# TorontoDeepLearning/convnet

Hardware: AMD Instinct MI355X
Metric: images/sec (fprop+bprop+wgrad) AlexNet 224x224 bs=256 (higher is better)
Workload: dtype f32

## Files before the change

convnet_amd/_lib.py:

```python
import ctypes
import os
import re

_HERE = os.path.dirname(os.path.abspath(__file__))
LIB_PATH = os.path.join(_HERE, "lib", "libconvnet_hip.so")
_ALT_LIB = os.environ.get("CONVNET_HIP_LIB")
if _ALT_LIB:
    LIB_PATH = _ALT_LIB if os.path.isabs(_ALT_LIB) else os.path.join(_HERE, "lib", _ALT_LIB)
HEADER_PATH = os.path.join(os.path.dirname(_HERE), "include", "convnet_hip.h")

c_float_p = ctypes.POINTER(ctypes.c_float)


class cudamat(ctypes.Structure):
    _fields_ = [("data_host", c_float_p),
                ("data_device", ctypes.c_void_p),
                ("on_device", ctypes.c_int),
                ("on_host", ctypes.c_int),
                ("size", ctypes.c_int * 2),
                ("is_trans", ctypes.c_int),
                ("owns_data", ctypes.c_int),
                ("tex_obj", ctypes.c_ulonglong)]


class Shape4D(ctypes.Structure):
    _fields_ = [("shape", ctypes.c_int * 4)]


class ConvDesc(ctypes.Structure):
    _fields_ = [(n, ctypes.c_int) for n in (
        "num_input_channels", "num_output_channels", "kernel_size_y", "kernel_size_x", "kernel_size_t",
        "stride_y", "stride_x", "stride_t", "padding_y", "padding_x", "padding_t",
        "input_channel_begin", "input_channel_end", "output_channel_begin", "output_channel_end", "num_groups")]

    def copy(self):
        c = ConvDesc()
        ctypes.memmove(ctypes.byref(c), ctypes.byref(self), ctypes.sizeof(ConvDesc))
        return c


class rnd_struct(ctypes.Structure):
    _fields_ = [("dev_mults", ctypes.c_void_p), ("dev_words", ctypes.c_void_p)]


class KernelInfo(ctypes.Structure):
    _fields_ = [("name", ctypes.c_char_p), ("flops", ctypes.c_double), ("grid_blocks", ctypes.c_int), ("split_k", ctypes.c_int)]


_CTYPES = {
    "void": None, "int": ctypes.c_int, "unsigned int": ctypes.c_uint, "long": ctypes.c_long, "size_t": ctypes.c_size_t,
    "float": ctypes.c_float, "double": ctypes.c_double, "bool": ctypes.c_bool,
    "void*": ctypes.c_void_p, "void**": ctypes.POINTER(ctypes.c_void_p), "char*": ctypes.c_char_p, "const char*": ctypes.c_char_p,
    "int*": ctypes.POINTER(ctypes.c_int), "float*": c_float_p, "const float*": c_float_p, "double*": ctypes.POINTER(ctypes.c_double),
    "cudamat*": ctypes.POINTER(cudamat), "cudamat**": ctypes.POINTER(ctypes.POINTER(cudamat)), "Shape4D*": ctypes.POINTER(Shape4D),
    "ConvDesc": ConvDesc, "rnd_struct*": ctypes.POINTER(rnd_struct), "ConvnetHipKernelInfo*": ctypes.POINTER(KernelInfo)}


def _ctype(decl, named, proto):
    tok = decl.replace("*", " * ").split()
    spell = lambda t: " ".join(t).replace(" *", "*")
    if named and len(tok) > 1 and tok[-1] != "*" and spell(tok) not in _CTYPES:
        tok = tok[:-1]
    if spell(tok) not in _CTYPES:
        raise ImportError(f"include/convnet_hip.h: '{proto}' uses the type '{spell(tok)}', which convnet_amd/_lib.py (_CTYPES) does not map")
    return _CTYPES[spell(tok)]


def header_signatures(text):
    body = re.sub(r"/\*.*?\*/", "", text, flags=re.S)
    body = body[body.index('extern "C" {'):]
    sigs = {}
    for res, name, args in re.findall(r"^[ \t]*([A-Za-z_][\w \t*]*?)\s*\b(\w+)\s*\(([^();{}]*)\)\s*;", body, flags=re.M):
        proto = f"{' '.join(res.split())} {name}({' '.join(args.split())})"
        args = [a for a in args.split(",") if a.split() not in ([], ["void"])]
        sigs[name] = (_ctype(res, False, proto), [_ctype(a, True, proto) for a in args])
    return sigs


def declared_symbols(header_path=HEADER_PATH):
    return sorted(header_signatures(open(header_path).read()))


def _load():
    if not os.path.exists(LIB_PATH):
        raise ImportError(
            f"{LIB_PATH} is missing: build it with `python -c 'import __graft_entry__ as g; g.build()'` "
            "(hipcc --offload-arch=gfx950).  There is no CPU fallback for the product path.")
    import torch
    lib = ctypes.CDLL(LIB_PATH)
    for name, (res, args) in header_signatures(open(HEADER_PATH).read()).items():
        if _ALT_LIB and not hasattr(lib, name):
            continue
        fn = getattr(lib, name)
        fn.restype = res
        fn.argtypes = args
    return lib


lib = _load()

_ERRORS = {
    -1: "Incompatible matrix dimensions.", -2: "CUBLAS error.", -3: "CUDA error: ", -4: "Operation not supported on views.",
    -5: "Operation not supported on transposed matrices.", -6: "Generic error.",
    -7: "Incompatible transposedness.", -8: "Matrix is not in device memory.", -9: "Operation not supported."}


def profile_enable(on=True):
    lib.convnet_hip_profile_enable(1 if on else 0)


def profile_report():
    buf = ctypes.create_string_buffer(1 << 16)
    n = lib.convnet_hip_profile_report(buf, len(buf))
    rows = []
    for line in buf.value.decode().splitlines() if n else []:
        k, op, cnt, ms, fl, by, ex = line.split("|")
        rows.append({"kernel": k, "op": op, "launches": int(cnt), "ms": float(ms), "flops": float(fl), "bytes": float(by), "executed": float(ex)})
    return rows


def GetStringError(err_code):
    msg = _ERRORS.get(err_code, "Unknown error")
    if err_code == -3:
        msg += lib.get_last_cuda_error().decode()
    return msg


def probe_matrix_pipe(random_operands=True, seconds=0.05):
    out = (ctypes.c_double * 4)()
    rc = lib.convnet_hip_probe_matrix_pipe(1 if random_operands else 0, float(seconds), out)
    if rc != 0:
        raise RuntimeError(f"convnet_hip_probe_matrix_pipe failed: {rc}")
    return {"bf16_tflops": out[0], "tflops_eq": out[1], "ghz_counter": out[2], "ghz_issue": out[3]}
```

convnet_amd/build.py:

```python
import os
import subprocess
import sys

HERE = os.path.dirname(os.path.abspath(__file__))
SRC = os.path.join(HERE, "csrc")
OUT = os.path.join(HERE, "lib", "libconvnet_hip.so")
SOURCES = ["state.hip", "gather_gemm.hip", "patch_gemm.hip", "wgrad_wide.hip", "fewc_conv.hip", "local_conv.hip", "conv3d.hip", "batch_norm.hip", "pool_norm.hip", "elementwise.hip", "input_staging.hip", "dataset_moments.hip", "feature_rows.hip", "comm.hip", "rccl_abi_check.hip", "probe.hip"]
FLAGS = ["--offload-arch=gfx950", "-O3", "-std=c++17", "-fPIC", "-Wno-comment", "-Wno-inline-asm"]
FILE_FLAGS = {"patch_gemm.hip": ["-fno-slp-vectorize"], "wgrad_wide.hip": ["-fno-slp-vectorize"], "fewc_conv.hip": ["-fno-slp-vectorize"]}
if os.environ.get("CONVNET_BUILD_NOSLP"):
    FILE_FLAGS["gather_gemm.hip"] = ["-fno-slp-vectorize"]
if os.environ.get("CONVNET_BUILD_DIAG"):
    FLAGS.append("-DCONVNET_DIAG")


def _stale(target, deps):
    if not os.path.exists(target):
        return True
    t = os.path.getmtime(target)
    return any(os.path.getmtime(d) > t for d in deps)


def build(force=False, verbose=False):
    os.makedirs(os.path.join(HERE, "lib"), exist_ok=True)
    objdir = os.path.join(HERE, "lib", "obj")
    os.makedirs(objdir, exist_ok=True)
    headers = [os.path.join(SRC, "common.h"), os.path.join(SRC, "gather_gemm.h"), os.path.join(SRC, "wgrad_wide_schedule.h"),
               os.path.join(HERE, "..", "include", "convnet_hip.h")]
    objs, procs = [], []
    for s in SOURCES:
        src = os.path.join(SRC, s)
        obj = os.path.join(objdir, s.replace(".hip", ".o"))
        objs.append(obj)
        if force or _stale(obj, [src] + headers):
            cmd = ["hipcc", *FLAGS, *FILE_FLAGS.get(s, []), "-c", src, "-o", obj]
            if verbose:
                print(" ".join(cmd))
            procs.append((s, subprocess.Popen(cmd, stdout=subprocess.PIPE, stderr=subprocess.STDOUT, text=True)))
    failed = False
    for s, p in procs:
        out, _ = p.communicate()
        if p.returncode != 0:
            failed = True
            print(f"--- {s} failed ---\n{out}", file=sys.stderr)
        elif verbose and out.strip():
            print(out)
    if failed:
        raise RuntimeError("hipcc failed")
    if force or procs or _stale(OUT, objs):
        cmd = ["hipcc", "--offload-arch=gfx950", "-shared", "-fPIC", "-o", OUT, *objs, "-ldl"]
        r = subprocess.run(cmd, capture_output=True, text=True)
        if r.returncode != 0:
            print(r.stdout, r.stderr, file=sys.stderr)
            raise RuntimeError("link failed")
    return OUT


if __name__ == "__main__":
    print(build(force="--force" in sys.argv, verbose=True))
```

convnet_amd/convnet.py:

```python
import os
import sys
from collections import deque
from typing import Callable, NamedTuple, Optional

import torch

from . import pbtxt
from .edge import AvgPoolEdge, ConvEdge, Edge, EdgeWithWeight, FCEdge, LocalEdge, MaxPoolEdge, ResponseNormEdge
from .layer import Layer, LinearLayer, LogisticLayer, ReLULayer, SoftmaxDistLayer, SoftmaxLayer
from .matrix import Matrix
from .optimizer import RunFusedSteps
from .trainer import TrainLoopMixin


class LayerPlan(NamedTuple):
    fuse_relu: Optional[bool]
    bn_relu: Optional[bool]
    activate: bool
    output_entry: Optional[Callable]
    logistic_dropout: bool
    dropout_scale: float
    down_scale: Optional[float]
    logistic_deriv: bool


def _zero_storage(m):
    t = getattr(m, "_t", None)
    if t is not None:
        t.zero_()


class ConvNet(TrainLoopMixin):
    def __init__(self, model, fused=False, process_id=0, num_processes=1, verbose=False, exchange=None, overlap_update=None,
                 overlap_wgrad=None):
        self.verbose = verbose
        self.fused = fused
        self.overlap_update_ = bool(overlap_update)
        self.overlap_wgrad_ = bool(overlap_wgrad)
        self.wgrad_order_ = os.environ.get("CONVNET_WGRAD_ORDER", "before")
        self.side_stream_ = None
        self._pending_updates = []
        self._in_train_step = False
        self.process_id_ = process_id
        self.num_processes_ = num_processes
        self.is_root_ = process_id == 0
        self.exchange_ = exchange
        if isinstance(model, pbtxt.Model):
            self.model_ = model
        elif "\n" in model or "{" in model:
            self.model_ = pbtxt.parse(model)
        else:
            self.model_ = pbtxt.read(model)
        m = self.model_
        for e in m.edge:
            if Edge.HasParameters(e):
                w_opt = m.default_weight_optimizer.copy()
                w_opt.MergeFrom(e.weight_optimizer)
                e.mutable("weight_optimizer").CopyFrom(w_opt)
                if not e.has_no_bias:
                    b_opt = m.default_bias_optimizer.copy()
                    b_opt.MergeFrom(e.bias_optimizer)
                    e.mutable("bias_optimizer").CopyFrom(b_opt)
        for l in m.layer:
            if l.batch_normalize:
                w_opt = m.default_weight_optimizer.copy()
                w_opt.MergeFrom(l.gamma_optimizer)
                l.mutable("gamma_optimizer").CopyFrom(w_opt)
                b_opt = m.default_bias_optimizer.copy()
                w_opt.MergeFrom(l.beta_optimizer)
                l.mutable("beta_optimizer").CopyFrom(b_opt)
        Matrix.InitRandom(m.seed + process_id)
        self.model_name_ = m.name
        self.layers_, self.edges_ = [], []
        self.input_layers_, self.output_layers_, self.data_layers_ = [], [], []
        self.batch_size_ = 0
        self.current_iter_ = 0
        self.parameters_, self.grad_parameters_, self.history_ = Matrix(), Matrix(), Matrix()
        self.second_history_ = Matrix()
        self.edge_slices_ = {}
        self.train_dataset_ = None
        self.train_dataset_config_ = self.valid_dataset_config_ = None
        self.correct_accum_ = None
        self._logits_pending = set()
        self._bn_steps = []
        self.BuildNet()
        if exchange is not None and any(l.UseBatchNormalization() for l in self.layers_):
            raise SystemExit("batch_normalize is not supported with a gradient exchange (data-parallel training)")

    def log(self, *a):
        if self.verbose:
            print(*a, file=sys.stderr)

    def BuildNet(self):
        m = self.model_
        self.layers_ = [Layer.ChooseLayerClass(l) for l in m.layer]
        self.edges_ = [Edge.ChooseEdgeClass(e) for e in m.edge]
        by_name = {e.GetName(): e for e in self.edges_}
        for e in self.edges_:
            if e.IsTied():
                e.SetTiedTo(by_name[e.GetTiedEdgeName()])
        for l in self.layers_:
            for e in self.edges_:
                if l.GetName() == e.GetSourceName():
                    l.AddOutgoing(e)
                    e.SetSource(l)
                    e.SetInputChannels(l.GetNumChannels(e.GetSourceSliceName()))
                if l.GetName() == e.GetDestName():
                    l.AddIncoming(e)
                    e.SetDest(l)
                    e.SetOutputChannels(l.GetNumChannels(e.GetDestSliceName()))
        self.Sort()
        for x in (*self.edges_, *self.layers_):
            x.fused = self.fused
            for opt in (getattr(x, n, None) for n in ("weight_optimizer_", "bias_optimizer_", "gamma_optimizer_", "beta_optimizer_")):
                if opt is not None:
                    opt.fused = self.fused
        for l in self.layers_:
            if l.UseBatchNormalization():
                self._check_batch_norm(l)
            self._check_slices(l)
            if not l.incoming_edge_:
                self.input_layers_.append(l)
                self.data_layers_.append(l)
            if not l.outgoing_edge_:
                self.output_layers_.append(l)
                self.data_layers_.append(l)
        for l in self.layers_:
            if l.IsInput():
                y, x, t = l.GetSizeY(), l.GetSizeX(), l.GetSizeT()
                if y <= 0:
                    y = m.patch_size
                if x <= 0:
                    x = m.patch_size
                if t <= 0:
                    t = 1
            else:
                e0 = l.incoming_edge_[0]
                y, x, t = e0.GetNumModulesY(), e0.GetNumModulesX(), e0.GetNumModulesT()
            l.SetSize(y, x, t)
            if t > 1 and l.UseBatchNormalization():
                raise SystemExit(f"batch_normalize on layer {l.GetName()}: not supported on a layer with image_size_t > 1 ({t} frames)")
            if t > 1 and l.HasSlices():
                raise SystemExit(f"layer_slice on layer {l.GetName()}: not supported on a layer with image_size_t > 1 ({t} frames): "
                                 "time is the outermost index, so a channel range is not one column range")
            self.log(f"Layer {l.GetName()}: {y}x{x}")
            for e in l.outgoing_edge_:
                e.SetImageSize(y, x, t)
        self.PlanLayers()

    def PlanLayers(self):
        self.plan_ = {l: self._plan_layer(l) for l in self.layers_}
        self.metric_on_device_ = len(self.output_layers_) == 1 and self.plan_[self.output_layers_[0]].output_entry is not None

    def _fused_down_scale(self, l):
        return self.plan_[l].down_scale

    def _plan_layer(self, l):
        fused, hidden = self.fused, not l.IsInput() and not l.IsOutput()
        bn, logistic, scale = l.UseBatchNormalization(), isinstance(l, LogisticLayer), l.TrainDropoutScale()
        for e in l.incoming_edge_:
            if isinstance(e, MaxPoolEdge):
                e.mask_legal_ = l.dropprob_ == 0 and type(l) in (LinearLayer, ReLULayer)
        fuse_up = (fused and self._each_alone_and_all_of(l, [e.GetDestSliceName() for e in l.incoming_edge_])
                   and not isinstance(l, SoftmaxLayer) and all(e.CanFuseUp(l) for e in l.incoming_edge_))
        activate = not fused if bn else not l.IsInput() and (not fuse_up or logistic)
        entry = None
        if fused and l.IsOutput() and not l.IsInput():
            single = len(self.output_layers_) == 1 and l.dropprob_ <= 0
            if type(l) is SoftmaxLayer:
                entry = Matrix.SoftmaxCEGradCorrect
            elif single and logistic and (l.loss_function_, l.performance_metric_) == ("CROSS_ENTROPY_BINARY", "CLASSIFICATION_BINARY"):
                entry = Matrix.LogisticCEGradCorrect
            elif single and isinstance(l, SoftmaxDistLayer) and l.loss_function_ == l.performance_metric_ == "CROSS_ENTROPY_MULTINOMIAL_DISTRIBUTED":
                entry = Matrix.SoftmaxDistCEGrad
        down_scale = None
        if fused and hidden and l.is_relu and self._each_alone_and_all_of(l, [e.GetSourceSliceName() for e in l.outgoing_edge_]):
            if all(e.can_fuse_mask and not e.IsBackPropBlocked() and not l.store_dropout_noise_
                   and not (isinstance(e, MaxPoolEdge) and scale != 1.0) for e in l.outgoing_edge_):
                down_scale = scale
        return LayerPlan(fuse_relu=(l.is_relu and not bn) if fuse_up else None, bn_relu=(fused and l.is_relu) if bn else None,
                         activate=activate, output_entry=entry, logistic_dropout=fused and logistic and not l.IsInput() and l.dropprob_ > 0,
                         dropout_scale=scale, down_scale=down_scale, logistic_deriv=fused and logistic and hidden)

    @staticmethod
    def _each_alone_and_all_of(l, slice_names):
        if slice_names == [""]:
            return True
        if not slice_names:
            return False
        return (len(set(slice_names)) == len(slice_names) and set(slice_names) == set(l.slice_channels_)
                and l.GetNumChannels() == sum(l.slice_channels_.values()))

    @staticmethod
    def _check_slices(l):
        name = l.GetName()
        for what, edges, get in (("read", l.outgoing_edge_, Edge.GetSourceSliceName), ("written", l.incoming_edge_, Edge.GetDestSliceName)):
            whole = [e.GetName() for e in edges if not get(e)]
            part = [e.GetName() for e in edges if get(e)]
            if whole and part:
                raise SystemExit(f"layer_slice on layer {name}: the layer is {what} both whole (edge {whole[0]}) and by slice (edge {part[0]}); "
                                 "their add-or-overwrite flags are independent, so one would overwrite what the other has written")
        if l.UseBatchNormalization():
            if l.HasSlices():
                raise SystemExit(f"batch_normalize on layer {name}: not supported on a layer with slices")
            for e in l.incoming_edge_:
                if e.GetSourceSliceName():
                    raise SystemExit(f"batch_normalize on layer {name}: not supported on a layer fed from a slice (edge {e.GetName()})")

    @staticmethod
    def _check_batch_norm(l):
        name = l.GetName()
        if l.IsInput() or l.IsOutput():
            raise SystemExit(f"batch_normalize on layer {name}: input and output layers cannot be batch-normalised")
        if type(l) not in (LinearLayer, ReLULayer):
            raise SystemExit(f"batch_normalize on layer {name}: only LINEAR and RECTIFIED_LINEAR activations are supported")
        for e in l.incoming_edge_:
            if isinstance(e, (MaxPoolEdge, ResponseNormEdge)):
                raise SystemExit(f"batch_normalize on layer {name}: not supported behind a {e.__class__.__name__} (edge {e.GetName()})")
            if not isinstance(e, (FCEdge, ConvEdge, LocalEdge, AvgPoolEdge)):
                raise SystemExit(f"batch_normalize on layer {name}: edge {e.GetName()} ({e.__class__.__name__}) is not supported")

    def Sort(self):
        L, S = [], deque(l for l in self.layers_ if l.IsInput())
        if not S:
            raise SystemExit("Error: No layer is set to be input!")
        while S:
            n = S.popleft()
            L.append(n)
            for e in n.outgoing_edge_:
                e.SetMark()
                mm = e.GetDest()
                if mm is None:
                    raise SystemExit(f"Edge {e.GetName()} has no destination layer")
                if all(f.HasMark() for f in mm.incoming_edge_):
                    S.append(mm)
        if not all(f.HasMark() for f in self.edges_):
            raise SystemExit("Error : Network has loop(s)!")
        self.layers_ = L

    def GetLayerByName(self, name):
        for l in self.layers_:
            if l.GetName() == name:
                return l
        raise SystemExit(f"Error: No layer called {name}")

    def GetEdgeByName(self, name):
        for e in self.edges_:
            if e.GetName() == name:
                return e
        raise SystemExit(f"Error: No edge called {name}")

    def SetBatchsize(self, batch_size):
        self.batch_size_ = batch_size

    def AllocateMemory(self, fprop_only=False):
        self.AllocateLayerMemory()
        self.AllocateEdgeMemory(fprop_only)
        if self.fused:
            self.correct_accum_ = Matrix()
            self.correct_accum_.AllocateGPUMemory(1, 1, "correct count")
            self.correct_accum_.Set(0.0)

    def AllocateLayerMemory(self):
        for l in self.layers_:
            l.AllocateMemory(self.batch_size_)

    def AllocateEdgeMemory(self, fprop_only):
        total, usage = 0, {}
        for e in self.edges_:
            mem = e.GetParameterMemoryRequirement()
            usage[e] = mem
            total += ((mem + 127) // 128) * 128
        self.parameters_.AllocateGPUMemory(1, total, "parameters")
        _zero_storage(self.parameters_)
        if not fprop_only:
            self.grad_parameters_.AllocateGPUMemory(1, total, "grad parameters")
            self.grad_parameters_.Set(0.0)
            self.history_.AllocateGPUMemory(1, total, "optimizer history")
            _zero_storage(self.history_)
            second = any(o is not None and o.NeedsSecondHistory() for e in self.edges_ if isinstance(e, EdgeWithWeight)
                         for o in (e.weight_optimizer_, e.bias_optimizer_))
            if second:
                self.second_history_.AllocateGPUMemory(1, total, "optimizer second-moment history")
                _zero_storage(self.second_history_)
        offset = 0
        for e in self.edges_:
            mem = usage[e]
            if mem == 0:
                continue
            s = Matrix()
            self.parameters_.GetSlice(s, offset, offset + mem)
            e.SetMemory(s)
            if not fprop_only:
                g, h, h2 = Matrix(), Matrix(), None
                self.grad_parameters_.GetSlice(g, offset, offset + mem)
                self.history_.GetSlice(h, offset, offset + mem)
                if second:
                    h2 = Matrix()
                    self.second_history_.GetSlice(h2, offset, offset + mem)
                e.SetGradMemory(g, h, h2)
            self.edge_slices_[e] = (offset, mem)
            offset += ((mem + 127) // 128) * 128
        if self.is_root_ or self.exchange_ is None:
            for e in self.edges_:
                e.Initialize()
# ... 66 lines not shown
            ev = torch.cuda.Event()
            ev.record(torch.cuda.current_stream())
            self._pending_updates.append((owner, ev, isinstance(owner, FCEdge)))
            self._flush_updates(final=False)

    def _flush_updates(self, final):
        keep = []
        for edge, ev, held in self._pending_updates:
            if held and not final:
                keep.append((edge, ev, held))
                continue
            bucket_ev = None
            if self.exchange_ is not None and edge in self.edge_slices_:
                state = self.exchange_.BucketState(edge)
                if state == "pending":
                    if final:
                        raise RuntimeError(f"gradient bucket of {edge.GetName()} was never exchanged")
                    keep.append((edge, ev, held))
                    continue
                bucket_ev = state
            self.side_stream_.wait_event(ev)
            if bucket_ev is not None and not hasattr(bucket_ev, "wait_library_stream"):
                self.side_stream_.wait_event(bucket_ev)
            with Matrix.OnStream(self.side_stream_):
                if hasattr(bucket_ev, "wait_library_stream"):
                    bucket_ev.wait_library_stream()
                edge.UpdateWeights()
        self._pending_updates = keep

    def Bprop(self):
        for l in reversed(self.layers_):
            p = self.plan_[l]
            for e in l.outgoing_edge_:
                self._bprop_edge(e.GetDest(), l, e, fuse_mask=p.down_scale)
            if p.logistic_deriv:
                l.GetDeriv().LogisticDerivScaled(l.GetState(), p.dropout_scale)
            elif p.down_scale is None:
                l.ApplyDerivativeofDropout()
                if not l.IsInput() and not l.IsOutput():
                    l.ApplyDerivativeOfActivation()
            if l.UseBatchNormalization():
                if not self.fused and self._in_train_step and self.side_stream_ is not None and self.overlap_wgrad_:
                    ev = torch.cuda.Event()
                    ev.record(self.side_stream_)
                    torch.cuda.current_stream().wait_event(ev)
                l.ApplyDerivativeofBatchNormalization(self._bn_steps if (self.fused and self._in_train_step) else None)

    def ComputeDeriv(self):
        for l in self.output_layers_:
            if l in self._logits_pending:
                self._logits_pending.discard(l)
                self.plan_[l].output_entry(l.GetState(), l.GetData(), l.GetState(), l.GetDeriv(), self.correct_accum_, l.loss_function_weight_)
            else:
                l.ComputeDeriv()

    def GetLoss(self):
        return None if self.metric_on_device_ else [l.GetPerformanceMetric() for l in self.output_layers_]

    def TimestampModel(self):
        import time
        ts = time.strftime("%Y%m%d%H%M%S")
        while ts in self.model_.timestamp:
            ts += "_"
        self.model_.timestamp.append(ts)
        fname = os.path.join(self.model_.checkpoint_dir, f"{self.model_.name}_{ts}")
        if self.model_.checkpoint_dir:
            os.makedirs(self.model_.checkpoint_dir, exist_ok=True)
            pbtxt.write(fname + ".pbtxt", self.model_)
        self.log_file_ = fname + "_train.log"
        self.val_log_file_ = fname + "_valid.log"
        return ts

    def ReadCorrectCount(self, reset=True):
        v = float(self.correct_accum_.ToNumpy().reshape(-1)[0])
        if reset:
            self.correct_accum_.Set(0.0)
        return v

    def UpdateWeights(self):
        bn_steps, self._bn_steps = self._bn_steps, []
        if self._in_train_step and self.side_stream_ is not None:
            if self.overlap_update_:
                self._flush_updates(final=True)
            done = torch.cuda.Event()
            done.record(self.side_stream_)
            torch.cuda.current_stream().wait_event(done)
            if self.overlap_update_:
                RunFusedSteps(bn_steps)
                return
        batch = list(bn_steps) if self.fused else None
        for e in self.edges_:
            if e.IsBackPropBlocked():
                continue
            if self.exchange_ is not None and e in self.edge_slices_:
                self.exchange_.WaitFor(e)
            if batch is not None and isinstance(e, EdgeWithWeight):
                e.UpdateWeights(batch)
            else:
                e.UpdateWeights()
        if batch:
            RunFusedSteps(batch)

    def SetupDataset(self, dataset, val_data_config_file=""):
        if not isinstance(dataset, str):
            self.train_dataset_ = dataset
            self.batch_size_ = dataset.GetBatchSize()
            return
        if dataset:
            self.train_dataset_config_ = pbtxt.read(dataset, pbtxt.DatasetConfig)
        if val_data_config_file:
            self.valid_dataset_config_ = pbtxt.read(val_data_config_file, pbtxt.DatasetConfig)
        if self.train_dataset_config_ is None:
            raise SystemExit("Error: No training set provided.")
        if self.valid_dataset_config_ is None:
            self.log("Warning: No validation set provided.")
        self.train_dataset_ = self._build_data_handler(self.train_dataset_config_)
        self.SetBatchsize(self.train_dataset_.GetBatchSize())
        self.log("Training data set size", self.train_dataset_.GetDataSetSize())
        if self.valid_dataset_config_ is not None:
            self.val_dataset_ = self._build_data_handler(self.valid_dataset_config_)
            self.log("Validation data set size", self.val_dataset_.GetDataSetSize())

    def _build_data_handler(self, config):
        from .datahandler import DataHandler
        dh = DataHandler(config, seed=self.model_.seed + self.process_id_)
        by_name = {l.GetName(): l for l in self.data_layers_}
        for name, st in dh.streams_.items():
            l = by_name.get(name)
            if l is None:
                raise SystemExit(f"Data stream for layer {name}: the model has no input or output layer of that name.")
            if l.IsInput():
                want = l.GetSizeY() * l.GetSizeX() * l.GetSizeT() * l.GetNumChannels()
                if st.StagedDims() != want:
                    raise SystemExit(f"Data stream for layer {name}: the stream stages {st.StagedDims()} values per case "
                                     f"(rows of {st.GetDims()}, cropped to gpu_image_size), the layer holds {want}.")
        dh.SetInputLayers([l.GetName() for l in self.data_layers_ if l.IsInput()])
        return dh

    def GetBatch(self, dataset):
        dataset.GetBatch(self.data_layers_)

    def TrainOneBatch(self):
        for l in self.layers_:
            l.ResetAddOrOverwrite()
        for e in self.edges_:
            e.NotifyStart()
        for l in self.layers_:
            l.NotifyStart()
        if self.exchange_ is not None:
            self.exchange_.StartStep()
        if (self.overlap_update_ or self.overlap_wgrad_) and self.side_stream_ is None and torch.cuda.is_available():
            self.side_stream_ = Matrix.SharedStream("side")
        self.GetBatch(self.train_dataset_)
        self.Fprop(True)
        self.ComputeDeriv()
        error = self.GetLoss()
        self._in_train_step = True
        try:
            self.Bprop()
            self.UpdateWeights()
        finally:
            self._in_train_step = False
        self.current_iter_ += 1
        return error

    def ReduceLearningRate(self, factor):
        for e in self.edges_:
            if isinstance(e, EdgeWithWeight):
                e.ReduceLearningRate(factor)

    def GetCheckpointFilename(self):
        m = self.model_
        ts = m.timestamp[-1] if m.timestamp else ""
        return os.path.join(m.checkpoint_dir, f"{m.name}_{ts}.h5")

    def Save(self, output_file=None):
        from . import hdf5io
        if output_file is None:
            fname = self.GetCheckpointFilename()
            self.Save(fname)
            if self.model_.polyak_after > 0:
                self.LoadPolyakWeights()
                self.Save(fname + "polyak")
                self.LoadCurrentWeights()
            return
        tmp = output_file + "temp"
        with hdf5io.File(tmp, "w") as f:
            for e in self.edges_:
                e.SaveParameters(f)
            f.WriteHDF5IntAttr("__lr_reduce_counter__", getattr(self, "lr_reduce_counter_", 0))
            f.WriteHDF5IntAttr("__current_iter__", self.current_iter_)
        os.replace(tmp, output_file)

    def Load(self, input_file=None):
        from . import hdf5io
        with hdf5io.File(input_file or self.GetCheckpointFilename()) as f:
            for e in self.edges_:
                e.LoadParameters(f)
            self.lr_reduce_counter_ = f.ReadHDF5IntAttr("__lr_reduce_counter__", getattr(self, "lr_reduce_counter_", 0))
            for _ in range(self.lr_reduce_counter_):
                self.ReduceLearningRate(self.model_.reduce_lr_factor)
            self.current_iter_ = f.ReadHDF5IntAttr("__current_iter__", self.current_iter_)
```

convnet_amd/csrc/common.h:

```cpp
#pragma once
#include <hip/hip_runtime.h>

#include <cstdint>
#include <cstdio>
#include <cstdlib>

#include "../../include/convnet_hip.h"

namespace chip {

hipStream_t stream();
void* workspace(size_t bytes);
void* workspace_aux(size_t bytes);
void* workspace_planes(size_t bytes);
void* workspace_banks(size_t bytes);
void* workspace_slabs(size_t bytes);
const float* zero_page();
int matrix_path();
void set_last_error(const char* msg);
void note_kernel(const char* name, double flops, int blocks, int split_k);

struct KernelTimer {
  KernelTimer(const char* name, const char* op, double flops, double bytes, double executed = 0.0);
  ~KernelTimer();
  int slot;
};

struct PendingOp {
  int kind;
  cudamat m[4];
  Shape4D s[3];
  ConvDesc desc;
  float scaleTargets;
  int i0, i1;
  float f0, f1;
  bool b0;
  cudamat bias, mask;
  int has_bias, relu, has_mask;
  void (*launch)(PendingOp&);
};
bool defer_begin(int kind, void (*launch)(PendingOp&));
PendingOp& pending();
void flush_pending();
extern long g_absorbed;

[[noreturn]] inline void fatal(const char* what, const char* file, int line) {
  fprintf(stderr, "libconvnet_hip: fatal: %s (%s:%d)\n", what, file, line);
  exit(EXIT_FAILURE);
}

#define CHIP_CHECK(expr)                                                            \
  do {                                                                              \
    hipError_t _e = (expr);                                                         \
    if (_e != hipSuccess) ::chip::fatal(hipGetErrorString(_e), __FILE__, __LINE__); \
  } while (0)

#define CHIP_REQUIRE(cond)                                       \
  do {                                                           \
    if (!(cond)) ::chip::fatal("check failed: " #cond, __FILE__, __LINE__); \
  } while (0)

inline int launch_status() {
  hipError_t e = hipGetLastError();
  if (e != hipSuccess) {
    set_last_error(hipGetErrorString(e));
    return CUDA_ERROR;
  }
  return 0;
}

inline int env_int(const char* name, int dflt) {
  const char* e = getenv(name);
  return e && *e ? atoi(e) : dflt;
}
#define CHIP_KNOB(name, dflt) ([] { static const int v_ = ::chip::env_int(name, dflt); return v_; }())
#ifdef CONVNET_DIAG
#define CHIP_DIAG_KNOB(name, dflt) CHIP_KNOB(name, dflt)
#else
#define CHIP_DIAG_KNOB(name, dflt) (dflt)
#endif

void filter_planes_share(bool on);
bool filter_planes_shared(const long long* key, int n);
void wg_batch_begin(int frames, void* (*slab_arena)(size_t bytes), size_t max_bytes);
bool wg_batch_active();
int wg_batch_frame();
void wg_batch_end();

inline int divup(int a, int b) { return (a + b - 1) / b; }
inline size_t numel(const cudamat* m) { return (size_t)m->size[0] * (size_t)m->size[1]; }
inline bool aligned16(const void* p) { return (reinterpret_cast<uintptr_t>(p) & 15) == 0; }

}
```

convnet_amd/csrc/elementwise.hip:

```cpp
#include <cfloat>
#include <climits>
#include <cmath>

#include "common.h"

namespace chip {

using f32x4 = __attribute__((ext_vector_type(4))) float;

constexpr int kThreads = 256;
constexpr int kMaxBlocks = 2048;

inline int blocks_for(size_t work_items) {
  size_t b = (work_items + kThreads - 1) / kThreads;
  if (b > kMaxBlocks) b = kMaxBlocks;
  if (b < 1) b = 1;
  return (int)b;
}

template <typename F>
__global__ void map2_kernel(float* __restrict__ out, const float* a, const float* b, size_t n, bool vec, F f) {
  const size_t tid = (size_t)blockIdx.x * blockDim.x + threadIdx.x, stride = (size_t)gridDim.x * blockDim.x;
  if (vec) {
    const size_t n4 = n >> 2;
// ... 678 lines not shown
}

__device__ __forceinline__ void sgd_one(float& g, float& w, float& h, float l2, float clip, float eps, float mom) {
#pragma clang fp contract(off)
  if (l2 > 0.f) {
    const float t = w * l2;
    g = g + t;
  }
  if (clip > 0.f) g = g > clip ? clip : (g < -clip ? -clip : g);
  g = g * eps;
  const float hm = h * mom;
  h = hm + g;
  w = w - h;
}

__device__ __forceinline__ void adagrad_one(float& g, float& w, float& h, float& a, float delta, float step_scale, float l2, float clip, float eps,
                                            float mom) {
#pragma clang fp contract(off)
  const float c = a - delta;
  const float cc = c * c;
  const float gg = g * g;
  const float s = cc + gg;
  a = delta + sqrtf(s);
  g = g / a;
  g = g * step_scale;
  sgd_one(g, w, h, l2, clip, eps, mom);
}
__device__ __forceinline__ void rmsprop_one(float& g, float& w, float& h, float& a, float factor, float l2, float clip, float eps, float mom) {
#pragma clang fp contract(off)
  h = h * mom;
  if (l2 > 0.f) {
    const float t = w * l2;
    g = g + t;
  }
  if (clip > 0.f) g = g > clip ? clip : (g < -clip ? -clip : g);
  const float fa = factor * a;
  const float faa = fa * a;
  const float omf = 1.f - factor;
  const float og = omf * g;
  const float ogg = og * g;
  const float s = faa + ogg;
  a = sqrtf(s);
  g = g / a;
  const float eg = eps * g;
  h = h + eg;
  w = w - h;
}

struct SgdOp {
  static constexpr int N = 3;
  static constexpr bool kRefuseHuge = false;
  float l2, clip, eps, mom;
  __device__ __forceinline__ void operator()(float (&v)[N]) const { sgd_one(v[0], v[1], v[2], l2, clip, eps, mom); }
};
struct AdagradOp {
  static constexpr int N = 4;
  static constexpr bool kRefuseHuge = true;
  float delta, step_scale, l2, clip, eps, mom;
  __device__ __forceinline__ void operator()(float (&v)[N]) const { adagrad_one(v[0], v[1], v[2], v[3], delta, step_scale, l2, clip, eps, mom); }
};
struct RmsPropOp {
  static constexpr int N = 4;
  static constexpr bool kRefuseHuge = true;
  float factor, l2, clip, eps, mom;
  __device__ __forceinline__ void operator()(float (&v)[N]) const { rmsprop_one(v[0], v[1], v[2], v[3], factor, l2, clip, eps, mom); }
};
template <typename Op>
struct StepItem {
  float* p[Op::N];
  unsigned long long n;
  Op op;
  int vec;
};
template <typename Op>
__device__ __forceinline__ void step_range(const StepItem<Op>& t, size_t tid, size_t stride) {
  constexpr int N = Op::N;
  const size_t n = (size_t)t.n;
  size_t done = 0;
  if (t.vec) {
    const size_t n4 = n >> 2;
    for (size_t i = tid; i < n4; i += stride) {
      f32x4 x[N];
#pragma unroll
      for (int k = 0; k < N; ++k) x[k] = reinterpret_cast<const f32x4*>(t.p[k])[i];
#pragma unroll
      for (int e = 0; e < 4; ++e) {
        float v[N];
#pragma unroll
        for (int k = 0; k < N; ++k) v[k] = x[k][e];
        t.op(v);
#pragma unroll
        for (int k = 0; k < N; ++k) x[k][e] = v[k];
      }
#pragma unroll
      for (int k = 0; k < N; ++k) reinterpret_cast<f32x4*>(t.p[k])[i] = x[k];
    }
    done = n4 << 2;
  }
  for (size_t i = done + tid; i < n; i += stride) {
    float v[N];
#pragma unroll
    for (int k = 0; k < N; ++k) v[k] = t.p[k][i];
    t.op(v);
#pragma unroll
    for (int k = 0; k < N; ++k) t.p[k][i] = v[k];
  }
}
constexpr int kSgdMulti = 16;
template <typename Op>
struct StepBatch {
  StepItem<Op> it[kSgdMulti];
};
template <typename Op>
__device__ __forceinline__ void step_single(const StepItem<Op>& t) {
  step_range(t, (size_t)blockIdx.x * blockDim.x + threadIdx.x, (size_t)gridDim.x * blockDim.x);
}
__global__ void sgd_kernel(const StepItem<SgdOp> t) { step_single(t); }
__global__ void adagrad_kernel(const StepItem<AdagradOp> t) { step_single(t); }
__global__ void rmsprop_kernel(const StepItem<RmsPropOp> t) { step_single(t); }
__global__ void sgd_multi_kernel(const StepBatch<SgdOp> b) { step_single(b.it[blockIdx.y]); }
__global__ void adagrad_multi_kernel(const StepBatch<AdagradOp> b) { step_single(b.it[blockIdx.y]); }
__global__ void rmsprop_multi_kernel(const StepBatch<RmsPropOp> b) { step_single(b.it[blockIdx.y]); }

template <typename Op>
int step_check(cudamat* const (&mats)[Op::N]) {
  const size_t n = numel(mats[1]);
  for (cudamat* m : mats)
    if (!m->on_device) return ERROR_NOT_ON_DEVICE;
  for (cudamat* m : mats)
    if (numel(m) != n) return ERROR_INCOMPATIBLE_DIMENSIONS;
  if (Op::kRefuseHuge && n > (size_t)INT_MAX) return ERROR_UNSUPPORTED;
  return 0;
}
template <typename Op>
StepItem<Op> step_item(cudamat* const (&mats)[Op::N], const Op& op) {
  StepItem<Op> t{};
  t.vec = 1;
  for (int k = 0; k < Op::N; ++k) {
    t.p[k] = mats[k]->data_device;
    t.vec &= aligned16(t.p[k]) ? 1 : 0;
  }
  t.n = numel(mats[1]);
  t.op = op;
  return t;
}
template <typename Op>
constexpr double step_bytes() { return 4.0 * (2 * Op::N - 1); }

template <typename Op, typename K>
int step_launch(K kernel, const char* name, const char* family, cudamat* const (&mats)[Op::N], const Op& op) {
  if (int rc = step_check<Op>(mats)) return rc;
  const size_t n = numel(mats[1]);
  if (n == 0) return 0;
  KernelTimer timer(name, family, 0.0, step_bytes<Op>() * n);
  hipLaunchKernelGGL(kernel, dim3(blocks_for(n / 4 + 1)), dim3(kThreads), 0, stream(), step_item<Op>(mats, op));
  return launch_status();
}
template <typename Op, typename K, typename F>
int step_launch_multi(K kernel, const char* name, const char* family, int count, F tensor) {
  cudamat* mats[Op::N];
  Op op;
  for (int i = 0; i < count; ++i) {
    tensor(i, mats, op);
    if (int rc = step_check<Op>(mats)) return rc;
  }
  for (int base = 0; base < count; base += kSgdMulti) {
    StepBatch<Op> b{};
    int m = 0;
    size_t most = 0, total = 0;
    for (int i = base; i < count && i < base + kSgdMulti; ++i) {
      tensor(i, mats, op);
      const size_t n = numel(mats[1]);
      if (n == 0) continue;
      b.it[m++] = step_item<Op>(mats, op);
      most = n > most ? n : most;
      total += n;
    }
    if (m == 0) continue;
    KernelTimer timer(name, family, 0.0, step_bytes<Op>() * total);
    hipLaunchKernelGGL(kernel, dim3(blocks_for(most / 4 + 1), m), dim3(kThreads), 0, stream(), b);
  }
  return launch_status();
}

}

using namespace chip;

extern "C" {

namespace {
inline bool same_mat(const cudamat* a, const cudamat& b) { return a->on_device && a->data_device == b.data_device && numel(a) == numel(&b); }
bool absorb_bias(cudamat* mat, cudamat* vec, cudamat* target) {
  PendingOp& o = pending();
  if (o.kind != 1 || o.has_bias || o.relu) return false;
  const int F = o.desc.num_output_channels;
  if (!same_mat(mat, o.m[2]) || !same_mat(target, o.m[2]) || mat->is_trans || !vec->on_device || (int)numel(vec) != F || mat->size[1] != F) return false;
  o.bias = *vec;
  o.has_bias = 1;
  ++g_absorbed;
  return true;
}
bool absorb_relu(cudamat* mat, float val, cudamat* target) {
  PendingOp& o = pending();
  if ((o.kind != 1 && o.kind != 4) || o.relu || val != 0.f) return false;
  const cudamat& t = o.kind == 1 ? o.m[2] : o.m[1];
  if (!same_mat(mat, t) || !same_mat(target, t)) return false;
  o.relu = 1;
  flush_pending();
  ++g_absorbed;
  return true;
}
bool absorb_relu_deriv(cudamat* deriv, cudamat* state, cudamat* target) {
  PendingOp& o = pending();
  if ((o.kind != 2 && o.kind != 3) || o.has_mask || !state->on_device || numel(state) != numel(deriv)) return false;
  const cudamat& t = o.kind == 2 ? o.m[2] : o.m[3];
  if (!same_mat(deriv, t) || !same_mat(target, t)) return false;
  if (o.kind == 3 && !same_mat(state, o.m[0])) return false;
  o.mask = *state;
  o.has_mask = 1;
  flush_pending();
  ++g_absorbed;
  return true;
}
}

int add_row_vec(cudamat* mat, cudamat* vec, cudamat* target) {
  if (absorb_bias(mat, vec, target)) return 0;
  return add_row(mat, vec, target, 1.0f);
}
int add_row_mult(cudamat* mat, cudamat* vec, cudamat* target, float mult) { return add_row(mat, vec, target, mult); }

int sum_by_axis(cudamat* mat, cudamat* target, int axis, float mult, float p) { return axis_sum<false>(mat, target, axis, mult, p); }
int sqsum_by_axis(cudamat* mat, cudamat* target, int axis, float mult, float p) { return axis_sum<true>(mat, target, axis, mult, p); }

float sum_all(cudamat* mat, int* err_code) { return reduce_all<0>(mat, nullptr, err_code); }
float vdot(cudamat* mat1, cudamat* mat2, int* err_code) {
  if (numel(mat1) != numel(mat2)) { *err_code = ERROR_INCOMPATIBLE_DIMENSIONS; return 0.f; }
  return reduce_all<1>(mat1, mat2, err_code);
}
float euclid_norm(cudamat* mat, int* err_code) { return sqrtf(reduce_all<2>(mat, nullptr, err_code)); }

int normlimit_by_axis(cudamat* mat, cudamat* target, int axis, float norm, int constraint) {
  if (!mat->on_device || !target->on_device) return ERROR_NOT_ON_DEVICE;
  if (mat->is_trans) return ERROR_TRANSPOSED;
  if (mat->size[0] != target->size[0] || mat->size[1] != target->size[1]) return ERROR_INCOMPATIBLE_DIMENSIONS;
  const int rows = mat->size[0], cols = mat->size[1];
  if (axis == 0)
    hipLaunchKernelGGL(normlimit_cols_kernel, dim3(cols), dim3(256), 0, stream(), mat->data_device, target->data_device, rows, norm, constraint);
  else
    return rows_normlimit(nullptr, mat->data_device, target->data_device, nullptr, rows, cols, norm, constraint, false, 0.f, 0.f, 0.f, 0.f);
  return launch_status();
}

int sgd_momentum_step_normlimit(cudamat* grad, cudamat* param, cudamat* history, float l2_decay, float gradient_clip, float epsilon,
                                float momentum, float norm, int constraint) {
  const size_t n = numel(param);
  if (!grad->on_device || !param->on_device || !history->on_device) return ERROR_NOT_ON_DEVICE;
  if (numel(grad) != n || numel(history) != n) return ERROR_INCOMPATIBLE_DIMENSIONS;
  if (param->is_trans) return ERROR_TRANSPOSED;
  if (n == 0) return 0;
  return rows_normlimit(grad->data_device, param->data_device, param->data_device, history->data_device, param->size[0], param->size[1], norm,
                        constraint, true, l2_decay, gradient_clip, epsilon, momentum);
}

int lower_bound_scalar(cudamat* mat, float val, cudamat* target) {
  if (absorb_relu(mat, val, target)) return 0;
  return map2(target, mat, nullptr, [val] __device__(float x, float) { return x > val ? x : val; });
}
int upper_bound_mod_scalar(cudamat* mat, float val, cudamat* target) {
  return map2(target, mat, nullptr, [val] __device__(float x, float) { return x > val ? val : (x < -val ? -val : x); });
}
int apply_rectified_linear_deriv(cudamat* mat1, cudamat* mat2, cudamat* target) {
  if (absorb_relu_deriv(mat1, mat2, target)) return 0;
  return map2(target, mat1, mat2, [] __device__(float d, float s) { return s > 0.f ? d : 0.f * d; });
}
int assign_scalar(cudamat* mat, float alpha) {
  return map2(mat, mat, nullptr, [alpha] __device__(float, float) { return alpha; });
}
int add_scalar(cudamat* mat, float alpha, cudamat* target) {
  return map2(target, mat, nullptr, [alpha] __device__(float x, float) { return x + alpha; });
}
int mult_by_scalar(cudamat* mat, float alpha, cudamat* target, float scale_targets) {
  if (scale_targets == 0.f) return map2(target, mat, nullptr, [alpha] __device__(float x, float) { return x * alpha; });
  return map2(target, mat, target, [alpha, scale_targets] __device__(float x, float t) { return scale_targets * t + x * alpha; });
}
int divide_by_scalar(cudamat* mat, float alpha, cudamat* target) {
  return map2(target, mat, nullptr, [alpha] __device__(float x, float) { return x / alpha; });
}
int add_mult(cudamat* mat1, cudamat* mat2, float alpha) {
  return map2(mat1, mat1, mat2, [alpha] __device__(float x, float y) {
#pragma clang fp contract(off)
    const float t = alpha * y;
    return x + t;
  });
}
int add_elementwise(cudamat* mat1, cudamat* mat2, cudamat* target) {
  return map2(target, mat1, mat2, [] __device__(float x, float y) { return x + y; });
}
int subtract_elementwise(cudamat* mat1, cudamat* mat2, cudamat* target) {
  return map2(target, mat1, mat2, [] __device__(float x, float y) { return x - y; });
}
int mult_elementwise(cudamat* mat1, cudamat* mat2, cudamat* target, float scale_targets) {
  if (scale_targets != 0.f) return ERROR_UNSUPPORTED;
  return map2(target, mat1, mat2, [] __device__(float x, float y) { return x * y; });
}
int apply_sqrt(cudamat* mat, cudamat* target) {
  return map2(target, mat, nullptr, [] __device__(float x, float) { return sqrtf(x); });
}

int softmax_row_major_multi(cudamat* mat, int numslices, cudamat* target) {
  if (!mat->on_device || !target->on_device) return ERROR_NOT_ON_DEVICE;
  if (mat->is_trans) return ERROR_TRANSPOSED;
  const size_t len = numel(mat);
  if (numslices <= 0 || len % numslices != 0 || numel(target) != len) return ERROR_INCOMPATIBLE_DIMENSIONS;
  const int rows = (int)(len / numslices), cols = numslices;
  SoftmaxOut o{target->data_device, nullptr, nullptr};
  hipLaunchKernelGGL(softmax_rows_kernel<32>, dim3(divup(rows, 32)), dim3(1024), 0, stream(), mat->data_device, nullptr, o, rows, cols, 1.0f);
  return launch_status();
}
int softmax_row_major(cudamat* mat, cudamat* target) { return softmax_row_major_multi(mat, mat->size[1], target); }

int apply_softmax_grad_row_major(cudamat* mat, cudamat* labels, cudamat* target) {
  if (!mat->on_device || !labels->on_device || !target->on_device) return ERROR_NOT_ON_DEVICE;
  if (numel(labels) != (size_t)mat->size[0] || numel(target) != numel(mat)) return ERROR_INCOMPATIBLE_DIMENSIONS;
  if (target->data_device != mat->data_device) {
    int rc = copy_on_device(mat, target);
    if (rc) return rc;
  }
  hipLaunchKernelGGL(softmax_grad_kernel, dim3(divup(mat->size[0], 256)), dim3(256), 0, stream(), labels->data_device, target->data_device, mat->size[0]);
  return launch_status();
}

int get_softmax_correct_row_major(cudamat* mat, cudamat* labels, cudamat* target) {
  if (!mat->on_device || !labels->on_device || !target->on_device) return ERROR_NOT_ON_DEVICE;
  if (mat->is_trans) return ERROR_TRANSPOSED;
  if (target->size[0] != mat->size[0] || target->size[1] != 1 || numel(labels) != (size_t)mat->size[0]) return ERROR_INCOMPATIBLE_DIMENSIONS;
  hipLaunchKernelGGL(softmax_correct_kernel, dim3(divup(mat->size[0], 32)), dim3(1024), 0, stream(), mat->data_device, labels->data_device,
                     target->data_device, mat->size[0], mat->size[1]);
  return launch_status();
}

int get_softmax_cross_entropy_row_major(cudamat* mat, cudamat* labels, cudamat* target, float tiny) {
  if (!mat->on_device || !labels->on_device || !target->on_device) return ERROR_NOT_ON_DEVICE;
  if (mat->is_trans) return ERROR_TRANSPOSED;
  if (target->size[0] != mat->size[0] || target->size[1] != 1 || labels->size[0] != mat->size[0] || labels->size[1] != 1)
    return ERROR_INCOMPATIBLE_DIMENSIONS;
  hipLaunchKernelGGL(softmax_ce_kernel, dim3(divup(mat->size[0], 256)), dim3(256), 0, stream(), mat->data_device, labels->data_device,
                     target->data_device, mat->size[0], tiny);
  return launch_status();
}

int softmax_ce_grad_correct(cudamat* logits, cudamat* labels, cudamat* probs, cudamat* deriv, cudamat* correct_accum, float deriv_scale) {
  if (!logits->on_device || !labels->on_device || !probs->on_device) return ERROR_NOT_ON_DEVICE;
  if (numel(probs) != numel(logits) || (deriv && numel(deriv) != numel(logits)) || numel(labels) != (size_t)logits->size[0])
    return ERROR_INCOMPATIBLE_DIMENSIONS;
  SoftmaxOut o{probs->data_device, deriv ? deriv->data_device : nullptr, correct_accum ? correct_accum->data_device : nullptr};
  KernelTimer timer("softmax_rows_kernel", "softmax_ce", 0.0, 4.0 * numel(logits) * (deriv ? 3 : 2));
  hipLaunchKernelGGL(softmax_rows_kernel<32>, dim3(divup(logits->size[0], 32)), dim3(1024), 0, stream(), logits->data_device, labels->data_device, o,
                     logits->size[0], logits->size[1], deriv_scale);
  return launch_status();
}

int sgd_momentum_step(cudamat* grad, cudamat* param, cudamat* history, float l2_decay, float gradient_clip, float epsilon, float momentum) {
  cudamat* const mats[] = {grad, param, history};
  return step_launch<SgdOp>(sgd_kernel, "sgd_kernel", "sgd", mats, SgdOp{l2_decay, gradient_clip, epsilon, momentum});
}

int sgd_momentum_step_multi(int count, cudamat** grads, cudamat** params, cudamat** histories, const float* l2_decay, const float* gradient_clip,
                            const float* epsilon, const float* momentum) {
  if (count < 0 || (count > 0 && (!grads || !params || !histories || !l2_decay || !gradient_clip || !epsilon || !momentum))) return ERROR_GENERIC;
  return step_launch_multi<SgdOp>(sgd_multi_kernel, "sgd_multi_kernel", "sgd", count, [&](int i, cudamat* (&m)[3], SgdOp& op) {
    m[0] = grads[i]; m[1] = params[i]; m[2] = histories[i];
    op = SgdOp{l2_decay[i], gradient_clip[i], epsilon[i], momentum[i]};
  });
}

namespace {
int second_moment_check(const cudamat* a, const cudamat* b, const cudamat* c) {
  if (!a->on_device || !b->on_device || (c && !c->on_device)) return ERROR_NOT_ON_DEVICE;
  if (a->is_trans != b->is_trans) return ERROR_TRANSPOSEDNESS;
  if (numel(a) != numel(b) || (c && numel(a) != numel(c))) return ERROR_INCOMPATIBLE_DIMENSIONS;
  return 0;
}
}

int adagrad(cudamat* history, cudamat* grad, float delta) {
  if (int rc = second_moment_check(history, grad, nullptr)) return rc;
  return map2(history, history, grad, [delta] __device__(float h, float g) {
#pragma clang fp contract(off)
    const float c = h - delta;
    const float cc = c * c;
    const float gg = g * g;
    const float s = cc + gg;
    return delta + sqrtf(s);
  });
}
int rms_prop(cudamat* history, cudamat* grad, float factor) {
  if (int rc = second_moment_check(history, grad, nullptr)) return rc;
  return map2(history, history, grad, [factor] __device__(float h, float g) {
#pragma clang fp contract(off)
    const float fh = factor * h;
    const float fhh = fh * h;
    const float omf = 1.f - factor;
    const float og = omf * g;
    const float ogg = og * g;
    const float s = fhh + ogg;
    return sqrtf(s);
  });
}
int divide_elementwise(cudamat* mat1, cudamat* mat2, cudamat* target) {
  if (int rc = second_moment_check(mat1, mat2, target)) return rc;
  return map2(target, mat1, mat2, [] __device__(float x, float y) { return x / y; });
}
// ... 156 lines not shown
```

convnet_amd/csrc/fewc_conv.hip:

```cpp
#include <algorithm>

#include "gather_gemm.h"

namespace chip {
namespace gfc {

constexpr int KX = 7, KY = 7, CH = 3, S = 2, NR = CH * KY, P = 4, IMG = 32;
constexpr int PW = S * (P - 1) + KX;
constexpr int XB = IMG * 4;
constexpr int RP = 2;
constexpr int ROWB = RP * 1024;
static_assert(PW * XB <= ROWB, "patch row");
constexpr int NCH = 10, ROWS = 96;
constexpr int H0_ROWS = 11, H1_ROWS = 10;
constexpr int H0_BYTES = H0_ROWS * ROWB, H1_BYTES = H1_ROWS * ROWB;
constexpr int BIAS_OFF = 0, BIAS_BYTES = 512;
constexpr int A_OFF = BIAS_BYTES;
constexpr int A_CHUNK = 6 * ROWS * 16;
constexpr int A_BYTES = NCH * A_CHUNK;
constexpr int A_PIECES = A_BYTES / 1024;
constexpr int PATCH_OFF = A_OFF + A_BYTES;
constexpr int ZERO_OFF = PATCH_OFF + H0_BYTES + H1_BYTES;
constexpr int ZERO_BYTES = 1024 + 256;
constexpr int LDS_BYTES = ZERO_OFF + ZERO_BYTES;
static_assert(LDS_BYTES <= 160 * 1024, "LDS");
static_assert(A_BYTES % 1024 == 0, "filter bank in whole pieces");
constexpr int NGROUP = 3 * 4;
constexpr int DUMP_BYTES = 4096;

__host__ __device__ constexpr int row_off(int r) { return r < 10 ? r * ROWB : r == 20 ? 10 * ROWB : H0_BYTES + (r - 10) * ROWB; }
__host__ __device__ constexpr int slot_k(int c, int lh, int j) {
  const int r = 2 * c + (j >> 2), kx = 2 * (j & 3) + lh;
  if (kx < KX) return kx + KX * r;
  return r < KX ? r + KX * 20 : -1;
}

struct Params {
  const float* src;
  const u32x4* planes;
  float* dst;
  float* dump;
  const float* bias;
  const float* zero;
  int F, N, H, W, My, Mx, pady, padx;
  int XG, IB, tiles;
  int relu;
  int diag;
};

}

__global__ void gfc_planes_kernel(const float* __restrict__ W, u32x4* __restrict__ out, int F) {
  using namespace gfc;
  const int i = blockIdx.x * blockDim.x + threadIdx.x;
  if (i >= NCH * 2 * ROWS) return;
  const int f = i % ROWS, lh = (i / ROWS) & 1, c = i / (2 * ROWS);
  Split8 sp = {};
  if (f < F) {
    float x[8];
#pragma unroll
    for (int j = 0; j < 8; ++j) {
      const int k = slot_k(c, lh, j);
      x[j] = k >= 0 ? W[(size_t)f + (size_t)F * k] : 0.f;
    }
    split8_sat(x, sp);
  }
  u32x4* o = out + ((size_t)c * 6 + lh) * ROWS + f;
  o[0] = sp.h;
  o[2 * ROWS] = sp.m;
  o[4 * ROWS] = sp.l;
}

template <bool RELU>
__global__ __launch_bounds__(320, 1) void gfc_kernel(const gfc::Params p) {
  using namespace gfc;
  extern __shared__ __attribute__((aligned(16))) float smem[];
  char* const lds = reinterpret_cast<char*>(smem);
  const int tid = threadIdx.x;
  const int wave = __builtin_amdgcn_readfirstlane(tid >> 6), lane = tid & 63;
  const int N = p.N;

  const int G = gridDim.x, q = p.tiles / G, rem = p.tiles % G, b = blockIdx.x;
  const int T0 = b * q + min(b, rem), T1 = T0 + q + (b < rem ? 1 : 0);
  if (T0 >= T1) return;
  int xg = T0 % p.XG, oy = (T0 / p.XG) % p.My, ib = T0 / (p.XG * p.My);
  auto next_tile = [&]() __attribute__((always_inline)) {
    if (++xg == p.XG) {
      xg = 0;
      if (++oy == p.My) {
        oy = 0;
        ++ib;
      }
    }
  };

  for (int i = wave; i < A_PIECES; i += 5) {
    const char* g = reinterpret_cast<const char*>(p.planes) + (size_t)i * 1024 + lane * 16;
    __builtin_amdgcn_global_load_lds((gbl_ptr_t)g, (lds_ptr_t)(lds + A_OFF + i * 1024), 16, 0, 0);
  }
  if (tid * 16 < ZERO_BYTES) *reinterpret_cast<u32x4*>(lds + ZERO_OFF + tid * 16) = u32x4{0, 0, 0, 0};
  if (tid < BIAS_BYTES / 4) *reinterpret_cast<float*>(lds + BIAS_OFF + tid * 4) = p.bias && tid < p.F ? p.bias[tid] : 0.f;

  if (wave == 4) {
    const int lx = lane >> 3;
    const unsigned lane_off = (unsigned)lx * (unsigned)(N * 4) + (unsigned)(lane & 7) * 16u;
    const size_t plane = (size_t)p.H * p.W * N * 4, rowb = (size_t)p.W * N * 4;
    auto issue_half = [&](auto HH) __attribute__((always_inline)) {
      constexpr int h = decltype(HH)::value;
      constexpr int n = h ? H1_ROWS : H0_ROWS;
      const int y0 = S * oy - p.pady, x0 = S * P * xg - p.padx;
      const char* const origin = reinterpret_cast<const char*>(p.src) + ((ptrdiff_t)y0 * p.W + x0) * (ptrdiff_t)(N * 4) + (ptrdiff_t)ib * (IMG * 4);
      bool xok[RP];
#pragma unroll
      for (int k = 0; k < RP; ++k) xok[k] = 8 * k + lx < PW && (unsigned)(x0 + 8 * k + lx) < (unsigned)p.W;
#pragma unroll
      for (int idx = 0; idx < n; ++idx) {
        const int r = h ? 10 + idx : idx == 10 ? 20 : idx;
        const int ch = r / KY, ky = r % KY;
        const bool yok = (unsigned)(y0 + ky) < (unsigned)p.H;
        const char* const rowp = origin + (size_t)ch * plane + (size_t)ky * rowb;
#pragma unroll
        for (int k = 0; k < RP; ++k) {
          const char* g = yok && xok[k] ? rowp + (size_t)(8 * k) * (size_t)(N * 4) + lane_off : reinterpret_cast<const char*>(p.zero);
          __builtin_amdgcn_global_load_lds((gbl_ptr_t)g, (lds_ptr_t)(lds + PATCH_OFF + (h ? H0_BYTES : 0) + idx * ROWB + k * 1024), 16, 0, 0);
        }
      }
    };
    using H0 = std::integral_constant<int, 0>;
    using H1 = std::integral_constant<int, 1>;
    issue_half(H0{});
    issue_half(H1{});
    __builtin_amdgcn_s_waitcnt(0x0070);
    __syncthreads();
    for (int T = T0; T < T1; ++T) {
      const bool more = T + 1 < T1 && !(p.diag & 2);
      __builtin_amdgcn_s_waitcnt(0x0070);
      __syncthreads();
      next_tile();
      if (more) issue_half(H0{});
      __builtin_amdgcn_s_waitcnt(0x0070);
      __syncthreads();
      if (more) issue_half(H1{});
    }
    __builtin_amdgcn_s_waitcnt(0x0070);
    return;
  }

  const int li = lane & 31, lh = lane >> 5;
  const unsigned base_l = (unsigned)(PATCH_OFF + (S * wave) * XB + li * 4 + lh * XB);
  const unsigned a_l = (unsigned)(A_OFF + (lh * ROWS + li) * 16);
  const unsigned lh_mask = lh ? 0xFFFFFFFFu : 0u;

  f32x16 acc[2][3];
  u32x4 fah[2][3], fam[3], fal[3];
  Split8 fb[2];
  float bv[8];
#ifndef CONVNET_EMU
#define CHIP_HERE() asm volatile("" ::: "memory")
#else
#define CHIP_HERE() ((void)0)
#endif
  auto read_a = [&](auto CC, auto PL, u32x4 (&dst)[3]) __attribute__((always_inline)) {
    constexpr int c = decltype(CC)::value, pl = decltype(PL)::value;
    CHIP_HERE();
#pragma unroll
    for (int t = 0; t < 3; ++t) dst[t] = *reinterpret_cast<const u32x4*>(lds + a_l + c * A_CHUNK + pl * (2 * ROWS * 16) + t * 512);
  };
  auto read_b = [&](auto CC) __attribute__((always_inline)) {
    constexpr int c = decltype(CC)::value;
    unsigned lhm = lh_mask;
    CHIP_HERE();
#ifndef CONVNET_EMU
    asm volatile("" : "+v"(lhm));
#endif
#pragma unroll
    for (int j = 0; j < 8; ++j) {
      const int r = 2 * c + (j >> 2);
      const int imm_n = row_off(r) + 2 * (j & 3) * XB;
      if ((j & 3) != 3) {
        bv[j] = *reinterpret_cast<const float*>(lds + base_l + imm_n);
      } else {
        const int imm_s = r < KX ? row_off(20) + (r - 1) * XB : (ZERO_OFF - PATCH_OFF);
        bv[j] = *reinterpret_cast<const float*>(lds + (base_l + (lhm & (unsigned)(imm_s - imm_n))) + imm_n);
      }
    }
  };
  auto split_pair = [&](int s, int q) __attribute__((always_inline)) {
    const float x0 = bv[2 * q], x1 = bv[2 * q + 1];
    const unsigned H = pk_bf16(x0, x1);
    const float r0 = x0 - __uint_as_float(H << 16), r1 = x1 - __uint_as_float(H & 0xffff0000u);
    const unsigned M = pk_bf16(r0, r1);
    const float s0 = r0 - __uint_as_float(M << 16), s1 = r1 - __uint_as_float(M & 0xffff0000u);
    fb[s].h[q] = H;
    fb[s].m[q] = M;
    fb[s].l[q] = pk_bf16(s0, s1);
#ifndef CONVNET_EMU
    asm volatile("" ::"v"(fb[s].h[q]), "v"(fb[s].m[q]), "v"(fb[s].l[q]));
#endif
  };
  auto mac_step = [&](auto K, int s, f32x16 (&a)[3]) __attribute__((always_inline)) {
    constexpr int k = decltype(K)::value;
#pragma unroll
    for (int t = 0; t < 3; ++t) {
      const u32x4& av = k == 1 ? fal[t] : k == 2 || k == 3 ? fam[t] : fah[s][t];
      const u32x4& bw = k == 0 ? fb[s].l : k == 2 || k == 4 ? fb[s].m : fb[s].h;
      a[t] = mma_bf16(av, bw, a[t]);
    }
#ifndef CONVNET_EMU
    asm volatile("" : "+v"(a[0]), "+v"(a[1]), "+v"(a[2]));
#endif
  };

  struct Out {
    unsigned lane_bytes;
    int flim;
  };
  const size_t fstride = (size_t)p.My * p.Mx * N;
  const int q4 = li & 3;
  auto out_of = [&](int xg_, int oy_, int ib_, bool exists) __attribute__((always_inline)) {
    const int ox = P * xg_ + wave;
    Out o;
    o.lane_bytes = (unsigned)((((size_t)oy_ * p.Mx + ox) * N + ib_ * IMG + 4 * (li >> 2) + (size_t)(q4 + 4 * lh) * fstride) * 4);
    o.flim = exists && ox < p.Mx ? p.F : 0;
// ... 3 lines not shown
    return o;
  };
  const unsigned bias_q = (unsigned)(BIAS_OFF + (q4 + 4 * lh) * 4);
  auto bias_of = [&](auto GG) __attribute__((always_inline)) {
    constexpr int gi = decltype(GG)::value;
    return *reinterpret_cast<const float*>(lds + bias_q + (32 * (gi >> 2) + 8 * (gi & 3)) * 4);
  };
  auto swap1 = [](float v) __attribute__((always_inline)) {
#ifndef CONVNET_EMU
    return __builtin_bit_cast(float, __builtin_amdgcn_mov_dpp(__builtin_bit_cast(int, v), 0xB1, 0xF, 0xF, true));
#else
    return emu::shfl_xor(v, 1);
#endif
  };
  auto swap2 = [](float v) __attribute__((always_inline)) {
#ifndef CONVNET_EMU
    return __builtin_bit_cast(float, __builtin_amdgcn_mov_dpp(__builtin_bit_cast(int, v), 0x4E, 0xF, 0xF, true));
#else
    return emu::shfl_xor(v, 2);
#endif
  };
  const bool odd1 = (li & 1) != 0, odd2 = (li & 2) != 0;
  auto store_group = [&](auto GG, const Out& o, const f32x16 (&a)[3], float bias) __attribute__((always_inline)) {
    constexpr int gi = decltype(GG)::value, t = gi >> 2, g = gi & 3;
    constexpr int cf = 32 * t + 8 * g;
    float x0 = a[t][4 * g], x1 = a[t][4 * g + 1], x2 = a[t][4 * g + 2], x3 = a[t][4 * g + 3];
    {
      const float r01 = swap1(odd1 ? x0 : x1), r23 = swap1(odd1 ? x2 : x3);
      x0 = odd1 ? r01 : x0; x1 = odd1 ? x1 : r01;
      x2 = odd1 ? r23 : x2; x3 = odd1 ? x3 : r23;
    }
    {
      const float ra = swap2(odd2 ? x0 : x2), rb = swap2(odd2 ? x1 : x3);
      x0 = odd2 ? ra : x0; x1 = odd2 ? rb : x1;
      x2 = odd2 ? x2 : ra; x3 = odd2 ? x3 : rb;
    }
    f32x4 v = {x0 + bias, x1 + bias, x2 + bias, x3 + bias};
    if constexpr (RELU) {
#pragma unroll
      for (int e = 0; e < 4; ++e) v[e] = fmaxf(v[e], 0.f);
    }
    const bool real = cf < o.flim;
    char* const rowb = real ? reinterpret_cast<char*>(p.dst) + (size_t)cf * fstride * 4 : reinterpret_cast<char*>(p.dump);
    const unsigned off = real ? o.lane_bytes : (unsigned)lane * 16u;
#ifdef CONVNET_DIAG
    if (p.diag & 4) return;
#endif
    *reinterpret_cast<f32x4*>(rowb + off) = v;
  };

  auto chunk_body = [&](auto CC, bool has_next, f32x16 (&cur)[3], const f32x16 (&prev)[3], const Out& po) __attribute__((always_inline)) {
    constexpr int c = decltype(CC)::value, s = c & 1;
    using CN = std::integral_constant<int, (c + 1) % NCH>;
    __builtin_amdgcn_sched_barrier(0);
    if (has_next) {
      read_b(CN{});
      read_a(CN{}, std::integral_constant<int, 0>{}, fah[s ^ 1]);
    }
    CHIP_HERE();
    const float bs0 = bias_of(std::integral_constant<int, c>{});
    float bs1 = 0.f;
    if constexpr (c >= 8) bs1 = bias_of(std::integral_constant<int, c + 2>{});
    static_for<0, 6>([&](auto KK) __attribute__((always_inline)) {
      constexpr int k = decltype(KK)::value;
      if constexpr (k >= 1 && k <= 4) {
        if (has_next) split_pair(s ^ 1, k - 1);
      }
      if constexpr (k == 0 && c >= 8) store_group(std::integral_constant<int, c + 2>{}, po, prev, bs1);
      if constexpr (k == 5) store_group(std::integral_constant<int, c>{}, po, prev, bs0);
      if constexpr (k == 2) {
        if (has_next) read_a(CN{}, std::integral_constant<int, 2>{}, fal);
      }
      if constexpr (k == 4) {
        if (has_next) read_a(CN{}, std::integral_constant<int, 1>{}, fam);
      }
      mac_step(KK, s, cur);
#pragma unroll
      for (int i = 0; i < 3; ++i) {
        __builtin_amdgcn_sched_group_barrier(0x008, 1, 0);
        __builtin_amdgcn_sched_group_barrier(0x100, 4, 0);
        __builtin_amdgcn_sched_group_barrier(0x002, 12, 0);
        __builtin_amdgcn_sched_group_barrier(0x040, 1, 0);
      }
      __builtin_amdgcn_sched_barrier(0);
    });
  };
  auto run_tile = [&](bool more, f32x16 (&cur)[3], const f32x16 (&prev)[3], const Out& po) __attribute__((always_inline)) {
#pragma unroll
    for (int t = 0; t < 3; ++t)
#pragma unroll
      for (int e = 0; e < 16; ++e) cur[t][e] = 0.f;
    static_for<0, NCH>([&](auto CC) __attribute__((always_inline)) {
      constexpr int c = decltype(CC)::value;
      if constexpr (c == 4) __syncthreads();
      if constexpr (c == NCH - 1) __syncthreads();
      if constexpr (c + 1 < NCH) chunk_body(CC, true, cur, prev, po);
      else chunk_body(CC, more, cur, prev, po);
    });
  };

  __builtin_amdgcn_s_waitcnt(0x0070);
  __syncthreads();
  {
    using C0 = std::integral_constant<int, 0>;
    read_b(C0{});
    read_a(C0{}, std::integral_constant<int, 0>{}, fah[0]);
    read_a(C0{}, std::integral_constant<int, 1>{}, fam);
    read_a(C0{}, std::integral_constant<int, 2>{}, fal);
  }
#pragma unroll
  for (int q4 = 0; q4 < 4; ++q4) split_pair(0, q4);
  Out po = out_of(0, 0, 0, false);
  int T = T0;
  for (;;) {
    run_tile(T + 1 < T1, acc[0], acc[1], po);
    po = out_of(xg, oy, ib, true);
    next_tile();
    if (++T >= T1) {
      static_for<0, NGROUP>([&](auto GG) __attribute__((always_inline)) { store_group(GG, po, acc[0], bias_of(GG)); });
      break;
    }
    run_tile(T + 1 < T1, acc[1], acc[0], po);
    po = out_of(xg, oy, ib, true);
    next_tile();
    if (++T >= T1) {
      static_for<0, NGROUP>([&](auto GG) __attribute__((always_inline)) { store_group(GG, po, acc[1], bias_of(GG)); });
      break;
    }
  }
}

bool gfc_try(const float* images, const float* filters, const float* bias, float* targets, int N, int C, int H, int W, int F, int Ky, int Kx,
             int sy, int sx, int pady, int padx, int My, int Mx, float scaleTargets, int relu, double flops) {
  using namespace gfc;
  if (!CHIP_KNOB("CONVNET_GG_FEWC", 1) || matrix_path() != 1) return false;
  if (Kx != KX || Ky != KY || C != CH || sy != S || sx != S || F > ROWS || F < 8 || F % 8 != 0 || N % IMG != 0 || My < 1 || Mx < 1) return false;
  if (pady < 0 || padx < 0 || (size_t)C * H * W * N * 4 >= (size_t(1) << 32) || (size_t)F * My * Mx * N * 4 >= (size_t(1) << 32)) return false;
  if (scaleTargets != 0.f) return false;
  if ((reinterpret_cast<uintptr_t>(images) | reinterpret_cast<uintptr_t>(targets)) & 15) return false;
  static bool once = false;
  static int cus = 256;
  if (!once) {
    CHIP_CHECK(hipFuncSetAttribute(reinterpret_cast<const void*>(gfc_kernel<false>), hipFuncAttributeMaxDynamicSharedMemorySize, LDS_BYTES));
    CHIP_CHECK(hipFuncSetAttribute(reinterpret_cast<const void*>(gfc_kernel<true>), hipFuncAttributeMaxDynamicSharedMemorySize, LDS_BYTES));
#ifndef CONVNET_EMU
    int dev = 0;
    hipDeviceProp_t prop;
    if (hipGetDevice(&dev) == hipSuccess && hipGetDeviceProperties(&prop, dev) == hipSuccess && prop.multiProcessorCount > 0) cus = prop.multiProcessorCount;
#else
    cus = 4;
#endif
    once = true;
  }
  u32x4* planes = static_cast<u32x4*>(workspace_aux(A_BYTES + DUMP_BYTES));
  (void)filter_planes_shared(nullptr, 0);
  {
    KernelTimer timer("filter_planes_kernel", "conv_fprop", 0.0, 4.0 * F * C * Ky * Kx + A_BYTES);
    hipLaunchKernelGGL(gfc_planes_kernel, dim3(divup(NCH * 2 * ROWS, 256)), dim3(256), 0, stream(), filters, planes, F);
  }
  Params p{};
  p.src = images; p.planes = planes; p.dst = targets; p.bias = bias; p.zero = zero_page();
  p.dump = reinterpret_cast<float*>(reinterpret_cast<char*>(planes) + A_BYTES);
  p.F = F; p.N = N; p.H = H; p.W = W; p.My = My; p.Mx = Mx; p.pady = pady; p.padx = padx;
  p.XG = divup(Mx, P); p.IB = N / IMG; p.tiles = p.XG * My * p.IB;
  p.relu = relu; p.diag = CHIP_DIAG_KNOB("CONVNET_GFC_DIAG", 0);
  const int grid = std::min(cus, p.tiles);
  {
    KernelTimer timer("gfc_kernel<96x128,split>", "conv_fprop", flops, 0.0, 0.0);
    if (relu) hipLaunchKernelGGL(gfc_kernel<true>, dim3(grid), dim3(320), LDS_BYTES, stream(), p);
    else hipLaunchKernelGGL(gfc_kernel<false>, dim3(grid), dim3(320), LDS_BYTES, stream(), p);
  }
  note_kernel("gfc_kernel(fprop)", flops, grid, 1);
  return true;
}

}
```

convnet_amd/csrc/gather_gemm.h:

```cpp
#pragma once
#include <cmath>
#include <cstring>
#include <type_traits>

#include "common.h"

namespace chip {

using f32x16 = __attribute__((ext_vector_type(16))) float;
using u32x4 = __attribute__((ext_vector_type(4))) unsigned;
using f32x4 = __attribute__((ext_vector_type(4))) float;

constexpr int BK = 16;

#ifdef CONVNET_GG_TRACE
constexpr bool kTrace = CONVNET_GG_TRACE >= 2;
__device__ unsigned long long* g_gg_trace = nullptr;
#else
constexpr bool kTrace = false;
#endif
__device__ __forceinline__ unsigned long long trace_clock() {
#ifdef CONVNET_GG_TRACE
  return __builtin_amdgcn_s_memtime();
#else
// ... 268 lines not shown
            for (int e = 0; e < NTC; ++e) v[e] = v[e] > 0.f ? v[e] : 0.f;
          }
          if (p.mask) {
            const fvec mk = *reinterpret_cast<const fvec*>(p.mask + (dp - p.dst));
#pragma unroll
            for (int e = 0; e < NTC; ++e) v[e] = mk[e] > 0.f ? v[e] * p.post_scale : 0.f;
          }
          *reinterpret_cast<fvec*>(dp) = v;
        } else {
#pragma unroll
          for (int e = 0; e < NTC; ++e) {
            if (n + e < N) {
              float x = v[e];
              if (p.scaleTargets != 0.f) x = p.scaleTargets * dp[e] + x;
              x += bv;
              if (p.relu) x = x > 0.f ? x : 0.f;
              if (p.mask) x = p.mask[(dp - p.dst) + e] > 0.f ? x * p.post_scale : 0.f;
              dp[e] = x;
            }
          }
        }
      } else {
        if (VEC) {
          *reinterpret_cast<fvec*>(dp) = v;
        } else {
#pragma unroll
          for (int e = 0; e < NTC; ++e)
            if (n + e < N) dp[e] = v[e];
        }
      }
    }
  }
}

struct Split8 {
  u32x4 h, m, l;
};
__device__ __forceinline__ unsigned pk_bf16(float a, float b) {
  typedef float f32x2_t __attribute__((ext_vector_type(2)));
  typedef __bf16 bf16x2_t __attribute__((ext_vector_type(2)));
  f32x2_t v = {a, b};
  return __builtin_bit_cast(unsigned, __builtin_convertvector(v, bf16x2_t));
}
__device__ __forceinline__ void split8(const float (&x)[8], Split8& s) {
#pragma unroll
  for (int q = 0; q < 4; ++q) {
    const float x0 = x[2 * q], x1 = x[2 * q + 1];
    const unsigned H = pk_bf16(x0, x1);
    const float r0 = x0 - __uint_as_float(H << 16), r1 = x1 - __uint_as_float(H & 0xffff0000u);
    const unsigned M = pk_bf16(r0, r1);
    const float s0 = r0 - __uint_as_float(M << 16), s1 = r1 - __uint_as_float(M & 0xffff0000u);
    s.h[q] = H;
    s.m[q] = M;
    s.l[q] = pk_bf16(s0, s1);
  }
}
__device__ __forceinline__ void split8_sat(float (&x)[8], Split8& s) {
#pragma unroll
  for (int j = 0; j < 8; ++j)
    if (fabsf(x[j]) > __uint_as_float(0x7F7F7FFFu)) x[j] = copysignf(__uint_as_float(0x7F7F0000u), x[j]);
  split8(x, s);
}
__device__ __forceinline__ f32x16 mma_bf16(u32x4 a, u32x4 b, f32x16 c) {
  typedef __bf16 bf16x8_t __attribute__((ext_vector_type(8)));
  return __builtin_amdgcn_mfma_f32_32x32x16_bf16(__builtin_bit_cast(bf16x8_t, a), __builtin_bit_cast(bf16x8_t, b), c, 0, 0, 0);
}
__device__ __forceinline__ f32x4 mma_bf16(u32x4 a, u32x4 b, f32x4 c) {
  typedef __bf16 bf16x8_t __attribute__((ext_vector_type(8)));
  return __builtin_amdgcn_mfma_f32_16x16x32_bf16(__builtin_bit_cast(bf16x8_t, a), __builtin_bit_cast(bf16x8_t, b), c, 0, 0, 0);
}

template <typename Acc>
__device__ __forceinline__ Acc split_mac(const Split8& a, const Split8& b, Acc v) {
  v = mma_bf16(a.m, b.m, v);
  v = mma_bf16(a.h, b.l, v);
  v = mma_bf16(a.l, b.h, v);
  v = mma_bf16(a.h, b.m, v);
  v = mma_bf16(a.m, b.h, v);
  v = mma_bf16(a.h, b.h, v);
  return v;
}

struct GGTile {
  const float* A;
  int K, GX, G, TX, TYX, y0, x0, dy0, dx0, ncols, col_tiles;
  int L, tsplit;
};
__device__ __forceinline__ bool gg_select_tile(const GGParams& p, const GGClassTable& ct, GGTile& t) {
  t.A = p.A; t.K = p.K; t.GX = p.GX; t.G = p.G; t.TX = p.TX; t.TYX = p.TYX; t.y0 = p.y0; t.x0 = p.x0; t.dy0 = p.dy0; t.dx0 = p.dx0;
  t.ncols = p.ncols; t.col_tiles = p.col_tiles; t.tsplit = -1;
  if (ct.n > 0) {
    const int b = blockIdx.x;
    if (b >= ct.c[ct.n - 1].tile_end) return false;
    int c = 0;
    while (b >= ct.c[c].tile_end) ++c;
    const int cbeg = c > 0 ? ct.c[c - 1].tile_end : 0;
    {
      const int i = b - cbeg, T = ct.c[c].tile_end - cbeg;
      const int q = T >> 3, m = T & 7, r = i & 7;
      t.L = r * q + (r < m ? r : m) + (i >> 3);
    }
    const GGClass& k = ct.c[c];
    t.A = k.A; t.K = k.K; t.GX = k.GX; t.G = k.G; t.TX = k.TX; t.TYX = k.TYX;
    t.y0 = k.y0; t.x0 = k.x0; t.dy0 = k.dy0; t.dx0 = k.dx0; t.ncols = k.ncols; t.col_tiles = k.col_tiles;
  } else if (p.tail_splits > 1) {
    const int k = blockIdx.x & 7, i = blockIdx.x >> 3;
    if (i < p.tail_tf8) {
      t.L = k * p.tail_tf8 + i;
    } else {
      const int j = k * p.tail_tt8 + (i - p.tail_tf8);
      if (j >= (p.row_tiles * t.col_tiles - p.tail_first) * p.tail_splits) return false;
      t.L = p.tail_first + j / p.tail_splits;
      t.tsplit = j % p.tail_splits;
    }
  } else {
    const int tiles = p.row_tiles * t.col_tiles;
    const int per = (tiles + 7) >> 3;
    t.L = xcd_remap(blockIdx.x, tiles);
    if (t.L >= tiles || (int)blockIdx.x >= per * 8) return false;
  }
  return true;
}

constexpr int kTailFixParts = 4;
template <int WR, int WC, int MT, int CW, bool VEC>
__global__ __launch_bounds__(WR* WC * 64) void gg_tail_fix_kernel(const GGParams p) {
  constexpr int NT = WR * WC * 64, NTC = CW / 32, ROWS = WR * MT * 32;
  using fvec = __attribute__((ext_vector_type(NTC))) float;
  const int tile = blockIdx.x / kTailFixParts, part = blockIdx.x % kTailFixParts;
  const int L = p.tail_first + tile;
  const int tid = threadIdx.x;
  const int reg_lo = part * (16 / kTailFixParts), reg_hi = reg_lo + 16 / kTailFixParts;
  f32x16 acc[MT][NTC];
  const float* pp = p.tail_partial + (size_t)tile * p.tail_splits * (size_t)(ROWS * WC * CW);
#pragma unroll
  for (int t = 0; t < MT; ++t)
#pragma unroll
    for (int reg = 0; reg < 16; ++reg) {
      if (reg < reg_lo || reg >= reg_hi) continue;
      fvec v = *reinterpret_cast<const fvec*>(pp + ((size_t)(t * 16 + reg) * NT + tid) * NTC);
      for (int sp = 1; sp < p.tail_splits; ++sp)
        v += *reinterpret_cast<const fvec*>(pp + (size_t)sp * (ROWS * WC * CW) + ((size_t)(t * 16 + reg) * NT + tid) * NTC);
#pragma unroll
      for (int u = 0; u < NTC; ++u) acc[t][u][reg] = v[u];
    }
  gg_epilogue<WR, WC, MT, CW, VEC>(p, acc, L % p.row_tiles, L / p.row_tiles, 0, p.ncols, p.GX, p.G, p.dy0, p.dx0, reg_lo, reg_hi);
}

struct PatchBank {
  const float* W;
  int F, C, Ky, Kx, cy, cx, sy, sx, TYc, TXc;
  bool dgrad;
};
void filter_planes_rt_launch(const PatchBank& bank, void* out, int TYX, int TH, const char* op);
void filter_planes_gk_launch(const float* W, void* out, int F, int K, int KP, int TH, const char* op);
bool patch_shape_ok(GGParams& p, size_t dst_elems);
void patch_run(GGParams& p, size_t dst_elems, const char* op, double flops, const PatchBank& bank);
bool patch_classes_ok(const GGParams& base, const GGClassTable& ct);
void patch_run_classes(GGParams& p, GGClassTable& ct, const char* op, double flops, double exec);

bool gfc_try(const float* images, const float* filters, const float* bias, float* targets, int N, int C, int H, int W, int F, int Ky, int Kx,
             int sy, int sx, int pady, int padx, int My, int Mx, float scaleTargets, int relu, double flops);

struct WGParams {
  const float* src;
  const float* dout;
  float* dst;
  float* partial;
  const float* zero;
  float* bias_dst;
  int K, F, N;
  int GX, M;
  int TX, TYX;
  int SH, SW;
  int ssy, ssx, y0, x0;
  int nchunk;
  int chunks_total;
  int chunks_per_split;
  int splits;
  int k_tiles, f_tiles;
  float scaleTargets, scaleOutput;
  int prio;
  int wide;
};

constexpr int WG_NB = 32;
constexpr int WG_PITCH = WG_NB + 4;

void wg_reduce_launch(const WGParams& p, size_t total, int splits, int groups, const char* op);
float* wg_batch_partial(const WGParams& p, size_t total, int splits);
bool wgw_try(WGParams& p, bool vec, bool split_products, const char* op, double flops, double exec);

void gg_reduce_launch(const GGParams& p, size_t dst_elems, int splits, const char* op);

inline double gg_split_time(int tiles, int sp, double slots, double tile_flops, double block_rate, size_t dst_elems) {
  const double rounds = std::ceil(tiles * (double)sp / slots);
  double t = rounds * (tile_flops / sp) / block_rate;
  if (sp > 1) t += sizeof(float) * (double)dst_elems * (2.0 * sp + 1) / 4.0e12 + 4e-6;
  return t;
}
inline int gg_split_k(int tiles, double slots, double tile_flops, double block_rate, size_t dst_elems, int kchunks, int units,
                      double* best_time = nullptr) {
  int splits = 1;
  double best_t = 1e30;
  if (dst_elems > 0 && kchunks >= 16)
    for (int sp = 1; sp <= 16 && kchunks / sp >= 8 && units / sp >= 1; ++sp) {
      const double t = gg_split_time(tiles, sp, slots, tile_flops, block_rate, dst_elems);
      if (t < best_t * 0.97) {
        best_t = t;
        splits = sp;
      }
    }
  if (best_time) *best_time = best_t;
  return splits;
}
inline bool gg_partial_last_round(int tiles, int slots, int kchunks) { return tiles > slots && tiles % slots != 0 && kchunks >= 32; }
inline int gg_tail_split(int tiles, int slots, double tile_flops, double block_rate, int tile_elems, int kchunks) {
  const int rem = tiles - (tiles / slots) * slots;
  const double tile_bytes = sizeof(float) * (double)tile_elems;
  const double t_round = tile_flops / block_rate;
  double best = 0.95;
  int best_s = 1;
  for (int s = 2; s <= 8 && kchunks / s >= 8; ++s) {
    const double cost = std::ceil(rem * (double)s / slots) / s + (rem * (s + 1.0) * tile_bytes / 4.0e12 + 6e-6) / t_round;
    if (cost < best) {
      best = cost;
      best_s = s;
    }
  }
  return best_s;
}
inline void gg_set_tail(GGParams& p, int tiles, int slots, int units, int s, int tile_elems) {
  const int full = (tiles / slots) * slots, rem = tiles - full;
  p.tail_first = full;
  p.tail_cps = divup(units, s);
  p.tail_splits = divup(units, p.tail_cps);
  p.tail_tf8 = full / 8;
  p.tail_tt8 = divup(rem * p.tail_splits, 8);
  p.tail_partial = static_cast<float*>(workspace(sizeof(float) * (size_t)rem * p.tail_splits * tile_elems));
}

}
```

convnet_amd/csrc/gather_gemm.hip:

```cpp
#include <algorithm>
#include <array>
#include <cmath>
#include <map>
#include <vector>
#include <cstdlib>
#include <string>
#include <type_traits>

#include "common.h"

#include "gather_gemm.h"

namespace chip {

template <int WR, int WC, int MT, int CW, bool A_KCONTIG, bool VEC, bool O3 = false, bool SPLIT = false>
__global__ __launch_bounds__(WR* WC * 64, (O3 ? 3 : 2)) void gg_kernel(const GGParams pin, const GGClassTable ct) {
  constexpr int NT = WR * WC * 64;
  constexpr int NTC = CW / 32, CW4 = CW / 4;
  using fvec = __attribute__((ext_vector_type(NTC))) float;
  constexpr int ROWS = WR * MT * 32;
  constexpr int APITCH = A_KCONTIG ? (BK + 4) : ROWS;
  constexpr int A_STAGE = A_KCONTIG ? ROWS * APITCH : BK * ROWS;
  constexpr int B_STAGE = WC * BK * CW;
  constexpr int NA = ((A_KCONTIG ? ROWS * (BK / 4) : BK * (ROWS / 4)) + NT - 1) / NT;
// ... 1482 lines not shown
}

void gg_run_classes(GGParams& p, GGClassTable& ct, bool vec, const GGTimer& tm) {
  gg_with_tile(gg_tile(p.R, vec, false), [&](auto t) {
    using T = decltype(t);
    gg_launch_classes<T::WR, T::WC, T::MT, T::CW>(p, ct, vec, tm);
  });
}

template <int WM, int WN, int MT, int NTL, int TS = 32>
void wg_launch_cfg(WGParams& p, bool vec, const GGTimer& tm) {
  constexpr int KT = WM * MT * TS, FT = WN * NTL * TS;
  const size_t lds = sizeof(float) * 2 * (KT + FT) * (vec ? WG_NB : WG_PITCH);
  p.k_tiles = divup(p.K, KT);
  if (p.bias_dst && divup(p.K + 1, KT) != p.k_tiles) p.bias_dst = nullptr;
  p.f_tiles = divup(p.F, FT);
  p.zero = zero_page();
  p.prio = wg_prio_mode();
  const int tiles = p.k_tiles * p.f_tiles;
  const size_t total = (size_t)(p.K + (p.bias_dst ? 1 : 0)) * p.F;
  const bool no_wide = CHIP_DIAG_KNOB("CONVNET_WG_NO_WIDE", 0) != 0;
  p.wide = (!no_wide && vec && TS == 32 && WM == 2 && WN == 2 && MT == 2 && NTL == 2 && p.F % 4 == 0 && aligned16(p.dst) &&
            (!p.bias_dst || aligned16(p.bias_dst))) ? 1 : 0;
  int splits = 1;
  if (tiles < kTargetBlocks) {
    splits = kTargetBlocks / tiles;
    const int max_by_len = p.chunks_total / 16 > 0 ? p.chunks_total / 16 : 1;
    if (splits > max_by_len) splits = max_by_len;
    const size_t max_by_bytes = (size_t(256) << 20) / (total * sizeof(float)) + 1;
    if ((size_t)splits > max_by_bytes) splits = (int)max_by_bytes;
    if (splits > 1024) splits = 1024;
    if (splits < 1) splits = 1;
  }
  p.chunks_per_split = divup(p.chunks_total, splits);
  splits = divup(p.chunks_total, p.chunks_per_split);
  p.splits = splits;
  const int groups = splits > 64 ? 32 : 1;
  float* const frame_slabs = wg_batch_partial(p, total, splits);
  p.partial = frame_slabs ? frame_slabs
                          : splits > 1 ? static_cast<float*>(workspace(sizeof(float) * total * (splits + (groups > 1 ? groups : 0)))) : nullptr;
  dim3 grid(((tiles * splits + 7) / 8) * 8), block(WM * WN * 64);
  static const std::string kname_f = "wg_kernel<" + std::to_string(WM) + "," + std::to_string(WN) + "," + std::to_string(MT) + "," + std::to_string(NTL) + (TS == 16 ? ",x16>" : ">");
  static const std::string kname_s = kname_f.substr(0, kname_f.size() - 1) + ",split>";
  const bool split_products = vec && wg_split_mode();
  const std::string& kname = split_products ? kname_s : kname_f;
  {
    KernelTimer timer(kname.c_str(), tm.op, tm.flops, 0.0, tm.exec);
    if (split_products) {
      allow_big_lds(wg_kernel<WM, WN, MT, NTL, true, TS, true>, lds);
      hipLaunchKernelGGL((wg_kernel<WM, WN, MT, NTL, true, TS, true>), grid, block, lds, stream(), p);
    } else if (vec) {
      allow_big_lds(wg_kernel<WM, WN, MT, NTL, true, TS>, lds);
      hipLaunchKernelGGL((wg_kernel<WM, WN, MT, NTL, true, TS>), grid, block, lds, stream(), p);
    } else {
      allow_big_lds(wg_kernel<WM, WN, MT, NTL, false, TS>, lds);
      hipLaunchKernelGGL((wg_kernel<WM, WN, MT, NTL, false, TS>), grid, block, lds, stream(), p);
    }
  }
  if (splits > 1 && !frame_slabs) wg_reduce_launch(p, total, splits, groups, tm.op);
}

void wg_launch(WGParams& p, bool vec, const GGTimer& tm) {
  if (wgw_try(p, vec, vec && wg_split_mode(), tm.op, tm.flops, tm.exec)) return;
  int ft = 128, pad = divup(p.F, 128) * 128;
  const int cands[3] = {96, 64, 32};
  for (int c : cands) {
    const int q = divup(p.F, c) * c;
    if (q < pad) {
      ft = c;
      pad = q;
    }
  }
  const bool k160 = divup(p.K, 160) * 160 < divup(p.K, 128) * 128;
  if (ft == 128) wg_launch_cfg<2, 2, 2, 2>(p, vec, tm);
  else if (ft == 96 && k160) wg_launch_cfg<2, 2, 5, 3, 16>(p, vec, tm);
  else if (ft == 96) wg_launch_cfg<4, 1, 1, 3>(p, vec, tm);
  else if (ft == 64) wg_launch_cfg<4, 1, 1, 2>(p, vec, tm);
  else wg_launch_cfg<4, 1, 1, 1>(p, vec, tm);
}

struct ConvGeo {
  int N, C, H, W, F, Ky, Kx, sy, sx, py, px, My, Mx;
};

ConvGeo conv_geo(const Shape4D* img, const Shape4D* flt, const Shape4D* out, const ConvDesc& d, const cudamat* mi,
                 const cudamat* mf, const cudamat* mo) {
  ConvGeo g;
  g.N = img->shape[0]; g.W = img->shape[1]; g.H = img->shape[2]; g.C = img->shape[3];
  g.Mx = out->shape[1]; g.My = out->shape[2]; g.F = out->shape[3];
  g.Ky = d.kernel_size_y; g.Kx = d.kernel_size_x; g.sy = d.stride_y; g.sx = d.stride_x;
  g.py = d.padding_y; g.px = d.padding_x;
  CHIP_REQUIRE(out->shape[0] == g.N);
  CHIP_REQUIRE(d.num_input_channels == g.C && d.num_output_channels == g.F);
  CHIP_REQUIRE(d.num_groups == 1);
  CHIP_REQUIRE(d.input_channel_begin == 0 && (d.input_channel_end == 0 || d.input_channel_end == g.C));
  CHIP_REQUIRE(d.output_channel_begin == 0 && (d.output_channel_end == 0 || d.output_channel_end == g.F));
  CHIP_REQUIRE(flt->shape[0] == g.F && flt->shape[1] == g.Kx && flt->shape[2] == g.Ky && flt->shape[3] == g.C);
  CHIP_REQUIRE(mi->size[0] == g.N && mi->size[1] == g.H * g.W * g.C);
  CHIP_REQUIRE(mo->size[0] == g.N && mo->size[1] == g.My * g.Mx * g.F);
  CHIP_REQUIRE(mf->size[0] == g.F && mf->size[1] == g.Ky * g.Kx * g.C);
  CHIP_REQUIRE(g.My == (g.H - 2 * g.py - g.Ky) / g.sy + 1 && g.Mx == (g.W - 2 * g.px - g.Kx) / g.sx + 1);
  CHIP_REQUIRE(d.kernel_size_t <= 1);
  CHIP_REQUIRE((size_t)g.N * g.H * g.W * g.C < (1ull << 31) && (size_t)g.N * g.My * g.Mx * g.F < (1ull << 31));
  return g;
}

inline bool gg_presplit_mode() {
  return gg_split_mode() && !CHIP_DIAG_KNOB("CONVNET_GG_NO_PRESPLIT", 0);
}

const unsigned* gk_table(int C, int H, int W, int N, int Ky, int Kx) {
  static std::map<std::array<int, 7>, unsigned*> cache;
  int dev = 0;
  CHIP_CHECK(hipGetDevice(&dev));
  const std::array<int, 7> key = {dev, C, H, W, N, Ky, Kx};
  auto it = cache.find(key);
  if (it != cache.end()) return it->second;
  const int K = C * Ky * Kx, KP = divup(K, BK) * BK;
  std::vector<unsigned> tab(2 * (size_t)KP);
  for (int k = 0; k < KP; ++k) {
    const int kk = std::min(k, K - 1), ch = kk / (Ky * Kx), tap = kk % (Ky * Kx), a = tap / Kx, b = tap % Kx;
    tab[k] = (unsigned)(((size_t)(ch * H + a) * W + b) * N * 4);
    tab[KP + k] = ((unsigned)a << 16) | (unsigned)b;
  }
  unsigned* d = nullptr;
  CHIP_CHECK(hipMalloc((void**)&d, tab.size() * sizeof(unsigned)));
  CHIP_CHECK(hipMemcpy(d, tab.data(), tab.size() * sizeof(unsigned), hipMemcpyHostToDevice));
  cache[key] = d;
  return d;
}

void conv_up_impl(cudamat* images, cudamat* filters, cudamat* bias, cudamat* targets, Shape4D* is, Shape4D* fs, Shape4D* ts,
                  const ConvDesc& d, float scaleTargets, int relu) {
  const ConvGeo g = conv_geo(is, fs, ts, d, images, filters, targets);
  GGParams p{};
  p.A = filters->data_device; p.src = images->data_device; p.dst = targets->data_device;
  p.bias = bias ? bias->data_device : nullptr;
  p.R = g.F; p.K = g.C * g.Ky * g.Kx; p.N = g.N; p.lda = g.F;
  p.GX = g.Mx; p.G = g.My * g.Mx; p.TX = g.Kx; p.TYX = g.Ky * g.Kx;
  p.SH = g.H; p.SW = g.W; p.ssy = g.sy; p.ssx = g.sx; p.y0 = g.py; p.x0 = g.px; p.dir = 1;
  p.DW = g.Mx; p.DP = g.My * g.Mx; p.dsy = 1; p.dsx = 1; p.dy0 = 0; p.dx0 = 0;
  p.scaleTargets = scaleTargets; p.relu = relu;
  const bool vec = g.N % 4 == 0 && g.F % 4 == 0 && aligned16(p.A) && aligned16(p.src) && aligned16(p.dst);
  const size_t dst_elems = (size_t)g.N * p.DP * g.F;
  const GGTimer tm{"conv_fprop", 2.0 * g.N * p.G * (double)g.F * p.K, 0.0};
  if (vec && gg_presplit_mode() && gg_producer_mode() &&
      gfc_try(images->data_device, filters->data_device, p.bias, targets->data_device, g.N, g.C, g.H, g.W, g.F, g.Ky, g.Kx, g.sy, g.sx, -g.py, -g.px,
              g.My, g.Mx, scaleTargets, relu, tm.flops))
    return;
  if (vec && gg_presplit_mode() && gg_producer_mode() && g.C % BK != 0 && g.F > 32 && CHIP_KNOB("CONVNET_GG_GK", 1) &&
      (size_t)g.C * g.H * g.W * g.N < (size_t(1) << 30)) {
    const int K = g.C * g.Ky * g.Kx, KP = divup(K, BK) * BK, TH = gg_tile_rows(g.F);
    void* planes = workspace_aux((size_t)96 * (KP / 16) * divup(g.F, TH) * TH);
    filter_planes_gk_launch(filters->data_device, planes, g.F, K, KP, TH, "conv_fprop");
    p.A = static_cast<const float*>(planes);
    p.apre = 1;
    p.gk = 1;
    p.ktab = gk_table(g.C, g.H, g.W, g.N, g.Ky, g.Kx);
    p.K = KP;
    p.KC = KP;
    gg_run<false>(p, vec, dst_elems, tm);
    note_kernel("gg_kernel(fprop)", tm.flops, p.row_tiles * p.col_tiles, p.splits);
    return;
  }
  if (vec && ggp_shape_ok(g.F, g.C) && gg_presplit_mode()) {
    p.KC = g.C;
    if (patch_shape_ok(p, dst_elems)) {
      const PatchBank bank{filters->data_device, g.F, g.C, g.Ky, g.Kx, 0, 0, 1, 1, g.Ky, g.Kx, false};
      patch_run(p, dst_elems, tm.op, tm.flops, bank);
      note_kernel(convnet_hip_get_patch_mode() >= 3 ? "gpw_kernel(fprop)" : "gpp_kernel(fprop)", tm.flops, p.row_tiles * p.col_tiles, p.splits);
      return;
    }
    p.KC = 0;
  }
  if (vec && ggp_shape_ok(g.F, g.C)) {
    const size_t welems = (size_t)g.F * p.K;
    if (gg_presplit_mode()) {
      const int TH = gg_tile_rows(g.F);
      void* planes = workspace_aux((size_t)96 * (g.C / 16) * p.TYX * divup(g.F, TH) * TH);
      const PatchBank bank{filters->data_device, g.F, g.C, g.Ky, g.Kx, 0, 0, 1, 1, g.Ky, g.Kx, false};
      filter_planes_rt_launch(bank, planes, p.TYX, TH, "conv_fprop");
      p.A = static_cast<const float*>(planes);
      p.apre = 1;
    } else if (p.TYX > 1) {
      float* wt = static_cast<float*>(workspace_aux(sizeof(float) * welems));
      int nb = (int)((welems + 255) / 256);
      if (nb > 2048) nb = 2048;
      const long long key[6] = {2, (long long)(uintptr_t)filters->data_device, (long long)(uintptr_t)wt, g.F, g.C, p.TYX};
      if (!filter_planes_shared(key, 6)) {
        KernelTimer timer("filter_tapmajor_kernel", "conv_fprop", 0.0, 8.0 * welems);
        hipLaunchKernelGGL(filter_tapmajor_kernel, dim3(nb), dim3(256), 0, stream(), filters->data_device, wt, g.F, g.C, p.TYX);
      }
      p.A = wt;
    }
    p.KC = g.C;
  }
  gg_run<false>(p, vec, dst_elems, tm);
  note_kernel("gg_kernel(fprop)", tm.flops, p.row_tiles * p.col_tiles, p.splits);
}

}
}

using namespace chip;

#ifdef CONVNET_GG_TRACE
extern "C" void convnet_hip_debug_set_gg_trace(unsigned long long* dev_buf) {
  CHIP_CHECK(hipMemcpyToSymbol(HIP_SYMBOL(chip::g_gg_trace), &dev_buf, sizeof dev_buf));
}
#endif

extern "C" {

static void conv_down_impl(cudamat* derivs, cudamat* filters, cudamat* targets, Shape4D* ds, Shape4D* fs, Shape4D* ts, const ConvDesc& d,
                           float scaleTargets, cudamat* mask, float post_scale);
static void launch_conv_up(PendingOp& o) {
  conv_up_impl(&o.m[0], &o.m[1], o.has_bias ? &o.bias : nullptr, &o.m[2], &o.s[0], &o.s[1], &o.s[2], o.desc, o.scaleTargets, o.relu);
}
static void launch_conv_down(PendingOp& o) {
  conv_down_impl(&o.m[0], &o.m[1], &o.m[2], &o.s[0], &o.s[1], &o.s[2], o.desc, o.scaleTargets, o.has_mask ? &o.mask : nullptr, 1.0f);
}
static bool park_conv(int kind, void (*launch)(PendingOp&), cudamat* a, cudamat* b, cudamat* c, Shape4D* sa, Shape4D* sb, Shape4D* sc, const ConvDesc& d,
                      float scaleTargets) {
  if (!defer_begin(kind, launch)) return false;
  if (kind == 1) (void)conv_geo(sa, sb, sc, d, a, b, c);
  else (void)conv_geo(sc, sb, sa, d, c, b, a);
  PendingOp& o = pending();
  o.m[0] = *a; o.m[1] = *b; o.m[2] = *c;
  o.s[0] = *sa; o.s[1] = *sb; o.s[2] = *sc;
  o.desc = d;
  o.scaleTargets = scaleTargets;
  return true;
}

void convUp(cudamat* images, cudamat* filters, cudamat* targets, Shape4D* is, Shape4D* fs, Shape4D* ts, ConvDesc d,
            float scaleTargets) {
  if (park_conv(1, launch_conv_up, images, filters, targets, is, fs, ts, d, scaleTargets)) return;
  conv_up_impl(images, filters, nullptr, targets, is, fs, ts, d, scaleTargets, 0);
}

void convUpGemm(cudamat* images, cudamat* filters, cudamat* targets, Shape4D* is, Shape4D* fs, Shape4D* ts, ConvDesc d,
                float scaleTargets) {
  convUp(images, filters, targets, is, fs, ts, d, scaleTargets);
}

void convUpBiasAct(cudamat* images, cudamat* filters, cudamat* bias, cudamat* targets, Shape4D* is, Shape4D* fs, Shape4D* ts,
                   ConvDesc d, float scaleTargets, int relu) {
  if (bias) CHIP_REQUIRE(bias->size[0] * bias->size[1] == d.num_output_channels);
  conv_up_impl(images, filters, bias, targets, is, fs, ts, d, scaleTargets, relu);
}

static void conv_down_impl(cudamat* derivs, cudamat* filters, cudamat* targets, Shape4D* ds, Shape4D* fs, Shape4D* ts, const ConvDesc& d,
                           float scaleTargets, cudamat* mask, float post_scale) {
  const ConvGeo g = conv_geo(ts, fs, ds, d, targets, filters, derivs);
  if (mask) CHIP_REQUIRE(numel(mask) == numel(targets));
  const size_t wt_floats = ((size_t)g.C * g.F * g.Ky * g.Kx + 64 * (size_t)g.sy * g.sx + 63) / 64 * 64;
  const int TH = gg_tile_rows(g.C);
  const size_t pl_floats = (size_t)24 * (g.F / 16 + 1) * g.Ky * g.Kx * divup(g.C, TH) * TH + 64 * (size_t)g.sy * g.sx;
  float* wt = static_cast<float*>(workspace_aux(sizeof(float) * (wt_floats + pl_floats)));
  size_t poff = 0;
  size_t woff = 0;
  double flops = 0;
  int blocks = 0;
  bool patched = false;
  GGParams base{};
  base.src = derivs->data_device; base.dst = targets->data_device; base.bias = nullptr;
  base.R = g.C; base.N = g.N; base.lda = g.C;
  base.SH = g.My; base.SW = g.Mx; base.ssy = 1; base.ssx = 1; base.dir = -1;
  base.DW = g.W; base.DP = g.H * g.W; base.dsy = g.sy; base.dsx = g.sx;
  base.scaleTargets = scaleTargets; base.relu = 0;
  base.mask = mask ? mask->data_device : nullptr; base.post_scale = post_scale;
  const bool vec = g.N % 4 == 0 && g.C % 4 == 0 && aligned16(base.src) && aligned16(base.dst) && aligned16(base.mask);
  GGClassTable ct{};
  const bool tapm = vec && ggp_shape_ok(g.C, g.F);
  if (tapm) base.KC = g.F;
  const bool pre = tapm && gg_presplit_mode();
  float* const planes = wt + wt_floats;
  if (pre) base.apre = 1;
  const bool multi = g.sy * g.sx > 1 && g.sy * g.sx <= kMaxClasses;
  const double alg_flops = 2.0 * g.N * (double)g.My * g.Mx * (double)g.F * g.C * g.Ky * g.Kx;
  struct StrideClass {
    int cy, cx, TYc, TXc, jy0, jx0, iy0, ix0, GY, GX;
  };
  std::vector<StrideClass> classes;
  double exec_total = 0;
  auto first_j = [](int cls, int pad, int s) {
    const int need = -pad - cls;
    return need > 0 ? (need + s - 1) / s : 0;
  };
  for (int cy = 0; cy < g.sy; ++cy)
    for (int cx = 0; cx < g.sx; ++cx) {
      StrideClass c{};
      c.cy = cy; c.cx = cx;
      c.TYc = cy < g.Ky ? divup(g.Ky - cy, g.sy) : 0;
      c.TXc = cx < g.Kx ? divup(g.Kx - cx, g.sx) : 0;
      c.jy0 = first_j(cy, g.py, g.sy); c.jx0 = first_j(cx, g.px, g.sx);
      c.iy0 = cy + g.py + g.sy * c.jy0; c.ix0 = cx + g.px + g.sx * c.jx0;
      if (c.iy0 >= g.H || c.ix0 >= g.W) continue;
      c.GY = (g.H - 1 - c.iy0) / g.sy + 1; c.GX = (g.W - 1 - c.ix0) / g.sx + 1;
      exec_total += 2.0 * g.N * (double)(c.GY * c.GX) * g.C * (double)(g.F * c.TYc * c.TXc);
      classes.push_back(c);
    }
  for (const StrideClass& c : classes) {
    const int cy = c.cy, cx = c.cx, TYc = c.TYc, TXc = c.TXc;
    float* wc = wt + woff;
    const size_t welems = (size_t)g.C * g.F * TYc * TXc;
    woff += (welems + 63) / 64 * 64;
    GGClass k{};
    k.A = wc; k.K = g.F * TYc * TXc;
    k.GX = c.GX; k.G = c.GY * c.GX; k.TX = TXc > 0 ? TXc : 1; k.TYX = TYc * TXc > 0 ? TYc * TXc : 1;
    k.y0 = c.jy0; k.x0 = c.jx0; k.dy0 = c.iy0; k.dx0 = c.ix0;
    const bool whole = g.sy == 1 && g.sx == 1 && c.GY == g.H && c.GX == g.W;
    const size_t dst_elems = whole ? (size_t)g.N * g.H * g.W * g.C : 0;
    const double cflops = 2.0 * g.N * k.G * (double)g.C * k.K;
    const GGTimer tm{"conv_dgrad", exec_total > 0 ? alg_flops * (cflops / exec_total) : 0.0, cflops};
    const PatchBank bank{filters->data_device, g.F, g.C, g.Ky, g.Kx, cy, cx, g.sy, g.sx, TYc, TXc, true};
    if (!multi && pre && welems > 0) {
      GGParams p = base;
      p.K = k.K; p.GX = c.GX; p.G = k.G; p.TX = TXc; p.TYX = TYc * TXc;
      p.y0 = k.y0; p.x0 = k.x0; p.dy0 = k.dy0; p.dx0 = k.dx0;
      if (patch_shape_ok(p, dst_elems)) {
        flops += cflops;
        patch_run(p, dst_elems, tm.op, tm.flops, bank);
        patched = true;
        blocks += p.row_tiles * p.col_tiles;
        continue;
      }
    }
    if (pre && welems > 0) {
      float* pc = planes + poff;
      poff += ((size_t)24 * (g.F / 16) * TYc * TXc * divup(g.C, TH) * TH + 63) / 64 * 64;
      filter_planes_rt_launch(bank, pc, TYc * TXc, TH, "conv_dgrad");
      k.A = pc;
    } else if (welems > 0) {
      int nb = (int)((welems + 255) / 256);
      if (nb > 2048) nb = 2048;
      (void)filter_planes_shared(nullptr, 0);
      KernelTimer timer("dgrad_filter_kernel", "conv_dgrad", 0.0, 8.0 * welems);
      hipLaunchKernelGGL(dgrad_filter_kernel, dim3(nb), dim3(256), 0, stream(), filters->data_device, wc, g.F, g.C, g.Ky,
                         g.Kx, cy, cx, g.sy, g.sx, TYc, TXc, tapm ? 1 : 0);
    }
    flops += cflops;
    if (multi) {
      ct.c[ct.n++] = k;
      continue;
    }
    GGParams p = base;
    p.A = k.A; p.K = k.K; p.GX = k.GX; p.G = k.G; p.TX = k.TX; p.TYX = k.TYX;
    p.y0 = k.y0; p.x0 = k.x0; p.dy0 = k.dy0; p.dx0 = k.dx0;
    gg_run<false>(p, vec, dst_elems, tm);
    blocks += p.row_tiles * p.col_tiles;
  }
  if (multi && ct.n > 0) {
    if (pre && patch_classes_ok(base, ct)) {
      patch_run_classes(base, ct, "conv_dgrad", alg_flops, flops);
      patched = true;
    } else {
      gg_run_classes(base, ct, vec, GGTimer{"conv_dgrad", alg_flops, flops});
    }
    blocks = ct.c[ct.n - 1].tile_end;
  }
  note_kernel(!patched ? "gg_kernel(dgrad)" : convnet_hip_get_patch_mode() >= 3 ? "gpw_kernel(dgrad)" : "gpp_kernel(dgrad)", alg_flops, blocks, 1);
}

void convDown(cudamat* derivs, cudamat* filters, cudamat* targets, Shape4D* ds, Shape4D* fs, Shape4D* ts, ConvDesc d,
              float scaleTargets) {
  if (park_conv(2, launch_conv_down, derivs, filters, targets, ds, fs, ts, d, scaleTargets)) return;
  conv_down_impl(derivs, filters, targets, ds, fs, ts, d, scaleTargets, nullptr, 1.0f);
}

void convDownGemm(cudamat* derivs, cudamat* filters, cudamat* targets, Shape4D* ds, Shape4D* fs, Shape4D* ts, ConvDesc d,
                  float scaleTargets) {
  convDown(derivs, filters, targets, ds, fs, ts, d, scaleTargets);
}

void convDownMask(cudamat* derivs, cudamat* filters, cudamat* state, cudamat* targets, Shape4D* ds, Shape4D* fs, Shape4D* ts, ConvDesc d,
                  float scaleTargets, float post_scale) {
  conv_down_impl(derivs, filters, targets, ds, fs, ts, d, scaleTargets, state, post_scale);
}

static void conv_outp_impl(cudamat* images, cudamat* derivs, cudamat* targets, cudamat* bias_grad, Shape4D* is, Shape4D* ds, Shape4D* ts,
                           const ConvDesc& d, float scaleTargets, float scaleOutput) {
  const ConvGeo g = conv_geo(is, ts, ds, d, images, targets, derivs);
  WGParams p{};
  if (bias_grad) {
    CHIP_REQUIRE(bias_grad->on_device && (size_t)numel(bias_grad) == (size_t)g.F);
    p.bias_dst = bias_grad->data_device;
  }
  p.src = images->data_device; p.dout = derivs->data_device; p.dst = targets->data_device;
  p.K = g.C * g.Ky * g.Kx; p.F = g.F; p.N = g.N;
  p.GX = g.Mx; p.M = g.My * g.Mx; p.TX = g.Kx; p.TYX = g.Ky * g.Kx; p.SH = g.H; p.SW = g.W;
  p.ssy = g.sy; p.ssx = g.sx; p.y0 = g.py; p.x0 = g.px;
  p.nchunk = divup(g.N, WG_NB); p.chunks_total = p.M * p.nchunk;
  p.scaleTargets = scaleTargets; p.scaleOutput = scaleOutput;
  const bool vec = g.N % 4 == 0 && aligned16(p.src) && aligned16(p.dout);
  const GGTimer tm{"conv_wgrad", 2.0 * g.N * p.M * (double)g.F * p.K, 0.0};
  wg_launch(p, vec, tm);
  note_kernel("wg_kernel(wgrad)", tm.flops, p.k_tiles * p.f_tiles, p.splits);
  if (bias_grad && !p.bias_dst) {
    cudamat view = *derivs;
    view.size[0] = g.N * p.M;
    view.size[1] = g.F;
    view.is_trans = 0;
    view.owns_data = 0;
    CHIP_REQUIRE(sum_by_axis(&view, bias_grad, 0, scaleOutput, wg_batch_active() && wg_batch_frame() > 1 ? 1.f : scaleTargets) == 0);
  }
}

void convOutpGemm(cudamat* images, cudamat* derivs, cudamat* targets, Shape4D* is, Shape4D* ds, Shape4D* ts, ConvDesc d,
                  float scaleTargets, float scaleOutput) {
  conv_outp_impl(images, derivs, targets, nullptr, is, ds, ts, d, scaleTargets, scaleOutput);
}

void convOutpBias(cudamat* images, cudamat* derivs, cudamat* targets, cudamat* bias_grad, Shape4D* is, Shape4D* ds, Shape4D* ts,
                  ConvDesc d, float scaleTargets, float scaleOutput) {
  conv_outp_impl(images, derivs, targets, bias_grad, is, ds, ts, d, scaleTargets, scaleOutput);
}

void convOutp(cudamat* images, cudamat* derivs, cudamat* targets, Shape4D* is, Shape4D* ds, Shape4D* ts, ConvDesc d,
              int , int , float scaleTargets, float scaleOutput) {
  convOutpGemm(images, derivs, targets, is, ds, ts, d, scaleTargets, scaleOutput);
}

static int dot_impl(cudamat* mat1, cudamat* mat2, cudamat* bias, cudamat* target, float beta, float alpha, int relu, cudamat* mask,
                    float post_scale) {
  if (!mat1->on_device || !mat2->on_device || !target->on_device) return ERROR_NOT_ON_DEVICE;
  const int t1 = mat1->is_trans, t2 = mat2->is_trans;
  const int m = t1 ? mat1->size[1] : mat1->size[0], k1 = t1 ? mat1->size[0] : mat1->size[1];
  const int k2 = t2 ? mat2->size[1] : mat2->size[0], n = t2 ? mat2->size[0] : mat2->size[1];
  if (m != target->size[0] || n != target->size[1] || k1 != k2) return ERROR_INCOMPATIBLE_DIMENSIONS;
  if (target->is_trans) return ERROR_TRANSPOSED;
  const int K = k1;
  if ((t1 && t2) || (!t1 && alpha != 1.0f)) {
    if (bias || relu || mask) return ERROR_UNSUPPORTED;
    if (m == 0 || n == 0) return 0;
    KernelTimer timer("dot_generic_kernel", "dot_generic", 2.0 * m * (double)n * K, 0.0);
    hipLaunchKernelGGL(dot_generic_kernel, dim3(divup(m, 32), divup(n, 32)), dim3(256), 0, stream(), mat1->data_device, mat2->data_device,
                       target->data_device, m, n, K, mat1->size[0], mat2->size[0], t1, t2, beta, alpha);
    return launch_status();
  }
  if (!t1) {
    GGParams p{};
    p.src = mat1->data_device; p.dst = target->data_device; p.bias = bias ? bias->data_device : nullptr;
    p.A = mat2->data_device;
    p.R = n; p.K = K; p.N = m; p.lda = mat2->size[0];
    p.GX = 1; p.G = 1; p.TX = 1; p.TYX = 1; p.SH = 1; p.SW = 1; p.ssy = 1; p.ssx = 1; p.y0 = 0; p.x0 = 0; p.dir = 1;
    p.DW = 1; p.DP = 1; p.dsy = 1; p.dsx = 1; p.dy0 = 0; p.dx0 = 0;
    p.scaleTargets = beta; p.relu = relu;
    if (mask && numel(mask) != numel(target)) return ERROR_INCOMPATIBLE_DIMENSIONS;
    p.mask = mask ? mask->data_device : nullptr; p.post_scale = post_scale;
    const bool base_vec = m % 4 == 0 && aligned16(p.src) && aligned16(p.dst) && aligned16(p.A) && aligned16(p.mask);
    const GGTimer tm{t2 ? "fc_fprop" : "fc_dgrad", 2.0 * m * (double)n * K, 0.0};
    p.skinny = m <= 128 && n > 64 && !CHIP_DIAG_KNOB("CONVNET_GG_NO_SKINNY", 0);
    if (t2) {
      const bool v = base_vec && n % 4 == 0;
      if (v && !p.skinny && ggp_shape_ok(n, K)) p.KC = K;
      gg_run<false>(p, v, (size_t)m * n, tm);
    } else {
      gg_run<true>(p, base_vec && K % 4 == 0 && mat2->size[0] % 4 == 0, (size_t)m * n, tm);
    }
    note_kernel(t2 ? "gg_kernel(fc NT)" : "gg_kernel(fc NN)", tm.flops, p.row_tiles * p.col_tiles, p.splits);
    return launch_status();
  }
  if (t1 && !t2) {
    if (bias || relu || mask) return ERROR_UNSUPPORTED;
    WGParams p{};
    p.src = mat2->data_device; p.dout = mat1->data_device; p.dst = target->data_device;
    p.K = n; p.F = m; p.N = K;
    p.GX = 1; p.M = 1; p.TX = 1; p.TYX = 1; p.SH = 1; p.SW = 1; p.ssy = 1; p.ssx = 1; p.y0 = 0; p.x0 = 0;
    p.nchunk = divup(K, WG_NB); p.chunks_total = p.nchunk;
    p.scaleTargets = beta; p.scaleOutput = alpha;
    const bool vec = K % 4 == 0 && aligned16(p.src) && aligned16(p.dout);
    const GGTimer tm{"fc_wgrad", 2.0 * m * (double)n * K, 0.0};
    wg_launch(p, vec, tm);
    note_kernel("wg_kernel(fc TN)", tm.flops, p.k_tiles * p.f_tiles, p.splits);
    return launch_status();
  }
  return ERROR_UNSUPPORTED;
}

int dotBiasAct(cudamat* mat1, cudamat* mat2, cudamat* bias, cudamat* target, float beta, float alpha, int relu) {
  return dot_impl(mat1, mat2, bias, target, beta, alpha, relu, nullptr, 1.0f);
}

int dotMask(cudamat* mat1, cudamat* mat2, cudamat* state, cudamat* target, float beta, float alpha, float post_scale) {
  return dot_impl(mat1, mat2, nullptr, target, beta, alpha, 0, state, post_scale);
// ... 8 lines not shown
```

convnet_amd/csrc/patch_gemm.hip:

```cpp
#include <algorithm>
#include <cmath>
#include <cstdlib>
#include <string>

#include "gather_gemm.h"

#ifndef CONVNET_GPV_LDS_MAP
#define CONVNET_GPV_LDS_MAP 0
#endif
#ifndef CONVNET_GPV_FILT_LATE
#define CONVNET_GPV_FILT_LATE 1
#endif

namespace chip {

__global__ void __launch_bounds__(256) act_planes_kernel(const float* __restrict__ src, u32x4* __restrict__ out, int CB, int HW, int N4) {
  const size_t total = (size_t)CB * 2 * HW * N4;
  const size_t cstride = (size_t)HW * N4 * 4;
  const int IB = N4 / 16;
  for (size_t i = (size_t)blockIdx.x * blockDim.x + threadIdx.x; i < total; i += (size_t)gridDim.x * blockDim.x) {
    const int n4 = (int)(i % N4);
    size_t r = i / N4;
    const int pix = (int)(r % HW);
    r /= HW;
    const int lh = (int)(r & 1), cb = (int)(r >> 1);
    const float* sp = src + ((size_t)(16 * cb + lh) * HW + pix) * (size_t)(N4 * 4) + 4 * n4;
    f32x4 v[8];
#pragma unroll
    for (int j = 0; j < 8; ++j) v[j] = ld4(sp + 2 * j * cstride);
    u32x4* o = out + ((((size_t)cb * HW + pix) * IB + (n4 >> 4)) * 6 + lh) * 64 + 4 * (n4 & 15);
#pragma unroll
    for (int e = 0; e < 4; ++e) {
      float x[8];
#pragma unroll
      for (int j = 0; j < 8; ++j) x[j] = v[j][e];
      Split8 s;
      split8_sat(x, s);
      o[e] = s.h;
      o[128 + e] = s.m;
      o[256 + e] = s.l;
    }
  }
}

__global__ void filter_planes_rt_kernel(const float* __restrict__ W, u32x4* __restrict__ out, int F, int C, int TYX, int TH) {
  const int RT = (F + TH - 1) / TH;
  const size_t total = (size_t)(C / 16) * TYX * 2 * RT * TH;
  for (size_t i = (size_t)blockIdx.x * blockDim.x + threadIdx.x; i < total; i += (size_t)gridDim.x * blockDim.x) {
    const int f = (int)(i % (RT * TH));
    const size_t r = i / (RT * TH);
    const int lh = (int)(r & 1);
    const size_t chunk = r >> 1;
    const int tap = (int)(chunk % TYX), cb = (int)(chunk / TYX);
    Split8 sp = {};
    if (f < F) {
      float x[8];
#pragma unroll
      for (int j = 0; j < 8; ++j) x[j] = W[(size_t)f + (size_t)F * (tap + (size_t)TYX * (16 * cb + 2 * j + lh))];
      split8_sat(x, sp);
    }
    u32x4* o = out + ((chunk * RT + f / TH) * 6 + lh) * TH + f % TH;
    o[0] = sp.h;
    o[2 * TH] = sp.m;
    o[4 * TH] = sp.l;
  }
}
__global__ void dgrad_filter_planes_rt_kernel(const float* __restrict__ W, u32x4* __restrict__ out, int F, int C, int Ky, int Kx, int cy, int cx,
                                              int sy, int sx, int TYc, int TXc, int TH) {
  const int TYXc = TYc * TXc, RT = (C + TH - 1) / TH;
  const size_t total = (size_t)(F / 16) * TYXc * 2 * RT * TH;
  for (size_t i = (size_t)blockIdx.x * blockDim.x + threadIdx.x; i < total; i += (size_t)gridDim.x * blockDim.x) {
    const int c = (int)(i % (RT * TH));
    const size_t r = i / (RT * TH);
    const int lh = (int)(r & 1);
    const size_t chunk = r >> 1;
    const int tap = (int)(chunk % TYXc), fb = (int)(chunk / TYXc);
    const int a = tap / TXc, b = tap - a * TXc;
    Split8 sp = {};
    if (c < C) {
      const float* wp = W + (size_t)F * ((cx + sx * b) + Kx * ((cy + sy * a) + (size_t)Ky * c)) + 16 * fb + lh;
      float x[8];
#pragma unroll
      for (int j = 0; j < 8; ++j) x[j] = wp[2 * j];
      split8_sat(x, sp);
    }
    u32x4* o = out + ((chunk * RT + c / TH) * 6 + lh) * TH + c % TH;
    o[0] = sp.h;
    o[2 * TH] = sp.m;
    o[4 * TH] = sp.l;
  }
}

__global__ void filter_planes_gk_kernel(const float* __restrict__ W, u32x4* __restrict__ out, int F, int K, int KP, int TH) {
  const int RT = (F + TH - 1) / TH;
  const size_t total = (size_t)(KP / 16) * 2 * RT * TH;
  for (size_t i = (size_t)blockIdx.x * blockDim.x + threadIdx.x; i < total; i += (size_t)gridDim.x * blockDim.x) {
    const int f = (int)(i % (RT * TH));
    const size_t r = i / (RT * TH);
    const int lh = (int)(r & 1);
    const size_t chunk = r >> 1;
    float x[8];
#pragma unroll
    for (int j = 0; j < 8; ++j) {
      const int k = 16 * (int)chunk + 2 * j + lh;
      x[j] = (f < F && k < K) ? W[(size_t)f + (size_t)F * k] : 0.f;
    }
    Split8 sp;
    split8_sat(x, sp);
    u32x4* o = out + ((chunk * RT + f / TH) * 6 + lh) * TH + f % TH;
    o[0] = sp.h;
    o[2 * TH] = sp.m;
    o[4 * TH] = sp.l;
  }
}
namespace {
bool g_share_on = false;
int g_share_n = 0;
long long g_share_key[20];
}
void filter_planes_share(bool on) {
  g_share_on = on;
  g_share_n = 0;
}
bool filter_planes_shared(const long long* key, int n) {
  if (!g_share_on) return false;
  bool same = n == g_share_n;
  for (int i = 0; same && i < n; ++i) same = key[i] == g_share_key[i];
  g_share_n = n;
  for (int i = 0; i < n; ++i) g_share_key[i] = key[i];
  return same;
}

void filter_planes_gk_launch(const float* W, void* out, int F, int K, int KP, int TH, const char* op) {
  const long long key[7] = {0, (long long)(uintptr_t)W, (long long)(uintptr_t)out, F, K, KP, TH};
  if (filter_planes_shared(key, 7)) return;
  const size_t work = (size_t)(KP / 16) * 2 * divup(F, TH) * TH;
  int nb = (int)((work + 255) / 256);
  if (nb > 2048) nb = 2048;
  KernelTimer timer("filter_planes_kernel", op, 0.0, 10.0 * (double)F * K);
  hipLaunchKernelGGL(filter_planes_gk_kernel, dim3(nb), dim3(256), 0, stream(), W, static_cast<u32x4*>(out), F, K, KP, TH);
}

void filter_planes_rt_launch(const PatchBank& b, void* out, int TYX, int TH, const char* op) {
  const long long key[17] = {1, (long long)(uintptr_t)b.W, (long long)(uintptr_t)out, b.F, b.C, b.Ky, b.Kx, b.cy, b.cx, b.sy, b.sx, b.TYc, b.TXc,
                             b.dgrad, TYX, TH, 0};
  if (filter_planes_shared(key, 17)) return;
  const int R = b.dgrad ? b.C : b.F, KCn = b.dgrad ? b.F : b.C;
  const size_t work = (size_t)(KCn / 16) * TYX * 2 * divup(R, TH) * TH;
  int nb = (int)((work + 255) / 256);
  if (nb > 2048) nb = 2048;
  KernelTimer timer(b.dgrad ? "dgrad_filter_planes_kernel" : "filter_planes_kernel", op, 0.0, 10.0 * (double)R * KCn * TYX);
  if (b.dgrad)
    hipLaunchKernelGGL(dgrad_filter_planes_rt_kernel, dim3(nb), dim3(256), 0, stream(), b.W, static_cast<u32x4*>(out), b.F, b.C, b.Ky, b.Kx, b.cy,
                       b.cx, b.sy, b.sx, b.TYc, b.TXc, TH);
  else
    hipLaunchKernelGGL(filter_planes_rt_kernel, dim3(nb), dim3(256), 0, stream(), b.W, static_cast<u32x4*>(out), b.F, b.C, TYX, TH);
}

__device__ __forceinline__ int slot_pos(int img) { return (img & 48) | ((img + (img >> 4)) & 15); }
__device__ __forceinline__ int slot_img(int pos) { return (pos & 48) | ((pos - (pos >> 4)) & 15); }

template <int WR, int WC, int MT, int CW, bool BRAW>
__global__ __launch_bounds__(WR* WC * 64 + 64, 2) void gpp_kernel(const GGParams pin, const GGClassTable ct) {
  constexpr int NC = WR * WC * 64;
  constexpr int NTC = CW / 32;
  using fvec = __attribute__((ext_vector_type(NTC))) float;
  constexpr int ROWS = WR * MT * 32;
  constexpr int A_STAGE = 6 * ROWS * 4;
  constexpr int STA = 3;
  constexpr int NS = 8;
  constexpr int PS = BRAW ? 4 : 6;
  constexpr int SLAB = PS * NS * 256;
  constexpr int NA = A_STAGE / 4 / 64;
  constexpr int NBP = PS * NS;
  constexpr int UW = CW / 64;
  static_assert(WC * UW == kPatchP && NTC == 4, "tile = kPatchP units of 64 images; slot_pos is the NTC = 4 swizzle");
  static_assert(NA + NBP < 64 && NA % 2 == 0, "vmcnt immediate; batch sizes are even");
  extern __shared__ __attribute__((aligned(16))) float smem[];
  float* As = smem;
  float* Bs = smem + STA * A_STAGE;

  const GGParams& p = pin;
  GGTile T;
  if (!gg_select_tile(p, ct, T)) return;
  const int L = T.L, tsplit = T.tsplit;
  const int row_tile = L % p.row_tiles, col_tile = L / p.row_tiles;
  const int split = blockIdx.y;
  const int tid = threadIdx.x;
  const int wave = __builtin_amdgcn_readfirstlane(tid >> 6), lane = tid & 63;
  const int r0 = row_tile * ROWS;
  const int N = p.N;

  const int G = T.G, GX = T.GX, units = p.IB * G;
  int u_ib[kPatchP], u_oy[kPatchP], u_ox[kPatchP], S[kPatchP];
  bool u_ok[kPatchP];
  int ys_f = 1 << 30, ys_l = -(1 << 30);
#pragma unroll
  for (int j = 0; j < kPatchP; ++j) {
    const int U = col_tile * kPatchP + j;
    u_ok[j] = U < units;
    const int ib = u_ok[j] ? U / G : 0, m = u_ok[j] ? U - ib * G : 0;
    u_ib[j] = ib;
    u_oy[j] = m / GX;
    u_ox[j] = m - u_oy[j] * GX;
    if (u_ok[j]) {
      const int ys0 = u_oy[j] * p.ssy + T.y0;
      ys_f = min(ys_f, ys0);
      ys_l = max(ys_l, ys0);
    }
    S[j] = j == 0 ? 0 : S[j - 1] + (!u_ok[j] ? 0 : (u_ib[j] == u_ib[j - 1] && u_oy[j] == u_oy[j - 1]) ? 1 : 3);
  }

  const int TX = T.TX, TYX = T.TYX, TYn = TYX / TX;
  const int ng = p.ng, gc0 = p.gcnt[0], gc1 = p.gcnt[1], gbase0 = p.gb0[0], gbase1 = p.gb0[1];
  int a_lo = 0, a_hi = TYn - 1;
  const bool skip = tsplit < 0 && p.splits == 1;
  if (skip) {
    if (p.dir > 0) { a_lo = max(0, -ys_l); a_hi = min(TYn - 1, p.SH - 1 - ys_f); }
    else { a_lo = max(0, ys_f - (p.SH - 1)); a_hi = min(TYn - 1, ys_l); }
  }
  const int nrow = max(0, a_hi - a_lo + 1);
  const int nsc_all = (p.KC / BK) * nrow * ng;
  int sc_beg = 0, sc_end = nsc_all;
  if (!skip) {
    const int cps = tsplit >= 0 ? p.tail_cps : p.chunks_per_split;
    sc_beg = min(nsc_all, (tsplit >= 0 ? tsplit : split) * cps);
    sc_end = min(nsc_all, sc_beg + cps);
  }
  const int nsc = sc_end - sc_beg;
  int nchunks;
  if (ng == 1) nchunks = nsc * gc0;
  else {
    const int n1 = (sc_end >> 1) - (sc_beg >> 1);
    nchunks = (nsc - n1) * gc0 + n1 * gc1;
  }


  if (wave == WR * WC) {
    __builtin_amdgcn_s_setprio(3);
    if (nchunks == 0) {
      __builtin_amdgcn_s_barrier();
      return;
    }
    const char* const planes = reinterpret_cast<const char*>(p.planes);
    const unsigned lane_off = (unsigned)slot_img(lane) * 16u;
    const size_t ch_bytes = (size_t)p.SH * p.SW * N * 4;
    const size_t lane_off_raw = (size_t)(lane >> 4) * ch_bytes + (size_t)(lane & 15) * 16;
    const char* const rawsrc = reinterpret_cast<const char*>(p.src);
    const int dir = p.dir, SH = p.SH, SW = p.SW, ssy = p.ssy, ssx = p.ssx;
#ifdef CONVNET_DIAG
    const int diag = p.prio;
#else
    constexpr int diag = 0;
#endif
    const unsigned a_lane = (unsigned)lane * 16u;
    const char* const abase0 = reinterpret_cast<const char*>(T.A) + (size_t)row_tile * (6 * ROWS * 16);
    const size_t a_chunk_bytes = (size_t)p.row_tiles * (6 * ROWS * 16);

    int A_cb, A_a, A_g, A_i, A_left = nchunks;
    {
      A_g = sc_beg % ng;
      const int r = sc_beg / ng;
      A_a = a_lo + (nrow > 0 ? r % nrow : 0);
      A_cb = nrow > 0 ? r / nrow : 0;
      A_i = 0;
    }
    auto issue_a = [&](int stage) __attribute__((always_inline)) {
      const int b = (A_g ? gbase1 : gbase0) + A_i * dir * ssx;
      const char* abase = abase0 + a_chunk_bytes * (size_t)(A_cb * TYX + A_a * TX + b);
      const unsigned lda0 = lds_addr(As + stage * A_STAGE);
#pragma unroll
      for (int it = 0; it < NA; it += 4) {
        lds_dma4(a_lane, abase, abase, abase, abase, lda0 + 1024u * it);
        abase += 4096;
      }
      --A_left;
      if (++A_i == (A_g ? gc1 : gc0)) {
        A_i = 0;
        if (++A_g == ng) {
          A_g = 0;
          if (++A_a > a_hi) {
            A_a = a_lo;
            ++A_cb;
          }
        }
      }
    };

    int B_cb, B_a, B_g;
    {
      B_g = sc_beg % ng;
      const int r = sc_beg / ng;
      B_a = a_lo + (nrow > 0 ? r % nrow : 0);
      B_cb = nrow > 0 ? r / nrow : 0;
    }
    constexpr unsigned kNoSlot = 0xFFFFFFFFu;
    constexpr unsigned kZeroSlot = 0xFFFFFFFEu;
    const int IBn = p.IB;
    auto slot_desc = [&]() __attribute__((always_inline)) {
      const int s = lane & (NS - 1);
      const int cnt = B_g ? gc1 : gc0, b0 = B_g ? gbase1 : gbase0;
      unsigned off = kNoSlot;
#pragma unroll
      for (int j = 0; j < kPatchP; ++j) {
        const int i = s - S[j];
        if (u_ok[j] && i >= 0 && i < cnt) {
          const int ys = u_oy[j] * ssy + T.y0 + dir * B_a;
          const int xs = u_ox[j] * ssx + T.x0 + dir * b0 + i * ssx;
          const bool in = (unsigned)ys < (unsigned)SH && (unsigned)xs < (unsigned)SW;
// ... 1172 lines not shown
        load_a(stage, fan);
        mac_step(K1{}, fa, fc, NTC - 1);
        split_pair(0, 0, fn);
        mac_step(K2{}, fa, fc, NTC - 1);
        split_pair(0, 1, fn);
        mac_step(K3{}, fa, fc, NTC - 1);
        split_pair(0, 2, fn);
        mac_step(K4{}, fa, fc, NTC - 1);
        split_pair(0, 3, fn);
        mac_step(K5{}, fa, fc, NTC - 1);
        CHIP_PIN_SPLIT8(fn);
        __builtin_amdgcn_sched_barrier(0);
      }
    };
    auto run = [&](Split8 (&fa)[MT], Split8 (&fan)[MT]) __attribute__((always_inline)) { chunk(fa, fan); };
    load_a(0, fa0);
    read_b();
#pragma unroll
    for (int q = 0; q < 4; ++q) split_pair(0, q, fb[0]);
    int c = 0;
    if (nchunks & 1) {
      run(fa0, fa1);
      c = 1;
    } else {
#pragma unroll
      for (int t = 0; t < MT; ++t) fa1[t] = fa0[t];
    }
    for (; c < nchunks; c += 2) {
      run(fa1, fa0);
      run(fa0, fa1);
    }
    __builtin_amdgcn_s_waitcnt(0x0070);
  }

  acc_settle();
  if (tsplit >= 0) {
    float* pp = p.tail_partial + ((size_t)(L - p.tail_first) * p.tail_splits + tsplit) * (size_t)(ROWS * WC * CW);
#pragma unroll
    for (int t = 0; t < MT; ++t)
#pragma unroll
      for (int reg = 0; reg < 16; ++reg) {
        fvec v;
#pragma unroll
        for (int u = 0; u < NTC; ++u) v[u] = acc_elem<true>(acc[t][u][reg]);
        *reinterpret_cast<fvec*>(pp + ((size_t)(t * 16 + reg) * NC + tid) * NTC) = v;
      }
    return;
  }
  gg_epilogue<1, WC, MT, CW, true, true>(p, acc, row_tile, col_tile, split, T.ncols, T.GX, T.G, T.dy0, T.dx0);
}

namespace {

int g_patch_mode = -1;
inline int patch_mode() {
  if (g_patch_mode < 0) g_patch_mode = CHIP_KNOB("CONVNET_GG_PATCH", 3);
  return g_patch_mode;
}

template <typename Kern>
int patch_slots(Kern kern, int threads, size_t lds) {
  CHIP_CHECK(hipFuncSetAttribute(reinterpret_cast<const void*>(kern), hipFuncAttributeMaxDynamicSharedMemorySize, (int)lds));
  int n = 0;
  CHIP_CHECK(hipOccupancyMaxActiveBlocksPerMultiprocessor(&n, reinterpret_cast<const void*>(kern), threads, lds));
#ifdef CONVNET_EMU
  if (const char* e = getenv("CONVNET_EMU_SLOTS")) return atoi(e);
#endif
  return (n < 1 ? 1 : n) * 256;
}

struct WidePlan {
  int splits;
  bool take;
};
inline int wide_rows(int R) { return R > 64 && R <= 96 ? 96 : 128; }
inline bool wide_is_var(const GGParams& p) { return !(p.ng == 1 && p.gcnt[0] == 3 && wide_rows(p.R) == 128); }
inline WidePlan wide_plan(const GGParams& p, size_t dst_elems, int slots) {
  const int CB = p.KC / BK, TYn = p.TYX / p.TX, rows = wide_rows(p.R);
  const int tiles = divup(p.R, rows) * divup((p.N / 64) * p.G, kWideP);
  const int nsc = CB * TYn * p.ng, kchunks = CB * p.TYX;
  const double block_rate = 230e12 / slots;
  const double fl = 2.0 * rows * (double)(kWideP * 64) * (double)p.K;
  auto finish = [&](int sp) {
    const int cps = divup(nsc, sp);
    return divup(nsc, cps);
  };
  if (tiles <= slots) {
    int best_sp = 1;
    double best_t = 1e30;
    for (int sp = 1; sp <= 16 && tiles * sp <= slots && (sp == 1 || (dst_elems > 0 && kchunks / sp >= 8 && nsc / sp >= 1)); ++sp) {
      const double t = gg_split_time(tiles, sp, slots, fl, block_rate, dst_elems);
      if (t < best_t * 0.97) {
        best_t = t;
        best_sp = sp;
      }
    }
    const int sp = finish(best_sp);
    const double fill = (double)tiles * sp / slots;
    if (fill >= (wide_is_var(p) ? 0.85 : sp > 1 ? 0.60 : 0.75)) return {sp, true};
  }
  const int splits = finish(gg_split_k(tiles, slots, fl, block_rate, dst_elems, kchunks, nsc));
  const long long blocks = (long long)tiles * splits;
  const long long rounds = (blocks + slots - 1) / slots;
  const bool fill = (double)blocks >= 0.85 * (double)(rounds * slots) || (splits == 1 && rounds >= 4);
  return {splits, fill && (splits == 1 || rounds == 1)};
}
constexpr size_t wide_lds(int rows) { return sizeof(float) * (3 * (6 * rows * 4) + 2 * (kWideNS * 1024) + 1024); }
constexpr size_t kWideLds = wide_lds(128);
inline int wide_slots(int rows = 128, bool var = false) {
  static const int n = patch_slots(gpw_kernel, 256, kWideLds);
  if (!var) return n;
  static const int n4 = patch_slots(gpv_kernel<4>, 256, wide_lds(128)), n3 = patch_slots(gpv_kernel<3>, 256, wide_lds(96));
  return rows == 96 ? n3 : n4;
}

}

bool patch_shape_ok(GGParams& p, size_t dst_elems) {
  if (!patch_mode() || matrix_path() == 0 || p.KC <= 0 || p.KC % BK != 0) return false;
  if (p.N % 64 != 0 || p.GX < 4 || p.R <= 64) return false;
  if ((size_t)p.SH * p.SW * p.N >= (size_t(1) << 28)) return false;
  if (p.ssx < 1 || p.ssx > 2 || (p.dir < 0 && p.ssx != 1)) return false;
  p.ng = p.ssx;
  for (int r = 0; r < p.ng; ++r) {
    const int cnt = p.TX > r ? (p.TX - r + p.ssx - 1) / p.ssx : 0;
    if (cnt < 2 || cnt > 3) return false;
    p.gcnt[r] = cnt;
    p.gb0[r] = p.dir > 0 ? r : r + (cnt - 1) * p.ssx;
  }
  if (p.ng == 1) { p.gcnt[1] = p.gcnt[0]; p.gb0[1] = p.gb0[0]; }
  if (patch_mode() >= 3) {
    if (p.GX < kWideP) return false;
    return patch_mode() == 4 || wide_plan(p, dst_elems, wide_slots(wide_rows(p.R), wide_is_var(p))).take;
  }
  return true;
}

void patch_run(GGParams& p, size_t dst_elems, const char* op, double flops, const PatchBank& bank) {
  constexpr int WR = 2, WC = 2, MT = 2, CW = 128;
  static_assert(128 == WR * MT * 32, "row tile");
  const int mode = patch_mode();
  const bool wide = mode >= 3, braw = mode != 2;
  const bool var = wide && wide_is_var(p);
  const int ROWS = wide ? wide_rows(p.R) : 128;
  const int PU = wide ? kWideP : kPatchP;
  const int TCOLS = PU * 64;
  const int threads = wide ? 256 : WR * WC * 64 + 64;
  const int C = p.KC, HW = p.SH * p.SW, N = p.N, CB = C / BK;
  const size_t elems = (size_t)C * HW * N;
  const int RT = divup(p.R, ROWS);
  {
    const size_t welems = (size_t)CB * p.TYX * RT * ROWS * 16;
    u32x4* ap = static_cast<u32x4*>(workspace_aux(welems * 6 + (CHIP_DIAG_KNOB("CONVNET_GPP_DIAG", 0) ? 65536 : 0)));
    filter_planes_rt_launch(bank, ap, p.TYX, ROWS, op);
    p.A = reinterpret_cast<const float*>(ap);
    p.apre = 1;
  }
  u32x4* planes = nullptr;
  if (!braw) {
    planes = static_cast<u32x4*>(workspace_planes(elems * 6));
    KernelTimer timer("act_planes_kernel", op, 0.0, 10.0 * elems);
    const size_t work = (size_t)CB * 2 * HW * (N / 4);
    size_t nb = (work + 255) / 256;
    if (nb > 16384) nb = 16384;
    hipLaunchKernelGGL(act_planes_kernel, dim3((unsigned)nb), dim3(256), 0, stream(), p.src, planes, CB, HW, N / 4);
  }
  p.patch = 1;
  p.IB = N / 64;
  p.planes = planes;
  p.NP = N;
  p.ncols = 0;
  p.row_tiles = RT;
  p.col_tiles = divup(p.IB * p.G, PU);
  p.zero = zero_page();
  p.prio = CHIP_DIAG_KNOB("CONVNET_GPP_DIAG", 0);
  constexpr size_t lds_p = sizeof(float) * (3 * (6 * 128 * 4) + 2 * (6 * 8 * 256)), lds_r = sizeof(float) * (3 * (6 * 128 * 4) + 2 * (4 * 8 * 256));
  const size_t lds_w = wide_lds(ROWS);
  static const int slots_p = patch_slots(gpp_kernel<WR, WC, MT, CW, false>, WR * WC * 64 + 64, lds_p);
  static const int slots_r = patch_slots(gpp_kernel<WR, WC, MT, CW, true>, WR * WC * 64 + 64, lds_r);
  const int slots = wide ? wide_slots(ROWS, var) : braw ? slots_r : slots_p;
  const int tiles = p.row_tiles * p.col_tiles;
  const int TYn = p.TYX / p.TX;
  const int nsc = CB * TYn * p.ng;
  const int kchunks = CB * p.TYX;
  const double block_rate = 230e12 / slots;
  const double fl = 2.0 * ROWS * (double)TCOLS * (double)p.K;
  int splits = wide ? wide_plan(p, dst_elems, slots).splits : gg_split_k(tiles, slots, fl, block_rate, dst_elems, kchunks, nsc);
  p.chunks_per_split = divup(nsc, splits);
  splits = divup(nsc, p.chunks_per_split);
  p.splits = splits;
  p.slab = dst_elems;
  p.partial = splits > 1 ? static_cast<float*>(workspace(sizeof(float) * dst_elems * splits)) : nullptr;
  p.tail_splits = 1;
  p.tail_partial = nullptr;
  if (splits == 1 && dst_elems > 0 && gg_partial_last_round(tiles, slots, kchunks)) {
    int best_s = gg_tail_split(tiles, slots, fl, block_rate, ROWS * TCOLS, kchunks);
#ifdef CONVNET_EMU
    if (const char* e = getenv("CONVNET_EMU_TAIL")) best_s = atoi(e);
#endif
    if (best_s > 1) gg_set_tail(p, tiles, slots, nsc, best_s, ROWS * TCOLS);
  }
  dim3 grid(p.tail_splits > 1 ? 8 * (p.tail_tf8 + p.tail_tt8) : ((tiles + 7) / 8) * 8, splits);
  static const GGClassTable kNone = {};
  {
    KernelTimer timer(var ? (ROWS == 96 ? "gpv_kernel<96x512,split,raw>" : "gpv_kernel<128x512,split,raw>")
                      : wide ? "gpw_kernel<128x512,split,raw>" : braw ? "gpp_kernel<2,2,2,128,split,raw>" : "gpp_kernel<2,2,2,128,split,planes>", op, flops, 0.0, 0.0);
    if (var && ROWS == 96) hipLaunchKernelGGL(gpv_kernel<3>, grid, dim3(threads), lds_w, stream(), p, kNone);
    else if (var) hipLaunchKernelGGL(gpv_kernel<4>, grid, dim3(threads), lds_w, stream(), p, kNone);
    else if (wide) hipLaunchKernelGGL(gpw_kernel, grid, dim3(threads), lds_w, stream(), p, kNone);
    else if (braw) hipLaunchKernelGGL((gpp_kernel<WR, WC, MT, CW, true>), grid, dim3(threads), lds_r, stream(), p, kNone);
    else hipLaunchKernelGGL((gpp_kernel<WR, WC, MT, CW, false>), grid, dim3(threads), lds_p, stream(), p, kNone);
  }
  if (p.tail_splits > 1) {
    const int rem = tiles - p.tail_first;
    KernelTimer timer("gg_tail_fix_kernel", op, 0.0, sizeof(float) * (double)rem * (p.tail_splits + 1) * ROWS * TCOLS);
    if (wide && ROWS == 96) hipLaunchKernelGGL(gpw_tail_fix_kernel<3>, dim3(rem * kTailFixParts), dim3(256), 0, stream(), p);
    else if (wide) hipLaunchKernelGGL(gpw_tail_fix_kernel<4>, dim3(rem * kTailFixParts), dim3(256), 0, stream(), p);
    else hipLaunchKernelGGL((gg_tail_fix_kernel<WR, WC, MT, CW, true>), dim3(rem * kTailFixParts), dim3(WR * WC * 64), 0, stream(), p);
  }
  if (splits > 1) gg_reduce_launch(p, dst_elems, splits, op);
}

bool patch_classes_ok(const GGParams& base, const GGClassTable& ct) {
  if (patch_mode() < 4 || matrix_path() == 0 || !base.apre || base.KC <= 0 || base.KC % BK != 0) return false;
  if (base.N % 64 != 0 || base.R <= 64 || base.dir >= 0 || base.ssx != 1 || base.ssy != 1) return false;
  if ((size_t)base.SH * base.SW * base.N >= (size_t(1) << 28)) return false;
  if (ct.n < 1) return false;
  for (int i = 0; i < ct.n; ++i)
    if (ct.c[i].TX < 2 || ct.c[i].TX > 3 || ct.c[i].GX < kWideP || ct.c[i].TYX % ct.c[i].TX != 0) return false;
  return true;
}
void patch_run_classes(GGParams& p, GGClassTable& ct, const char* op, double flops, double exec) {
  const int ROWS = wide_rows(p.R);
  p.patch = 1;
  p.IB = p.N / 64;
  p.planes = nullptr;
  p.NP = p.N;
  p.ncols = 0;
  p.row_tiles = divup(p.R, ROWS);
  p.zero = zero_page();
  p.prio = CHIP_DIAG_KNOB("CONVNET_GPP_DIAG", 0);
  p.splits = 1;
  p.chunks_per_split = 1 << 24;
  p.partial = nullptr;
  p.slab = 0;
  p.tail_splits = 1;
  p.tail_partial = nullptr;
  p.ng = 1;
  std::sort(ct.c, ct.c + ct.n, [](const GGClass& a, const GGClass& b) { return a.K > b.K; });
  int end = 0;
  for (int i = 0; i < ct.n; ++i) {
    ct.c[i].ncols = 0;
    ct.c[i].col_tiles = divup(p.IB * ct.c[i].G, kWideP);
    end += p.row_tiles * ct.c[i].col_tiles;
    ct.c[i].tile_end = end;
  }
  p.col_tiles = ct.c[0].col_tiles;
  wide_slots(ROWS, true);
  KernelTimer timer(ROWS == 96 ? "gpv_kernel<96x512,split,raw>" : "gpv_kernel<128x512,split,raw>", op, flops, 0.0, exec);
  if (ROWS == 96) hipLaunchKernelGGL(gpv_kernel<3>, dim3(end), dim3(256), wide_lds(96), stream(), p, ct);
  else hipLaunchKernelGGL(gpv_kernel<4>, dim3(end), dim3(256), wide_lds(128), stream(), p, ct);
}

}

extern "C" {
void convnet_hip_set_patch_mode(int mode) { chip::g_patch_mode = mode < 0 ? 0 : mode > 4 ? 4 : mode; }
int convnet_hip_get_patch_mode(void) { return chip::patch_mode(); }
}
```

convnet_amd/csrc/state.hip:

```cpp
#include <cstdio>
#include <cstring>
#include <map>
#include <string>
#include <vector>

#include "common.h"

namespace chip {
namespace {
hipStream_t g_stream = nullptr;
std::string g_last_error;
ConvnetHipKernelInfo g_info = {"none", 0.0, 0, 1};
}

namespace {
int g_defer = -1;
PendingOp g_pending = {};
bool g_flushing = false;
inline bool defer_on() {
  if (g_defer < 0) g_defer = env_int("CONVNET_DEFER_EPILOGUES", 0) != 0 ? 1 : 0;
  return g_defer != 0;
}
}
long g_absorbed = 0;
PendingOp& pending() { return g_pending; }
void flush_pending() {
  if (g_pending.kind == 0 || g_flushing) return;
  PendingOp o = g_pending;
  g_pending.kind = 0;
  g_flushing = true;
  o.launch(o);
  g_flushing = false;
}
bool defer_begin(int kind, void (*launch)(PendingOp&)) {
  if (!defer_on() || g_flushing) return false;
  flush_pending();
  g_pending = PendingOp{};
  g_pending.kind = kind;
  g_pending.launch = launch;
  return true;
}

hipStream_t stream() {
  flush_pending();
  return g_stream;
}

int g_matrix_path = -1;
int matrix_path() {
  if (g_matrix_path < 0) {
    const char* e = getenv("CONVNET_GG_SPLIT");
    g_matrix_path = (e && *e) ? (atoi(e) != 0 ? 1 : 0) : 0;
  }
  return g_matrix_path;
}

namespace {
struct Arena {
  void* p = nullptr;
  size_t cap = 0;
};
std::map<hipStream_t, Arena> g_arena[5];

void* arena_get(int which, size_t bytes, size_t slack) {
  flush_pending();
  Arena& a = g_arena[which][g_stream];
  if (bytes <= a.cap) return a.p;
  CHIP_CHECK(hipStreamSynchronize(stream()));
  if (a.p) CHIP_CHECK(hipFree(a.p));
  a.cap = ((bytes + slack) >> 20) << 20;
  CHIP_CHECK(hipMalloc(&a.p, a.cap));
  return a.p;
}
}

void* workspace(size_t bytes) { return arena_get(0, bytes, size_t(1) << 22); }

void* workspace_aux(size_t bytes) { return arena_get(1, bytes, size_t(1) << 20); }
void* workspace_planes(size_t bytes) { return arena_get(2, bytes, size_t(1) << 22); }
void* workspace_banks(size_t bytes) { return arena_get(3, bytes, size_t(1) << 20); }
void* workspace_slabs(size_t bytes) { return arena_get(4, bytes, size_t(1) << 20); }

const float* zero_page() {
  static float* z = nullptr;
  if (!z) {
    CHIP_CHECK(hipMalloc((void**)&z, 256));
    CHIP_CHECK(hipMemset(z, 0, 256));
    const float ones[4] = {1.f, 1.f, 1.f, 1.f};
    CHIP_CHECK(hipMemcpy(z + 32, ones, sizeof ones, hipMemcpyHostToDevice));
  }
  return z;
}

void set_last_error(const char* msg) { g_last_error = msg ? msg : ""; }

void note_kernel(const char* name, double flops, int blocks, int split_k) {
  g_info.name = name;
  g_info.flops = flops;
  g_info.grid_blocks = blocks;
  g_info.split_k = split_k;
}

namespace {
struct ProfRec {
  std::string name, op;
  double flops, bytes, executed;
  hipEvent_t start, stop;
};
bool g_prof_on = false;
std::vector<ProfRec> g_prof;
std::vector<hipEvent_t> g_event_pool;
hipEvent_t get_event() {
  if (!g_event_pool.empty()) {
    hipEvent_t e = g_event_pool.back();
    g_event_pool.pop_back();
    return e;
  }
  hipEvent_t e;
  CHIP_CHECK(hipEventCreate(&e));
  return e;
}
}

KernelTimer::KernelTimer(const char* name, const char* op, double flops, double bytes, double executed) : slot(-1) {
  if (!g_prof_on) return;
  ProfRec r{name, op, flops, bytes, executed > 0.0 ? executed : flops, get_event(), get_event()};
  CHIP_CHECK(hipEventRecord(r.start, stream()));
  g_prof.push_back(r);
  slot = (int)g_prof.size() - 1;
}
KernelTimer::~KernelTimer() {
  if (slot >= 0) CHIP_CHECK(hipEventRecord(g_prof[slot].stop, stream()));
}

__global__ void transpose_kernel(const float* __restrict__ src, float* __restrict__ dst, int rows, int cols) {
  __shared__ float tile[32][33];
  const int bx = blockIdx.x * 32, by = blockIdx.y * 32;
  const int tx = threadIdx.x & 31, ty = threadIdx.x >> 5;
  for (int j = ty; j < 32; j += 8) {
    const int r = bx + tx, c = by + j;
    if (r < rows && c < cols) tile[j][tx] = src[(size_t)r + (size_t)rows * c];
  }
  __syncthreads();
  for (int j = ty; j < 32; j += 8) {
    const int c = by + tx, r = bx + j;
    if (r < rows && c < cols) dst[(size_t)c + (size_t)cols * r] = tile[tx][j];
  }
}

}

using namespace chip;

extern "C" {

int convnet_hip_init(int device_id) {
  if (hipSetDevice(device_id) != hipSuccess) return CUDA_ERROR;
  return 0;
}

void convnet_hip_shutdown(void) {
  flush_pending();
  hipDeviceSynchronize();
  for (auto& per_stream : g_arena) {
    for (auto& kv : per_stream)
      if (kv.second.p) hipFree(kv.second.p);
    per_stream.clear();
  }
}

void convnet_hip_set_stream(void* s) {
  flush_pending();
  g_stream = (hipStream_t)s;
}
void convnet_hip_set_deferred_epilogues(int on) {
  flush_pending();
  g_defer = on != 0 ? 1 : 0;
}
int convnet_hip_get_deferred_epilogues(void) { return defer_on() ? 1 : 0; }
long convnet_hip_deferred_absorbed(void) { return chip::g_absorbed; }
void* convnet_hip_get_stream(void) {
  flush_pending();
  return (void*)g_stream;
}

int convnet_hip_reserve_workspace(size_t bytes) {
  workspace(bytes);
  return 0;
}

const char* convnet_hip_version(void) { return "convnet_hip 0.2 (gfx950; fp32 products via bf16-split or fp32 MFMA)"; }
void convnet_hip_set_matrix_path(int path) { chip::g_matrix_path = path != 0 ? 1 : 0; }
int convnet_hip_get_matrix_path(void) { return chip::matrix_path(); }
const char* get_last_cuda_error(void) {
  flush_pending();
  return g_last_error.c_str();
}

int cuda_set_device(int deviceId) {
  flush_pending();
  return hipSetDevice(deviceId) == hipSuccess ? 0 : CUDA_ERROR;
}

void cuda_sync_threads(void) { CHIP_CHECK(hipStreamSynchronize(stream())); }

static int event_status(hipError_t err) {
  if (err != hipSuccess) {
    set_last_error(hipGetErrorString(err));
    printf("%s\n", hipGetErrorString(err));
  }
  return err != hipSuccess;
}
int cuda_create_event(void** t) { return event_status(hipEventCreateWithFlags(reinterpret_cast<hipEvent_t*>(t), hipEventDisableTiming)); }
int cuda_record_event(void** t) { return event_status(hipEventRecord(*reinterpret_cast<hipEvent_t*>(t), stream())); }
int cuda_synchronize_event(void** t) { return event_status(hipStreamWaitEvent(stream(), *reinterpret_cast<hipEvent_t*>(t), 0)); }
int destroy_tex(cudamat* mat) {
  if (mat) mat->tex_obj = 0;
  return 0;
}
int cublas_init(void) { return 0; }
int cublas_shutdown(void) {
  convnet_hip_shutdown();
  return 0;
}

void convnet_hip_last_kernel_info(ConvnetHipKernelInfo* out) {
  flush_pending();
  *out = g_info;
}

void convnet_hip_profile_enable(int on) { g_prof_on = on != 0; }

size_t convnet_hip_profile_report(char* buf, size_t cap) {
  if (g_prof.empty()) return 0;
  hipStreamSynchronize(stream());
  struct Agg { long n = 0; double ms = 0, flops = 0, bytes = 0, executed = 0; };
  std::map<std::string, Agg> agg;
  for (auto& r : g_prof) {
    float ms = 0.f;
    hipEventElapsedTime(&ms, r.start, r.stop);
    Agg& a = agg[r.name + "|" + r.op];
    a.n++; a.ms += ms; a.flops += r.flops; a.bytes += r.bytes; a.executed += r.executed;
    g_event_pool.push_back(r.start);
    g_event_pool.push_back(r.stop);
  }
  g_prof.clear();
  std::string out;
  char line[512];
  for (auto& kv : agg) {
    snprintf(line, sizeof line, "%s|%ld|%.6f|%.6e|%.6e|%.6e\n", kv.first.c_str(), kv.second.n, kv.second.ms, kv.second.flops, kv.second.bytes,
             kv.second.executed);
    out += line;
  }
  if (out.size() + 1 > cap) return 0;
  memcpy(buf, out.c_str(), out.size() + 1);
  return out.size();
}

int allocate_device_memory(cudamat* mat) {
  const size_t bytes = numel(mat) * sizeof(float);
  if (hipMalloc((void**)&mat->data_device, bytes ? bytes : 4) != hipSuccess) {
    set_last_error("hipMalloc failed");
    return CUDA_ERROR;
  }
  mat->on_device = 1;
  return 0;
}

int free_device_memory(cudamat* mat) {
  flush_pending();
  if (mat->owns_data && mat->on_device) {
    if (hipFree(mat->data_device) != hipSuccess) return CUDA_ERROR;
    mat->on_device = 0;
    mat->data_device = nullptr;
  }
  return 0;
}

int copy_to_host(cudamat* mat) {
  if (!mat->on_device) return ERROR_NOT_ON_DEVICE;
  const size_t bytes = numel(mat) * sizeof(float);
  if (hipMemcpyAsync(mat->data_host, mat->data_device, bytes, hipMemcpyDeviceToHost, stream()) != hipSuccess) return CUDA_ERROR;
  if (hipStreamSynchronize(stream()) != hipSuccess) return CUDA_ERROR;
  mat->on_host = 1;
  return 0;
}

int copy_to_device(cudamat* mat) {
  if (!mat->on_device) {
    int rc = allocate_device_memory(mat);
    if (rc) return rc;
  }
  const size_t bytes = numel(mat) * sizeof(float);
  if (hipMemcpyAsync(mat->data_device, mat->data_host, bytes, hipMemcpyHostToDevice, stream()) != hipSuccess) return CUDA_ERROR;
  if (hipStreamSynchronize(stream()) != hipSuccess) return CUDA_ERROR;
  return 0;
}

int copy_to_host_slice(cudamat* mat, size_t start, size_t end) {
  if (!mat->on_device) return ERROR_NOT_ON_DEVICE;
  if (end > (size_t)mat->size[1] || start > end) return ERROR_INCOMPATIBLE_DIMENSIONS;
  const size_t off = start * mat->size[0], bytes = (end - start) * mat->size[0] * sizeof(float);
  if (hipMemcpyAsync(mat->data_host + off, mat->data_device + off, bytes, hipMemcpyDeviceToHost, stream()) != hipSuccess) return CUDA_ERROR;
  return hipStreamSynchronize(stream()) == hipSuccess ? 0 : CUDA_ERROR;
}

int copy_to_device_slice(cudamat* mat, size_t start, size_t end) {
  if (end <= start || end > (size_t)mat->size[1]) return ERROR_GENERIC;
  if (!mat->on_device) {
    const int rc = allocate_device_memory(mat);
    if (rc) return rc;
  }
  const size_t off = start * mat->size[0], bytes = (end - start) * mat->size[0] * sizeof(float);
  if (hipMemcpyAsync(mat->data_device + off, mat->data_host + off, bytes, hipMemcpyHostToDevice, stream()) != hipSuccess) return CUDA_ERROR;
  return hipStreamSynchronize(stream()) == hipSuccess ? 0 : CUDA_ERROR;
}

int copy_on_device(cudamat* mat1, cudamat* mat2) {
  if (mat1->size[0] != mat2->size[0] || mat1->size[1] != mat2->size[1]) return ERROR_INCOMPATIBLE_DIMENSIONS;
  if (hipMemcpyAsync(mat2->data_device, mat1->data_device, numel(mat1) * sizeof(float), hipMemcpyDeviceToDevice, stream()) != hipSuccess) return CUDA_ERROR;
  return 0;
}

int copy_transpose(cudamat* source, cudamat* target) {
  if (source->size[0] != target->size[1] || source->size[1] != target->size[0]) return ERROR_INCOMPATIBLE_DIMENSIONS;
  const int rows = source->size[0], cols = source->size[1];
  dim3 grid(divup(rows, 32), divup(cols, 32));
  hipLaunchKernelGGL(transpose_kernel, grid, dim3(256), 0, stream(), source->data_device, target->data_device, rows, cols);
  return launch_status();
}

int reshape(cudamat* mat, int m, int n) {
  if (m < 0 && n < 0) return ERROR_GENERIC;
  const long long total = (long long)mat->size[0] * mat->size[1];
  if (m < 0) m = (int)(total / n);
  if (n < 0) n = (int)(total / m);
  if (total != (long long)m * n) return ERROR_INCOMPATIBLE_DIMENSIONS;
  mat->size[0] = m;
  mat->size[1] = n;
  return 0;
}

int get_slice(cudamat* source, cudamat* target, unsigned int first_col, unsigned int last_col) {
  if (source->is_trans) return ERROR_TRANSPOSED;
  if (!source->on_device) return ERROR_NOT_ON_DEVICE;
  if (last_col > (unsigned)source->size[1] || first_col >= last_col) return ERROR_INCOMPATIBLE_DIMENSIONS;
  const size_t rows = source->size[0];
  target->data_host = source->data_host ? source->data_host + first_col * rows : nullptr;
  target->data_device = source->data_device + first_col * rows;
  target->on_device = 1;
  target->on_host = 0;
  target->size[0] = source->size[0];
  target->size[1] = last_col - first_col;
// ... 50 lines not shown
```

include/convnet_hip.h:

```cpp
#ifndef CONVNET_HIP_H_
#define CONVNET_HIP_H_

#include <stdbool.h>
#include <stddef.h>

#ifdef __cplusplus
extern "C" {
#endif

#define ERROR_INCOMPATIBLE_DIMENSIONS -1
#define CUBLAS_ERROR -2
#define CUDA_ERROR -3
#define VIEW_ERROR -4
#define ERROR_TRANSPOSED -5
#define ERROR_GENERIC -6
#define ERROR_TRANSPOSEDNESS -7
#define ERROR_NOT_ON_DEVICE -8
#define ERROR_UNSUPPORTED -9

typedef struct cudamat {
  float* data_host;
  float* data_device;
  int on_device;
  int on_host;
  int size[2];
  int is_trans;
  int owns_data;
  unsigned long long tex_obj;
} cudamat;
typedef cudamat hipmat;

typedef struct Shape4D {
  int shape[4];
} Shape4D;

typedef struct ConvDesc {
  int num_input_channels;
  int num_output_channels;
  int kernel_size_y;
  int kernel_size_x;
  int kernel_size_t;
  int stride_y;
  int stride_x;
  int stride_t;
  int padding_y;
  int padding_x;
  int padding_t;
  int input_channel_begin;
  int input_channel_end;
  int output_channel_begin;
  int output_channel_end;
  int num_groups;
} ConvDesc;

int convnet_hip_init(int device_id);
void convnet_hip_shutdown(void);
void convnet_hip_set_stream(void* hip_stream);
void* convnet_hip_get_stream(void);
int convnet_hip_reserve_workspace(size_t bytes);
const char* convnet_hip_version(void);
void convnet_hip_set_matrix_path(int path);
int convnet_hip_get_matrix_path(void);
void convnet_hip_set_patch_mode(int mode);
int convnet_hip_get_patch_mode(void);
void convnet_hip_set_wgrad_tile(int mode);
int convnet_hip_get_wgrad_tile(void);
void convnet_hip_set_deferred_epilogues(int on);
int convnet_hip_get_deferred_epilogues(void);
long convnet_hip_deferred_absorbed(void);
const char* get_last_cuda_error(void);
int cuda_set_device(int deviceId);
void cuda_sync_threads(void);
int cuda_create_event(void** t);
int cuda_record_event(void** t);
int cuda_synchronize_event(void** t);
int cublas_init(void);
int cublas_shutdown(void);
int destroy_tex(cudamat* mat);

int allocate_device_memory(cudamat* mat);
int free_device_memory(cudamat* mat);
int copy_to_host(cudamat* mat);
int copy_to_device(cudamat* mat);
int copy_to_host_slice(cudamat* mat, size_t start, size_t end);
int copy_to_device_slice(cudamat* mat, size_t start, size_t end);
int copy_on_device(cudamat* mat1, cudamat* mat2);
int copy_transpose(cudamat* source, cudamat* target);
int reshape(cudamat* mat, int m, int n);
int get_slice(cudamat* source, cudamat* target, unsigned int first_col, unsigned int last_col);
void init_from_array(cudamat* mat, float* data, int m, int n);
int init_empty(cudamat* mat, int m, int n);
int write_at(cudamat* mat, int row, int col, float val);
float read_from(cudamat* mat, int row, int col, int* err_code);

int extract_patches(cudamat* images, cudamat* patches, cudamat* width_offset, cudamat* height_offset, cudamat* flip,
                    int img_width, int img_height, int patch_width, int patch_height);
int stage_patches_u8(void* chunk, int dims, int num_cases, cudamat* case_index, cudamat* mean, cudamat* std, cudamat* patches,
                     cudamat* width_offset, cudamat* height_offset, cudamat* flip, int img_width, int img_height, int patch_width,
                     int patch_height);
int chunk_moments_u8(void* chunk, int dims, int num_cases, int first_case, int cases, int num_colors, void* acc);
int stage_clips_u8(void* frames, int frame_dims, int num_frames, cudamat* first_frame, int clip_frames, cudamat* mean, cudamat* std,
                   cudamat* patches, cudamat* width_offset, cudamat* height_offset, cudamat* flip, int img_width, int img_height,
                   int patch_width, int patch_height);
void convnet_hip_set_stage_clips_grid(int mode);
int stage_images_u8(void* bytes, size_t num_bytes, void* image_table, int num_images, void* taps, int num_taps, void* case_table,
                    cudamat* mean, cudamat* std, cudamat* patches, cudamat* width_offset, cudamat* height_offset, cudamat* flip,
                    int img_width, int img_height, int patch_width, int patch_height);
int crop_images_u8(void* bytes, size_t num_bytes, void* image_table, int num_images, void* taps, int num_taps, void* case_table,
                   int num_cases, void* rows, int img_width, int img_height);
int feature_rows(cudamat* state, cudamat* sum, int pass, int passes, int cases, cudamat* carry, int consumed, int group, cudamat* rows);
int shuffleColumns(cudamat* source, cudamat* rand_perm_indices);
int add_col_vec(cudamat* mat, cudamat* vec, cudamat* target);
int add_col_mult(cudamat* mat, cudamat* vec, cudamat* target, float mult);
int div_by_col_vec(cudamat* mat, cudamat* vec, cudamat* target);
int mult_by_row_vec(cudamat* mat, cudamat* vec, cudamat* target);
int div_by_row_vec(cudamat* mat, cudamat* vec, cudamat* target);
int add_to_each_pixel(cudamat* mat1, cudamat* mat2, cudamat* target, float mult);
int normalize_by_axis(cudamat* mat, cudamat* target, int axis);

void convUpGemm(cudamat* images, cudamat* filters, cudamat* targets,
                Shape4D* images_shape, Shape4D* filters_shape,
                Shape4D* targets_shape, ConvDesc conv_desc,
                float scaleTargets);
void convDownGemm(cudamat* derivs, cudamat* filters, cudamat* targets,
                  Shape4D* derivs_shape, Shape4D* filters_shape,
                  Shape4D* targets_shape, ConvDesc conv_desc,
                  float scaleTargets);
void convOutpGemm(cudamat* images, cudamat* derivs, cudamat* targets,
                  Shape4D* images_shape, Shape4D* derivs_shape,
                  Shape4D* targets_shape, ConvDesc conv_desc,
                  float scaleTargets, float scaleOutput);
void convUp(cudamat* images, cudamat* filters, cudamat* targets,
            Shape4D* images_shape, Shape4D* filters_shape, Shape4D* targets_shape,
            ConvDesc conv_desc, float scaleTargets);
void convDown(cudamat* derivs, cudamat* filters, cudamat* targets,
              Shape4D* derivs_shape, Shape4D* filters_shape, Shape4D* targets_shape,
              ConvDesc conv_desc, float scaleTargets);
void convOutp(cudamat* images, cudamat* derivs, cudamat* targets,
              Shape4D* images_shape, Shape4D* derivs_shape, Shape4D* targets_shape,
              ConvDesc conv_desc, int partialSumY, int partialSumX, float scaleTargets,
              float scaleOutput);

void localUp(cudamat* images, cudamat* filters, cudamat* targets,
             Shape4D* images_shape, Shape4D* filters_shape, Shape4D* targets_shape,
             ConvDesc conv_desc, float scaleTargets);
void localDown(cudamat* derivs, cudamat* filters, cudamat* targets,
               Shape4D* derivs_shape, Shape4D* filters_shape, Shape4D* targets_shape,
               ConvDesc conv_desc, float scaleTargets);
void localOutp(cudamat* images, cudamat* derivs, cudamat* targets,
               Shape4D* images_shape, Shape4D* derivs_shape, Shape4D* targets_shape,
               ConvDesc conv_desc, float scaleTargets, float scaleOutput);
void localUpGemm(cudamat* images, cudamat* filters, cudamat* targets,
                Shape4D* images_shape, Shape4D* filters_shape,
                Shape4D* targets_shape, ConvDesc conv_desc,
                float scaleTargets);
void localDownGemm(cudamat* derivs, cudamat* filters, cudamat* targets,
                  Shape4D* derivs_shape, Shape4D* filters_shape,
                  Shape4D* targets_shape, ConvDesc conv_desc,
                  float scaleTargets);
void localOutpGemm(cudamat* images, cudamat* derivs, cudamat* targets,
                  Shape4D* images_shape, Shape4D* derivs_shape,
                  Shape4D* targets_shape, ConvDesc conv_desc,
                  float scaleTargets, float scaleOutput);
void localUpBiasAct(cudamat* images, cudamat* filters, cudamat* bias, cudamat* targets,
                    Shape4D* images_shape, Shape4D* filters_shape, Shape4D* targets_shape,
                    ConvDesc conv_desc, float scaleTargets, int relu);

void convUp3DGemm(cudamat* images, cudamat* filters, cudamat* targets,
                  Shape4D* images_shape, Shape4D* filters_shape,
                  Shape4D* targets_shape, ConvDesc conv_desc,
                  float scaleTargets);
void convDown3DGemm(cudamat* derivs, cudamat* filters, cudamat* targets,
                    Shape4D* derivs_shape, Shape4D* filters_shape,
                    Shape4D* targets_shape, ConvDesc conv_desc,
                    float scaleTargets);
void convOutp3DGemm(cudamat* images, cudamat* derivs, cudamat* targets,
                    Shape4D* images_shape, Shape4D* derivs_shape,
                    Shape4D* targets_shape, ConvDesc conv_desc,
                    float scaleTargets, float scaleOutput);
void ResponseNormCrossMap3DGemm(cudamat* images, cudamat* targets, int numFilters, int sizeF, float addScale,
                                float powScale, bool blocked, int image_size_t);
void ResponseNormCrossMap3DUndoGemm(cudamat* outGrads, cudamat* inputs, cudamat* targets,
                                    int numFilters, int sizeF, float addScale, float powScale, bool blocked,
                                    int image_size_t);
void convUp3DBiasAct(cudamat* images, cudamat* filters, cudamat* bias, cudamat* targets,
                     Shape4D* images_shape, Shape4D* filters_shape, Shape4D* targets_shape,
                     ConvDesc conv_desc, float scaleTargets, int relu);
void convDown3DMask(cudamat* derivs, cudamat* filters, cudamat* state, cudamat* targets,
                    Shape4D* derivs_shape, Shape4D* filters_shape, Shape4D* targets_shape,
                    ConvDesc conv_desc, float scaleTargets, float post_scale);
void convOutp3DBias(cudamat* images, cudamat* derivs, cudamat* targets, cudamat* bias_grad,
                    Shape4D* images_shape, Shape4D* derivs_shape, Shape4D* targets_shape,
                    ConvDesc conv_desc, float scaleTargets, float scaleOutput);
void ResponseNormCrossMap3DRelu(cudamat* images, cudamat* targets, int numFilters, int sizeF, float addScale,
                                float powScale, bool blocked, int image_size_t);

void MaxPoolGemm(cudamat* images, cudamat* targets, Shape4D* images_shape,
                 Shape4D* targets_shape, ConvDesc conv_desc, float scaleTargets,
                 float scaleOutput);
void MaxPoolUndoGemm(cudamat* images, cudamat* maxGrads, cudamat* maxActs,
                     cudamat* targets, Shape4D* images_shape,
                     Shape4D* maxGrads_shape, ConvDesc conv_desc,
                     float scaleTargets);
void AvgPoolGemm(cudamat* images, cudamat* targets, Shape4D* images_shape,
                 Shape4D* targets_shape, ConvDesc conv_desc, float scaleTargets,
                 float scaleOutput);
void AvgPoolUndoGemm(cudamat* avgGrads, cudamat* targets,
                     Shape4D* avgGrads_shape, Shape4D* targets_shape,
                     ConvDesc conv_desc, float scaleTargets);
void MaxPool(cudamat* images, cudamat* targets, Shape4D* images_shape,
             Shape4D* targets_shape, ConvDesc conv_desc);
void AvgPool(cudamat* images, cudamat* targets, Shape4D* images_shape,
             Shape4D* targets_shape, ConvDesc conv_desc);
void MaxPoolUndo(cudamat* images, cudamat* maxGrads, cudamat* maxActs,
                 cudamat* targets, Shape4D* images_shape, Shape4D* maxGrads_shape,
                 ConvDesc conv_desc, float scaleTargets);
void AvgPoolUndo(cudamat* avgGrads, cudamat* targets, Shape4D* avgGrads_shape,
                 Shape4D* targets_shape, ConvDesc conv_desc, float scaleTargets);

void ResponseNormCrossMapGemm(cudamat* images, cudamat* targets, int numFilters, int sizeF,
                              float addScale, float powScale, bool blocked);
void ResponseNormCrossMapUndoGemm(cudamat* outGrads, cudamat* inputs, cudamat* targets,
// ... 140 lines not shown
```

Before: 28060.

## Batch per-step filter plane builds into one table launched at step start

Adds a per-training-step plane table. At step begin, all filter split-plane conversions recorded in the previous step (fprop, dgrad, gfc forms) are built together into a dedicated arena, and later conv calls look up the prebuilt planes instead of launching their own conversion kernels. The table is dropped whenever weights are updated, so stale planes are never used. The intent is to cut many small conversion kernel launches and the reconversion of the same weights for fprop and dgrad, at the cost of extra workspace and bookkeeping.

```diff
diff --git a/convnet_amd/_lib.py b/convnet_amd/_lib.py
--- a/convnet_amd/_lib.py
+++ b/convnet_amd/_lib.py
@@ -45,6 +45,13 @@
 
 class KernelInfo(ctypes.Structure):
     _fields_ = [("name", ctypes.c_char_p), ("flops", ctypes.c_double), ("grid_blocks", ctypes.c_int), ("split_k", ctypes.c_int)]
+
+
+PLANES_MAX = 16
+
+
+class PlaneRequest(ctypes.Structure):
+    _fields_ = [("bank", ctypes.c_void_p), ("form", ctypes.c_int), ("geo", ctypes.c_int * 13)]
 
 
 _CTYPES = {
diff --git a/convnet_amd/build.py b/convnet_amd/build.py
--- a/convnet_amd/build.py
+++ b/convnet_amd/build.py
@@ -25,7 +25,7 @@
     os.makedirs(os.path.join(HERE, "lib"), exist_ok=True)
     objdir = os.path.join(HERE, "lib", "obj")
     os.makedirs(objdir, exist_ok=True)
-    headers = [os.path.join(SRC, "common.h"), os.path.join(SRC, "gather_gemm.h"), os.path.join(SRC, "wgrad_wide_schedule.h"),
+    headers = [os.path.join(SRC, "common.h"), os.path.join(SRC, "gather_gemm.h"), os.path.join(SRC, "wgrad_wide_schedule.h"), os.path.join(SRC, "plane_forms.h"),
                os.path.join(HERE, "..", "include", "convnet_hip.h")]
     objs, procs = [], []
     for s in SOURCES:
diff --git a/convnet_amd/convnet.py b/convnet_amd/convnet.py
--- a/convnet_amd/convnet.py
+++ b/convnet_amd/convnet.py
@@ -8,9 +8,13 @@
 from . import pbtxt
 from .edge import AvgPoolEdge, ConvEdge, Edge, EdgeWithWeight, FCEdge, LocalEdge, MaxPoolEdge, ResponseNormEdge
 from .layer import Layer, LinearLayer, LogisticLayer, ReLULayer, SoftmaxDistLayer, SoftmaxLayer
+from ._lib import PLANES_MAX, PlaneRequest, lib
 from .matrix import Matrix
 from .optimizer import RunFusedSteps
 from .trainer import TrainLoopMixin
+
+
+_planes_begin, _planes_end = getattr(lib, "convnet_hip_planes_begin", None), getattr(lib, "convnet_hip_planes_end", None)
 
 
 class LayerPlan(NamedTuple):
@@ -83,6 +87,9 @@
         self.correct_accum_ = None
         self._logits_pending = set()
         self._bn_steps = []
+        self.plane_table_ = True
+        self._plane_requests = (PlaneRequest * PLANES_MAX)()
+        self._plane_count = 0
         self.BuildNet()
         if exchange is not None and any(l.UseBatchNormalization() for l in self.layers_):
             raise SystemExit("batch_normalize is not supported with a gradient exchange (data-parallel training)")
@@ -151,6 +158,10 @@
     def PlanLayers(self):
         self.plan_ = {l: self._plan_layer(l) for l in self.layers_}
         self.metric_on_device_ = len(self.output_layers_) == 1 and self.plan_[self.output_layers_[0]].output_entry is not None
+        convs = [e for e in self.edges_ if isinstance(e, ConvEdge)]
+        self.plane_table_ok_ = bool(self.fused and convs and _planes_begin is not None and all(
+            not e.IsTied() and e.image_size_t_ == 1 and not e.weight_optimizer_.NeedsSecondHistory() for e in convs))
+        self._plane_count = 0
 
     def _fused_down_scale(self, l):
         return self.plan_[l].down_scale
@@ -523,15 +534,21 @@
         if (self.overlap_update_ or self.overlap_wgrad_) and self.side_stream_ is None and torch.cuda.is_available():
             self.side_stream_ = Matrix.SharedStream("side")
         self.GetBatch(self.train_dataset_)
-        self.Fprop(True)
-        self.ComputeDeriv()
-        error = self.GetLoss()
-        self._in_train_step = True
+        planes = (self.plane_table_ and self.plane_table_ok_ and self.exchange_ is None
+                  and not self.overlap_update_ and not self.overlap_wgrad_)
         try:
+            if planes:
+                _planes_begin(self._plane_requests, self._plane_count)
+            self.Fprop(True)
+            self.ComputeDeriv()
+            error = self.GetLoss()
+            self._in_train_step = True
             self.Bprop()
             self.UpdateWeights()
         finally:
             self._in_train_step = False
+            if planes:
+                self._plane_count = _planes_end(self._plane_requests, PLANES_MAX)
         self.current_iter_ += 1
         return error
 
diff --git a/convnet_amd/csrc/common.h b/convnet_amd/csrc/common.h
--- a/convnet_amd/csrc/common.h
+++ b/convnet_amd/csrc/common.h
@@ -15,6 +15,7 @@
 void* workspace_planes(size_t bytes);
 void* workspace_banks(size_t bytes);
 void* workspace_slabs(size_t bytes);
+void* workspace_step_planes(size_t bytes);
 const float* zero_page();
 int matrix_path();
 void set_last_error(const char* msg);
@@ -87,6 +88,8 @@
 int wg_batch_frame();
 void wg_batch_end();
 
+void planes_table_drop();
+
 inline int divup(int a, int b) { return (a + b - 1) / b; }
 inline size_t numel(const cudamat* m) { return (size_t)m->size[0] * (size_t)m->size[1]; }
 inline bool aligned16(const void* p) { return (reinterpret_cast<uintptr_t>(p) & 15) == 0; }
diff --git a/convnet_amd/csrc/elementwise.hip b/convnet_amd/csrc/elementwise.hip
--- a/convnet_amd/csrc/elementwise.hip
+++ b/convnet_amd/csrc/elementwise.hip
@@ -854,6 +854,7 @@
   if (int rc = step_check<Op>(mats)) return rc;
   const size_t n = numel(mats[1]);
   if (n == 0) return 0;
+  planes_table_drop();
   KernelTimer timer(name, family, 0.0, step_bytes<Op>() * n);
   hipLaunchKernelGGL(kernel, dim3(blocks_for(n / 4 + 1)), dim3(kThreads), 0, stream(), step_item<Op>(mats, op));
   return launch_status();
@@ -866,6 +867,7 @@
     tensor(i, mats, op);
     if (int rc = step_check<Op>(mats)) return rc;
   }
+  planes_table_drop();
   for (int base = 0; base < count; base += kSgdMulti) {
     StepBatch<Op> b{};
     int m = 0;
@@ -948,6 +950,7 @@
   if (mat->is_trans) return ERROR_TRANSPOSED;
   if (mat->size[0] != target->size[0] || mat->size[1] != target->size[1]) return ERROR_INCOMPATIBLE_DIMENSIONS;
   const int rows = mat->size[0], cols = mat->size[1];
+  planes_table_drop();
   if (axis == 0)
     hipLaunchKernelGGL(normlimit_cols_kernel, dim3(cols), dim3(256), 0, stream(), mat->data_device, target->data_device, rows, norm, constraint);
   else
@@ -962,6 +965,7 @@
   if (numel(grad) != n || numel(history) != n) return ERROR_INCOMPATIBLE_DIMENSIONS;
   if (param->is_trans) return ERROR_TRANSPOSED;
   if (n == 0) return 0;
+  planes_table_drop();
   return rows_normlimit(grad->data_device, param->data_device, param->data_device, history->data_device, param->size[0], param->size[1], norm,
                         constraint, true, l2_decay, gradient_clip, epsilon, momentum);
 }
diff --git a/convnet_amd/csrc/fewc_conv.hip b/convnet_amd/csrc/fewc_conv.hip
--- a/convnet_amd/csrc/fewc_conv.hip
+++ b/convnet_amd/csrc/fewc_conv.hip
@@ -1,17 +1,16 @@
 #include <algorithm>
 
-#include "gather_gemm.h"
+#include "plane_forms.h"
 
 namespace chip {
 namespace gfc {
 
-constexpr int KX = 7, KY = 7, CH = 3, S = 2, NR = CH * KY, P = 4, IMG = 32;
+constexpr int KY = 7, CH = 3, S = 2, NR = CH * KY, P = 4, IMG = 32;
 constexpr int PW = S * (P - 1) + KX;
 constexpr int XB = IMG * 4;
 constexpr int RP = 2;
 constexpr int ROWB = RP * 1024;
 static_assert(PW * XB <= ROWB, "patch row");
-constexpr int NCH = 10, ROWS = 96;
 constexpr int H0_ROWS = 11, H1_ROWS = 10;
 constexpr int H0_BYTES = H0_ROWS * ROWB, H1_BYTES = H1_ROWS * ROWB;
 constexpr int BIAS_OFF = 0, BIAS_BYTES = 512;
@@ -29,11 +28,6 @@
 constexpr int DUMP_BYTES = 4096;
 
 __host__ __device__ constexpr int row_off(int r) { return r < 10 ? r * ROWB : r == 20 ? 10 * ROWB : H0_BYTES + (r - 10) * ROWB; }
-__host__ __device__ constexpr int slot_k(int c, int lh, int j) {
-  const int r = 2 * c + (j >> 2), kx = 2 * (j & 3) + lh;
-  if (kx < KX) return kx + KX * r;
-  return r < KX ? r + KX * 20 : -1;
-}
 
 struct Params {
   const float* src;
@@ -51,24 +45,13 @@
 }
 
 __global__ void gfc_planes_kernel(const float* __restrict__ W, u32x4* __restrict__ out, int F) {
+  gfc_planes_body(W, out, F, (size_t)blockIdx.x * blockDim.x + threadIdx.x, (size_t)gridDim.x * blockDim.x);
+}
+
+void gfc_planes_launch(const float* W, void* out, int F) {
   using namespace gfc;
-  const int i = blockIdx.x * blockDim.x + threadIdx.x;
-  if (i >= NCH * 2 * ROWS) return;
-  const int f = i % ROWS, lh = (i / ROWS) & 1, c = i / (2 * ROWS);
-  Split8 sp = {};
-  if (f < F) {
-    float x[8];
-#pragma unroll
-    for (int j = 0; j < 8; ++j) {
-      const int k = slot_k(c, lh, j);
-      x[j] = k >= 0 ? W[(size_t)f + (size_t)F * k] : 0.f;
-    }
-    split8_sat(x, sp);
-  }
-  u32x4* o = out + ((size_t)c * 6 + lh) * ROWS + f;
-  o[0] = sp.h;
-  o[2 * ROWS] = sp.m;
-  o[4 * ROWS] = sp.l;
+  KernelTimer timer("filter_planes_kernel", "conv_fprop", 0.0, 4.0 * F * CH * KY * KX + A_BYTES);
+  hipLaunchKernelGGL(gfc_planes_kernel, dim3(divup(NCH * 2 * ROWS, 256)), dim3(256), 0, stream(), W, static_cast<u32x4*>(out), F);
 }
 
 template <bool RELU>
@@ -378,15 +361,18 @@
 #endif
     once = true;
   }
-  u32x4* planes = static_cast<u32x4*>(workspace_aux(A_BYTES + DUMP_BYTES));
+  u32x4* const aux = static_cast<u32x4*>(workspace_aux(A_BYTES + DUMP_BYTES));
   (void)filter_planes_shared(nullptr, 0);
-  {
-    KernelTimer timer("filter_planes_kernel", "conv_fprop", 0.0, 4.0 * F * C * Ky * Kx + A_BYTES);
-    hipLaunchKernelGGL(gfc_planes_kernel, dim3(divup(NCH * 2 * ROWS, 256)), dim3(256), 0, stream(), filters, planes, F);
+  ConvnetPlaneRequest rq = plane_request(CONVNET_PLANES_GFC, filters);
+  rq.geo[0] = F;
+  const u32x4* planes = static_cast<const u32x4*>(planes_table_find(rq));
+  if (!planes) {
+    planes = aux;
+    gfc_planes_launch(filters, aux, F);
   }
   Params p{};
   p.src = images; p.planes = planes; p.dst = targets; p.bias = bias; p.zero = zero_page();
-  p.dump = reinterpret_cast<float*>(reinterpret_cast<char*>(planes) + A_BYTES);
+  p.dump = reinterpret_cast<float*>(reinterpret_cast<char*>(aux) + A_BYTES);
   p.F = F; p.N = N; p.H = H; p.W = W; p.My = My; p.Mx = Mx; p.pady = pady; p.padx = padx;
   p.XG = divup(Mx, P); p.IB = N / IMG; p.tiles = p.XG * My * p.IB;
   p.relu = relu; p.diag = CHIP_DIAG_KNOB("CONVNET_GFC_DIAG", 0);
diff --git a/convnet_amd/csrc/gather_gemm.h b/convnet_amd/csrc/gather_gemm.h
--- a/convnet_amd/csrc/gather_gemm.h
+++ b/convnet_amd/csrc/gather_gemm.h
@@ -444,8 +444,8 @@
   int F, C, Ky, Kx, cy, cx, sy, sx, TYc, TXc;
   bool dgrad;
 };
-void filter_planes_rt_launch(const PatchBank& bank, void* out, int TYX, int TH, const char* op);
-void filter_planes_gk_launch(const float* W, void* out, int F, int K, int KP, int TH, const char* op);
+const void* filter_planes_rt_launch(const PatchBank& bank, void* out, int TYX, int TH, const char* op);
+const void* filter_planes_gk_launch(const float* W, void* out, int F, int K, int KP, int TH, const char* op);
 bool patch_shape_ok(GGParams& p, size_t dst_elems);
 void patch_run(GGParams& p, size_t dst_elems, const char* op, double flops, const PatchBank& bank);
 bool patch_classes_ok(const GGParams& base, const GGClassTable& ct);
diff --git a/convnet_amd/csrc/gather_gemm.hip b/convnet_amd/csrc/gather_gemm.hip
--- a/convnet_amd/csrc/gather_gemm.hip
+++ b/convnet_amd/csrc/gather_gemm.hip
@@ -1658,8 +1658,7 @@
       (size_t)g.C * g.H * g.W * g.N < (size_t(1) << 30)) {
     const int K = g.C * g.Ky * g.Kx, KP = divup(K, BK) * BK, TH = gg_tile_rows(g.F);
     void* planes = workspace_aux((size_t)96 * (KP / 16) * divup(g.F, TH) * TH);
-    filter_planes_gk_launch(filters->data_device, planes, g.F, K, KP, TH, "conv_fprop");
-    p.A = static_cast<const float*>(planes);
+    p.A = static_cast<const float*>(filter_planes_gk_launch(filters->data_device, planes, g.F, K, KP, TH, "conv_fprop"));
     p.apre = 1;
     p.gk = 1;
     p.ktab = gk_table(g.C, g.H, g.W, g.N, g.Ky, g.Kx);
@@ -1685,8 +1684,7 @@
       const int TH = gg_tile_rows(g.F);
       void* planes = workspace_aux((size_t)96 * (g.C / 16) * p.TYX * divup(g.F, TH) * TH);
       const PatchBank bank{filters->data_device, g.F, g.C, g.Ky, g.Kx, 0, 0, 1, 1, g.Ky, g.Kx, false};
-      filter_planes_rt_launch(bank, planes, p.TYX, TH, "conv_fprop");
-      p.A = static_cast<const float*>(planes);
+      p.A = static_cast<const float*>(filter_planes_rt_launch(bank, planes, p.TYX, TH, "conv_fprop"));
       p.apre = 1;
     } else if (p.TYX > 1) {
       float* wt = static_cast<float*>(workspace_aux(sizeof(float) * welems));
@@ -1836,8 +1834,7 @@
     if (pre && welems > 0) {
       float* pc = planes + poff;
       poff += ((size_t)24 * (g.F / 16) * TYc * TXc * divup(g.C, TH) * TH + 63) / 64 * 64;
-      filter_planes_rt_launch(bank, pc, TYc * TXc, TH, "conv_dgrad");
-      k.A = pc;
+      k.A = static_cast<const float*>(filter_planes_rt_launch(bank, pc, TYc * TXc, TH, "conv_dgrad"));
     } else if (welems > 0) {
       int nb = (int)((welems + 255) / 256);
       if (nb > 2048) nb = 2048;
diff --git a/convnet_amd/csrc/patch_gemm.hip b/convnet_amd/csrc/patch_gemm.hip
--- a/convnet_amd/csrc/patch_gemm.hip
+++ b/convnet_amd/csrc/patch_gemm.hip
@@ -2,8 +2,9 @@
 #include <cmath>
 #include <cstdlib>
 #include <string>
-
-#include "gather_gemm.h"
+#include <vector>
+
+#include "plane_forms.h"
 
 #ifndef CONVNET_GPV_LDS_MAP
 #define CONVNET_GPV_LDS_MAP 0
@@ -44,74 +45,16 @@
 }
 
 __global__ void filter_planes_rt_kernel(const float* __restrict__ W, u32x4* __restrict__ out, int F, int C, int TYX, int TH) {
-  const int RT = (F + TH - 1) / TH;
-  const size_t total = (size_t)(C / 16) * TYX * 2 * RT * TH;
-  for (size_t i = (size_t)blockIdx.x * blockDim.x + threadIdx.x; i < total; i += (size_t)gridDim.x * blockDim.x) {
-    const int f = (int)(i % (RT * TH));
-    const size_t r = i / (RT * TH);
-    const int lh = (int)(r & 1);
-    const size_t chunk = r >> 1;
-    const int tap = (int)(chunk % TYX), cb = (int)(chunk / TYX);
-    Split8 sp = {};
-    if (f < F) {
-      float x[8];
-#pragma unroll
-      for (int j = 0; j < 8; ++j) x[j] = W[(size_t)f + (size_t)F * (tap + (size_t)TYX * (16 * cb + 2 * j + lh))];
-      split8_sat(x, sp);
-    }
-    u32x4* o = out + ((chunk * RT + f / TH) * 6 + lh) * TH + f % TH;
-    o[0] = sp.h;
-    o[2 * TH] = sp.m;
-    o[4 * TH] = sp.l;
-  }
+  filter_planes_rt_body(W, out, F, C, TYX, TH, (size_t)blockIdx.x * blockDim.x + threadIdx.x, (size_t)gridDim.x * blockDim.x);
 }
 __global__ void dgrad_filter_planes_rt_kernel(const float* __restrict__ W, u32x4* __restrict__ out, int F, int C, int Ky, int Kx, int cy, int cx,
                                               int sy, int sx, int TYc, int TXc, int TH) {
-  const int TYXc = TYc * TXc, RT = (C + TH - 1) / TH;
-  const size_t total = (size_t)(F / 16) * TYXc * 2 * RT * TH;
-  for (size_t i = (size_t)blockIdx.x * blockDim.x + threadIdx.x; i < total; i += (size_t)gridDim.x * blockDim.x) {
-    const int c = (int)(i % (RT * TH));
-    const size_t r = i / (RT * TH);
-    const int lh = (int)(r & 1);
-    const size_t chunk = r >> 1;
-    const int tap = (int)(chunk % TYXc), fb = (int)(chunk / TYXc);
-    const int a = tap / TXc, b = tap - a * TXc;
-    Split8 sp = {};
-    if (c < C) {
-      const float* wp = W + (size_t)F * ((cx + sx * b) + Kx * ((cy + sy * a) + (size_t)Ky * c)) + 16 * fb + lh;
-      float x[8];
-#pragma unroll
-      for (int j = 0; j < 8; ++j) x[j] = wp[2 * j];
-      split8_sat(x, sp);
-    }
-    u32x4* o = out + ((chunk * RT + c / TH) * 6 + lh) * TH + c % TH;
-    o[0] = sp.h;
-    o[2 * TH] = sp.m;
-    o[4 * TH] = sp.l;
-  }
+  dgrad_filter_planes_rt_body(W, out, F, C, Ky, Kx, cy, cx, sy, sx, TYc, TXc, TH, (size_t)blockIdx.x * blockDim.x + threadIdx.x,
+                              (size_t)gridDim.x * blockDim.x);
 }
 
 __global__ void filter_planes_gk_kernel(const float* __restrict__ W, u32x4* __restrict__ out, int F, int K, int KP, int TH) {
-  const int RT = (F + TH - 1) / TH;
-  const size_t total = (size_t)(KP / 16) * 2 * RT * TH;
-  for (size_t i = (size_t)blockIdx.x * blockDim.x + threadIdx.x; i < total; i += (size_t)gridDim.x * blockDim.x) {
-    const int f = (int)(i % (RT * TH));
-    const size_t r = i / (RT * TH);
-    const int lh = (int)(r & 1);
-    const size_t chunk = r >> 1;
-    float x[8];
-#pragma unroll
-    for (int j = 0; j < 8; ++j) {
-      const int k = 16 * (int)chunk + 2 * j + lh;
-      x[j] = (f < F && k < K) ? W[(size_t)f + (size_t)F * k] : 0.f;
-    }
-    Split8 sp;
-    split8_sat(x, sp);
-    u32x4* o = out + ((chunk * RT + f / TH) * 6 + lh) * TH + f % TH;
-    o[0] = sp.h;
-    o[2 * TH] = sp.m;
-    o[4 * TH] = sp.l;
-  }
+  filter_planes_gk_body(W, out, F, K, KP, TH, (size_t)blockIdx.x * blockDim.x + threadIdx.x, (size_t)gridDim.x * blockDim.x);
 }
 namespace {
 bool g_share_on = false;
@@ -131,30 +74,206 @@
   return same;
 }
 
-void filter_planes_gk_launch(const float* W, void* out, int F, int K, int KP, int TH, const char* op) {
+namespace {
+struct PlaneJob {
+  const float* W;
+  u32x4* out;
+  int form, b0;
+  int g[12];
+};
+struct PlaneBatch {
+  PlaneJob j[CONVNET_PLANES_MAX];
+  int n;
+};
+struct PlaneSlot {
+  ConvnetPlaneRequest rq;
+  const void* buf;
+};
+bool g_tab_open = false;
+hipStream_t g_tab_stream = nullptr;
+int g_tab_n = 0;
+PlaneSlot g_tab[CONVNET_PLANES_MAX];
+std::vector<ConvnetPlaneRequest> g_seen;
+constexpr size_t kSeenMax = 256;
+
+bool same_request(const ConvnetPlaneRequest& a, const ConvnetPlaneRequest& b) {
+  if (a.bank != b.bank || a.form != b.form) return false;
+  for (int i = 0; i < 13; ++i)
+    if (a.geo[i] != b.geo[i]) return false;
+  return true;
+}
+size_t plane_work(const ConvnetPlaneRequest& r) {
+  const int* g = r.geo;
+  if (!r.bank) return 0;
+  switch (r.form) {
+    case CONVNET_PLANES_GK: {
+      const int F = g[0], K = g[1], KP = g[2], TH = g[3];
+      if (F < 1 || K < 1 || KP < K || KP % 16 != 0 || TH < 1) return 0;
+      return (size_t)(KP / 16) * 2 * divup(F, TH) * TH;
+    }
+    case CONVNET_PLANES_RT:
+    case CONVNET_PLANES_RT_DGRAD: {
+      const int F = g[0], C = g[1], Ky = g[2], Kx = g[3], cy = g[4], cx = g[5], sy = g[6], sx = g[7], TYc = g[8], TXc = g[9], TYX = g[10], TH = g[11];
+      const bool dgrad = r.form == CONVNET_PLANES_RT_DGRAD;
+      if (F < 1 || C < 1 || Ky < 1 || Kx < 1 || cy < 0 || cx < 0 || sy < 1 || sx < 1 || TYc < 1 || TXc < 1 || TH < 1) return 0;
+      if (TYX != TYc * TXc || cy + sy * (TYc - 1) >= Ky || cx + sx * (TXc - 1) >= Kx) return 0;
+      if (!dgrad && (cy != 0 || cx != 0 || sy != 1 || sx != 1 || TYc != Ky || TXc != Kx)) return 0;
+      const int R = dgrad ? C : F, KCn = dgrad ? F : C;
+      if (KCn % 16 != 0) return 0;
+      return (size_t)(KCn / 16) * TYX * 2 * divup(R, TH) * TH;
+    }
+    case CONVNET_PLANES_GFC:
+      if (g[0] < 1 || g[0] > gfc::ROWS) return 0;
+      return (size_t)gfc::NCH * 2 * gfc::ROWS;
+    default:
+      return 0;
+  }
+}
+}
+
+__global__ void __launch_bounds__(256) planes_multi_kernel(const PlaneBatch b) {
+  int j = 0;
+  while (j + 1 < b.n && (int)blockIdx.x >= b.j[j + 1].b0) ++j;
+  const PlaneJob& q = b.j[j];
+  const int nb = (j + 1 < b.n ? b.j[j + 1].b0 : (int)gridDim.x) - q.b0;
+  const size_t tid = (size_t)((int)blockIdx.x - q.b0) * 256 + threadIdx.x, stride = (size_t)nb * 256;
+  const int* g = q.g;
+  switch (q.form) {
+    case CONVNET_PLANES_GK: filter_planes_gk_body(q.W, q.out, g[0], g[1], g[2], g[3], tid, stride); break;
+    case CONVNET_PLANES_RT: filter_planes_rt_body(q.W, q.out, g[0], g[1], g[10], g[11], tid, stride); break;
+    case CONVNET_PLANES_RT_DGRAD:
+      dgrad_filter_planes_rt_body(q.W, q.out, g[0], g[1], g[2], g[3], g[4], g[5], g[6], g[7], g[8], g[9], g[11], tid, stride);
+      break;
+    default: gfc_planes_body(q.W, q.out, g[0], tid, stride); break;
+  }
+}
+
+#ifdef CONVNET_EMU
+void* workspace_step_planes(size_t bytes) {
+  static void* p = nullptr;
+  static size_t cap = 0;
+  if (bytes > cap) {
+    free(p);
+    cap = (bytes + 4095) / 4096 * 4096;
+    p = aligned_alloc(4096, cap);
+  }
+  return p;
+}
+#endif
+
+ConvnetPlaneRequest plane_request(int form, const float* bank) {
+  ConvnetPlaneRequest rq{};
+  rq.bank = bank;
+  rq.form = form;
+  return rq;
+}
+const void* planes_table_find(const ConvnetPlaneRequest& rq) {
+  if (!g_tab_open || g_share_on || CHIP_DIAG_KNOB("CONVNET_GPP_DIAG", 0) || stream() != g_tab_stream) return nullptr;
+  bool known = false;
+  for (const ConvnetPlaneRequest& s : g_seen) known = known || same_request(s, rq);
+  if (!known && g_seen.size() < kSeenMax) g_seen.push_back(rq);
+  for (int i = 0; i < g_tab_n; ++i)
+    if (same_request(g_tab[i].rq, rq)) return g_tab[i].buf;
+  return nullptr;
+}
+void planes_table_drop() { g_tab_n = 0; }
+
+int planes_table_begin(const ConvnetPlaneRequest* reqs, int n) {
+  g_tab_open = false;
+  g_tab_n = 0;
+  g_seen.clear();
+  g_tab_open = true;
+  g_tab_stream = stream();
+  if (!reqs || n <= 0) return 0;
+  PlaneBatch b{};
+  size_t off[CONVNET_PLANES_MAX], bytes = 0;
+  double moved = 0;
+  int blocks = 0;
+  for (int i = 0; i < n && b.n < CONVNET_PLANES_MAX; ++i) {
+    const size_t work = plane_work(reqs[i]);
+    if (work == 0) continue;
+    bool twice = false;
+    for (int k = 0; k < b.n; ++k) twice = twice || same_request(g_tab[k].rq, reqs[i]);
+    if (twice) continue;
+    int nb = (int)((work + 255) / 256);
+    if (nb > 2048) nb = 2048;
+    PlaneJob& q = b.j[b.n];
+    q.W = reqs[i].bank;
+    q.form = reqs[i].form;
+    q.b0 = blocks;
+    for (int k = 0; k < 12; ++k) q.g[k] = reqs[i].geo[k];
+    g_tab[b.n].rq = reqs[i];
+    off[b.n] = bytes;
+    bytes += (work * 48 + 255) / 256 * 256;
+    moved += 48.0 * work + 4.0 * 8 * work;
+    blocks += nb;
+    ++b.n;
+  }
+  if (b.n == 0) return 0;
+  char* base = static_cast<char*>(workspace_step_planes(bytes));
+  for (int i = 0; i < b.n; ++i) {
+    b.j[i].out = reinterpret_cast<u32x4*>(base + off[i]);
+    g_tab[i].buf = base + off[i];
+  }
+  {
+    KernelTimer timer("planes_multi_kernel", "conv_planes", 0.0, moved);
+    hipLaunchKernelGGL(planes_multi_kernel, dim3(blocks), dim3(256), 0, stream(), b);
+  }
+  g_tab_n = b.n;
+  g_tab_open = true;
+  return b.n;
+}
+int planes_table_end(ConvnetPlaneRequest* seen, int cap) {
+  int m = 0;
+  if (g_tab_open && seen)
+    for (const ConvnetPlaneRequest& s : g_seen)
+      if (m < cap) seen[m++] = s;
+  g_tab_open = false;
+  g_tab_n = 0;
+  g_seen.clear();
+  return m;
+}
+
+void plane_launch_one(const ConvnetPlaneRequest& rq, void* out, const char* op) {
+  const int* g = rq.geo;
+  int nb = (int)((plane_work(rq) + 255) / 256);
+  if (nb > 2048) nb = 2048;
+  u32x4* o = static_cast<u32x4*>(out);
+  if (rq.form == CONVNET_PLANES_GFC) {
+    gfc_planes_launch(rq.bank, out, g[0]);
+  } else if (rq.form == CONVNET_PLANES_GK) {
+    KernelTimer timer("filter_planes_kernel", op, 0.0, 10.0 * (double)g[0] * g[1]);
+    hipLaunchKernelGGL(filter_planes_gk_kernel, dim3(nb), dim3(256), 0, stream(), rq.bank, o, g[0], g[1], g[2], g[3]);
+  } else if (rq.form == CONVNET_PLANES_RT) {
+    KernelTimer timer("filter_planes_kernel", op, 0.0, 10.0 * (double)g[0] * g[1] * g[10]);
+    hipLaunchKernelGGL(filter_planes_rt_kernel, dim3(nb), dim3(256), 0, stream(), rq.bank, o, g[0], g[1], g[10], g[11]);
+  } else {
+    KernelTimer timer("dgrad_filter_planes_kernel", op, 0.0, 10.0 * (double)g[1] * g[0] * g[10]);
+    hipLaunchKernelGGL(dgrad_filter_planes_rt_kernel, dim3(nb), dim3(256), 0, stream(), rq.bank, o, g[0], g[1], g[2], g[3], g[4], g[5], g[6], g[7],
+                       g[8], g[9], g[11]);
+  }
+}
+
+const void* filter_planes_gk_launch(const float* W, void* out, int F, int K, int KP, int TH, const char* op) {
   const long long key[7] = {0, (long long)(uintptr_t)W, (long long)(uintptr_t)out, F, K, KP, TH};
-  if (filter_planes_shared(key, 7)) return;
-  const size_t work = (size_t)(KP / 16) * 2 * divup(F, TH) * TH;
-  int nb = (int)((work + 255) / 256);
-  if (nb > 2048) nb = 2048;
-  KernelTimer timer("filter_planes_kernel", op, 0.0, 10.0 * (double)F * K);
-  hipLaunchKernelGGL(filter_planes_gk_kernel, dim3(nb), dim3(256), 0, stream(), W, static_cast<u32x4*>(out), F, K, KP, TH);
-}
-
-void filter_planes_rt_launch(const PatchBank& b, void* out, int TYX, int TH, const char* op) {
+  if (filter_planes_shared(key, 7)) return out;
+  ConvnetPlaneRequest rq = plane_request(CONVNET_PLANES_GK, W);
+  rq.geo[0] = F; rq.geo[1] = K; rq.geo[2] = KP; rq.geo[3] = TH;
+  if (const void* ready = planes_table_find(rq)) return ready;
+  plane_launch_one(rq, out, op);
+  return out;
+}
+
+const void* filter_planes_rt_launch(const PatchBank& b, void* out, int TYX, int TH, const char* op) {
   const long long key[17] = {1, (long long)(uintptr_t)b.W, (long long)(uintptr_t)out, b.F, b.C, b.Ky, b.Kx, b.cy, b.cx, b.sy, b.sx, b.TYc, b.TXc,
                              b.dgrad, TYX, TH, 0};
-  if (filter_planes_shared(key, 17)) return;
-  const int R = b.dgrad ? b.C : b.F, KCn = b.dgrad ? b.F : b.C;
-  const size_t work = (size_t)(KCn / 16) * TYX * 2 * divup(R, TH) * TH;
-  int nb = (int)((work + 255) / 256);
-  if (nb > 2048) nb = 2048;
-  KernelTimer timer(b.dgrad ? "dgrad_filter_planes_kernel" : "filter_planes_kernel", op, 0.0, 10.0 * (double)R * KCn * TYX);
-  if (b.dgrad)
-    hipLaunchKernelGGL(dgrad_filter_planes_rt_kernel, dim3(nb), dim3(256), 0, stream(), b.W, static_cast<u32x4*>(out), b.F, b.C, b.Ky, b.Kx, b.cy,
-                       b.cx, b.sy, b.sx, b.TYc, b.TXc, TH);
-  else
-    hipLaunchKernelGGL(filter_planes_rt_kernel, dim3(nb), dim3(256), 0, stream(), b.W, static_cast<u32x4*>(out), b.F, b.C, TYX, TH);
+  if (filter_planes_shared(key, 17)) return out;
+  ConvnetPlaneRequest rq = plane_request(b.dgrad ? CONVNET_PLANES_RT_DGRAD : CONVNET_PLANES_RT, b.W);
+  const int geo[12] = {b.F, b.C, b.Ky, b.Kx, b.cy, b.cx, b.sy, b.sx, b.TYc, b.TXc, TYX, TH};
+  for (int i = 0; i < 12; ++i) rq.geo[i] = geo[i];
+  if (const void* ready = planes_table_find(rq)) return ready;
+  plane_launch_one(rq, out, op);
+  return out;
 }
 
 __device__ __forceinline__ int slot_pos(int img) { return (img & 48) | ((img + (img >> 4)) & 15); }
@@ -1633,8 +1752,7 @@
   {
     const size_t welems = (size_t)CB * p.TYX * RT * ROWS * 16;
     u32x4* ap = static_cast<u32x4*>(workspace_aux(welems * 6 + (CHIP_DIAG_KNOB("CONVNET_GPP_DIAG", 0) ? 65536 : 0)));
-    filter_planes_rt_launch(bank, ap, p.TYX, ROWS, op);
-    p.A = reinterpret_cast<const float*>(ap);
+    p.A = static_cast<const float*>(filter_planes_rt_launch(bank, ap, p.TYX, ROWS, op));
     p.apre = 1;
   }
   u32x4* planes = nullptr;
@@ -1746,6 +1864,15 @@
 }
 
 extern "C" {
+int convnet_hip_planes_begin(void* reqs, int n) { return chip::planes_table_begin(static_cast<const ConvnetPlaneRequest*>(reqs), n); }
+int convnet_hip_planes_end(void* seen, int cap) { return chip::planes_table_end(static_cast<ConvnetPlaneRequest*>(seen), cap); }
+size_t convnet_hip_planes_bytes(void* req) { return req ? 48 * chip::plane_work(*static_cast<const ConvnetPlaneRequest*>(req)) : 0; }
+int convnet_hip_planes_build(void* req, void* out) {
+  if (convnet_hip_planes_bytes(req) == 0 || !out || !chip::aligned16(out)) return ERROR_UNSUPPORTED;
+  chip::plane_launch_one(*static_cast<const ConvnetPlaneRequest*>(req), out, "conv_planes");
+  return chip::launch_status();
+}
+void* convnet_hip_planes_find(void* req) { return req ? const_cast<void*>(chip::planes_table_find(*static_cast<const ConvnetPlaneRequest*>(req))) : nullptr; }
 void convnet_hip_set_patch_mode(int mode) { chip::g_patch_mode = mode < 0 ? 0 : mode > 4 ? 4 : mode; }
 int convnet_hip_get_patch_mode(void) { return chip::patch_mode(); }
 }
diff --git a/convnet_amd/csrc/plane_forms.h b/convnet_amd/csrc/plane_forms.h
--- /dev/null
+++ b/convnet_amd/csrc/plane_forms.h
@@ -0,0 +1,106 @@
+#pragma once
+#include "gather_gemm.h"
+
+namespace chip {
+
+namespace gfc {
+constexpr int KX = 7, NCH = 10, ROWS = 96;
+__host__ __device__ constexpr int slot_k(int c, int lh, int j) {
+  const int r = 2 * c + (j >> 2), kx = 2 * (j & 3) + lh;
+  if (kx < KX) return kx + KX * r;
+  return r < KX ? r + KX * 20 : -1;
+}
+}
+
+__device__ __forceinline__ void planes_store(u32x4* o, const Split8& sp, int TH) {
+  o[0] = sp.h;
+  o[2 * TH] = sp.m;
+  o[4 * TH] = sp.l;
+}
+
+__device__ __forceinline__ void filter_planes_rt_body(const float* __restrict__ W, u32x4* __restrict__ out, int F, int C, int TYX, int TH, size_t tid,
+                                                      size_t stride) {
+  const int RT = (F + TH - 1) / TH;
+  const size_t total = (size_t)(C / 16) * TYX * 2 * RT * TH;
+  for (size_t i = tid; i < total; i += stride) {
+    const int f = (int)(i % (RT * TH));
+    const size_t r = i / (RT * TH);
+    const int lh = (int)(r & 1);
+    const size_t chunk = r >> 1;
+    const int tap = (int)(chunk % TYX), cb = (int)(chunk / TYX);
+    Split8 sp = {};
+    if (f < F) {
+      float x[8];
+#pragma unroll
+      for (int j = 0; j < 8; ++j) x[j] = W[(size_t)f + (size_t)F * (tap + (size_t)TYX * (16 * cb + 2 * j + lh))];
+      split8_sat(x, sp);
+    }
+    planes_store(out + ((chunk * RT + f / TH) * 6 + lh) * TH + f % TH, sp, TH);
+  }
+}
+__device__ __forceinline__ void dgrad_filter_planes_rt_body(const float* __restrict__ W, u32x4* __restrict__ out, int F, int C, int Ky, int Kx, int cy,
+                                                            int cx, int sy, int sx, int TYc, int TXc, int TH, size_t tid, size_t stride) {
+  const int TYXc = TYc * TXc, RT = (C + TH - 1) / TH;
+  const size_t total = (size_t)(F / 16) * TYXc * 2 * RT * TH;
+  for (size_t i = tid; i < total; i += stride) {
+    const int c = (int)(i % (RT * TH));
+    const size_t r = i / (RT * TH);
+    const int lh = (int)(r & 1);
+    const size_t chunk = r >> 1;
+    const int tap = (int)(chunk % TYXc), fb = (int)(chunk / TYXc);
+    const int a = tap / TXc, b = tap - a * TXc;
+    Split8 sp = {};
+    if (c < C) {
+      const float* wp = W + (size_t)F * ((cx + sx * b) + Kx * ((cy + sy * a) + (size_t)Ky * c)) + 16 * fb + lh;
+      float x[8];
+#pragma unroll
+      for (int j = 0; j < 8; ++j) x[j] = wp[2 * j];
+      split8_sat(x, sp);
+    }
+    planes_store(out + ((chunk * RT + c / TH) * 6 + lh) * TH + c % TH, sp, TH);
+  }
+}
+__device__ __forceinline__ void filter_planes_gk_body(const float* __restrict__ W, u32x4* __restrict__ out, int F, int K, int KP, int TH, size_t tid,
+                                                      size_t stride) {
+  const int RT = (F + TH - 1) / TH;
+  const size_t total = (size_t)(KP / 16) * 2 * RT * TH;
+  for (size_t i = tid; i < total; i += stride) {
+    const int f = (int)(i % (RT * TH));
+    const size_t r = i / (RT * TH);
+    const int lh = (int)(r & 1);
+    const size_t chunk = r >> 1;
+    float x[8];
+#pragma unroll
+    for (int j = 0; j < 8; ++j) {
+      const int k = 16 * (int)chunk + 2 * j + lh;
+      x[j] = (f < F && k < K) ? W[(size_t)f + (size_t)F * k] : 0.f;
+    }
+    Split8 sp;
+    split8_sat(x, sp);
+    planes_store(out + ((chunk * RT + f / TH) * 6 + lh) * TH + f % TH, sp, TH);
+  }
+}
+__device__ __forceinline__ void gfc_planes_body(const float* __restrict__ W, u32x4* __restrict__ out, int F, size_t tid, size_t stride) {
+  using namespace gfc;
+  for (size_t t = tid; t < (size_t)(NCH * 2 * ROWS); t += stride) {
+    const int i = (int)t;
+    const int f = i % ROWS, lh = (i / ROWS) & 1, c = i / (2 * ROWS);
+    Split8 sp = {};
+    if (f < F) {
+      float x[8];
+#pragma unroll
+      for (int j = 0; j < 8; ++j) {
+        const int k = slot_k(c, lh, j);
+        x[j] = k >= 0 ? W[(size_t)f + (size_t)F * k] : 0.f;
+      }
+      split8_sat(x, sp);
+    }
+    planes_store(out + ((size_t)c * 6 + lh) * ROWS + f, sp, ROWS);
+  }
+}
+
+ConvnetPlaneRequest plane_request(int form, const float* bank);
+const void* planes_table_find(const ConvnetPlaneRequest& rq);
+void gfc_planes_launch(const float* W, void* out, int F);
+
+}
diff --git a/convnet_amd/csrc/state.hip b/convnet_amd/csrc/state.hip
--- a/convnet_amd/csrc/state.hip
+++ b/convnet_amd/csrc/state.hip
@@ -60,7 +60,7 @@
   void* p = nullptr;
   size_t cap = 0;
 };
-std::map<hipStream_t, Arena> g_arena[5];
+std::map<hipStream_t, Arena> g_arena[6];
 
 void* arena_get(int which, size_t bytes, size_t slack) {
   flush_pending();
@@ -80,6 +80,8 @@
 void* workspace_planes(size_t bytes) { return arena_get(2, bytes, size_t(1) << 22); }
 void* workspace_banks(size_t bytes) { return arena_get(3, bytes, size_t(1) << 20); }
 void* workspace_slabs(size_t bytes) { return arena_get(4, bytes, size_t(1) << 20); }
+
+void* workspace_step_planes(size_t bytes) { return arena_get(5, bytes, size_t(1) << 20); }
 
 const float* zero_page() {
   static float* z = nullptr;
@@ -161,6 +163,7 @@
 
 void convnet_hip_shutdown(void) {
   flush_pending();
+  planes_table_drop();
   hipDeviceSynchronize();
   for (auto& per_stream : g_arena) {
     for (auto& kv : per_stream)
@@ -199,6 +202,7 @@
 
 int cuda_set_device(int deviceId) {
   flush_pending();
+  planes_table_drop();
   return hipSetDevice(deviceId) == hipSuccess ? 0 : CUDA_ERROR;
 }
 
diff --git a/include/convnet_hip.h b/include/convnet_hip.h
--- a/include/convnet_hip.h
+++ b/include/convnet_hip.h
@@ -68,6 +68,21 @@
 void convnet_hip_set_deferred_epilogues(int on);
 int convnet_hip_get_deferred_epilogues(void);
 long convnet_hip_deferred_absorbed(void);
+#define CONVNET_PLANES_MAX 16
+#define CONVNET_PLANES_GK 0
+#define CONVNET_PLANES_RT 1
+#define CONVNET_PLANES_RT_DGRAD 2
+#define CONVNET_PLANES_GFC 3
+typedef struct ConvnetPlaneRequest {
+  const float* bank;
+  int form;
+  int geo[13];
+} ConvnetPlaneRequest;
+int convnet_hip_planes_begin(void* reqs, int n);
+int convnet_hip_planes_end(void* seen, int cap);
+size_t convnet_hip_planes_bytes(void* req);
+int convnet_hip_planes_build(void* req, void* out);
+void* convnet_hip_planes_find(void* req);
 const char* get_last_cuda_error(void);
 int cuda_set_device(int deviceId);
 void cuda_sync_threads(void);
```

New measurement: 28140 (median of 6 runs). Within noise of the previous version (+0.3%).
